# BoyBaykiller/IDKEngine

Hardware: AMD Instinct MI355X
Metric: Mray/s (primary+1 bounce) at 1920x1080, 1M-tri scene (higher is better)
Workload: dtype f32

## Files before the change

### idkengine_amd/csrc/host_context.hpp

```cpp
#pragma once


struct DevBuf {
    void* p = nullptr; size_t bytes = 0;
    hipError_t ensure(size_t n) { if (n <= bytes && p) return hipSuccess; if (p) (void)hipFree(p); p = nullptr; bytes = 0; if (n == 0) return hipSuccess; hipError_t e = hipMalloc(&p, n); if (e == hipSuccess) bytes = n; return e; }
    void release() { if (p) (void)hipFree(p); p = nullptr; bytes = 0; }
    template <class T> T* as() const { return (T*)p; }
};

struct DevOptions {
    int forceGeneric = 0;
    int noTileCull = 0;
    int noLeanPrimary = 0;
    int leafMin = 0;
    int grabUnitLog2 = 10, grabFixed = 0;
    int ldsPad = 0;
    int traceWaves = 0;
    int gridHint = 2;
    int deferLast = 1;
    int graphProbe = 0;
    int gridMidWaves = 20;
    int gridRaysX4 = 6;
    int traceVariant = 0;
    int bvhTiming = 0, bvhSmall = 32;
    int advMin = 0;
    int poolMin = 12;
    int leafPool = -1;
    int splitScatter = 6;
    int queryScheduler = 1;
    int groupThreads = -1;
    int fused = 1;
    int fusedShadeMin = 16;
    int splitPeek = 64;
    int splitDonor = 1;
    int split = 1;
    int wide = 0;
    int wideCap = 0;
    int wideCount = 0;
    int genPixelMajor = 8;
    int bouncePixelMajor = 1;
    int genGroupMax = 16;
    int instSieve = 8;
    int instSieveOverlap = 50;
    int instTlas = 8;
    int instTlasOverlap = 10;
    int instBraid = 0;
    int instUnify = 4096;
    int instGeneral = 0;
    int uniRefill = 32;
    int instUnifyRadius = 15;
    int pairNodes = 1;
    int packet = 1;
    int packetMinLive = 60;
    int packetWaves = 0;
    int bvhStackOptHost = 0;
};

enum { VB_NODES = 0, VB_TRIVERTS, VB_VERTICES, VB_TLAS, VB_XFORMS, VB_COUNT };
struct PendingSample { uint32_t accum; int slot; float cam[36]; uint8_t vs[VB_COUNT]; };

struct dev_ctx {
    int device = 0;
    hipStream_t stream = nullptr; bool ownStream = true;
    std::string lastError;
    idkpt_error_fn errFn = nullptr; void* errUser = nullptr;
    int numCUs = 256;
    idkpt_settings st;
    idkpt_settings stCaller;
    int W = 0, H = 0, rowMod = 1, rowRem = 0, rows = 0, rowBandLog2 = 0;
    float invProj[16], invView[16], viewPos[3];
    int ringSize = 1, curSlot = 0; bool ringStarted = false; std::vector<uint32_t> accum = std::vector<uint32_t>(1, 0u);
    bool counters = false, timing = false, capturePrimary = false;
    DevOptions opt;
    uint32_t seqFirst = 0, seqStride = 1;
    bool haveScene = false, frameOk = false;
    DevBuf nodes, tris, triVerts, descs, instances, tlas, parents, leaves, positions, prevPositions, vertices, meshes, materials, xforms, lights, sky, texDescs, unskinned, joints, levelNodes, tlasScratch, queryIn, queryOut, queryRec, queryList, tileClass, gbases;
    std::vector<DevBuf> texData; std::vector<std::pair<int, int>> texDims; std::vector<uint32_t> texState;
    DevBuf srgbLut;
    std::vector<GpuBlasDesc> hDescs;
    std::vector<std::vector<uint32_t>> levelOffsets;
    std::vector<uint32_t> levelBase;
    std::vector<char> refitCoversAll;
    int nodeCount = 0, triCount = 0, instanceCount = 0, tlasCount = 0, vertexCount = 0, meshCount = 0, materialCount = 0, xformCount = 0, lightCount = 0, skySize = 0, textureCount = 0, unskinnedCount = 0;
    int sceneStack = 1;
    int hInst0Blas = 0;
    DevBuf wnodes, wleaf, wids, wpair, wcounts, wtotals; std::vector<uint32_t> wNodeOff, wLeafOff; bool wideTopoValid = false, wideFillValid = false;
    DevBuf pairNodes; bool pairValid = false;
    DevBuf instRec; bool instRecValid = false;
    DevBuf itlas, imarks, ichunks; int itlasNeed = 1; uint32_t ichunkCount = 0; bool itlasValid = false, imarksValid = false;
    int uniMode = 0; uint32_t uniBaseB = 0, uniRestoreIdx = 0;
    DevBuf unodes, utlas, uTabs, uniBuf, uniEntRec; bool uniValid = false, uniEligible = false, uniTabsValid = false; int uniCap = 0, uniEntries = 0, uniDepth = 0; float* hUni = nullptr; float* dUni = nullptr;
    std::vector<GpuBlasInstance> hInstances; std::vector<char> hXforms; uint64_t uniLaunches = 0;
    DevBuf entRec, braidBuf; bool itlasBraided = false; int itlasDepth = 0, itlasEntries = 0;
    int pkState = 0, pkBatchesSinceProbe = 0; unsigned long long* hPkStats = nullptr; unsigned long long* dPkStats = nullptr; unsigned long long pkSeen[6] = {0, 0, 0, 0, 0, 0}; float pkCam[36] = {0}; int pkW = 0, pkRows = 0, pkBatch = 0; float pkLastLive = -1.0f;
    float* hInstOverlap = nullptr; float* dInstOverlap = nullptr; bool instOverlapKnown = false, itlasBuilt = false, isieveWorth = false;
    int verSlots = 1; size_t vbytes[VB_COUNT] = {0}, vstride[VB_COUNT] = {0}; int valloc[VB_COUNT] = {1, 1, 1, 1, 1}, vcur[VB_COUNT] = {0};
    uint64_t lastMask[VB_COUNT] = {0};
    uint8_t lastSlots[VB_COUNT] = {0}; bool lastMulti = false;
    DevBuf verTab; uint32_t* hVerTab = nullptr; hipEvent_t evVer[2] = {nullptr, nullptr}; int verHalf = 0;
    char* hStage = nullptr; hipEvent_t evStage[4] = {nullptr, nullptr, nullptr, nullptr}; int stageNext = 0;
    int (*groupFlushAll)(void* user) = nullptr;
    DevBuf pmList;
    DevBuf trRec, contFlag, blockSums, rayO, rayT, rayR, aovA, aovN, hit, hitCost, primHit, queue[2], keys[2], keysTmp, sortKeys, sortVals, contMask, waveCounts, counts, work, sortHist, counters64;
    DevBuf img[3];
    DevBuf camTab;
    int rowLimit = 0x7fffffff;
    idkpt_bounce_exchange_fn exchangeFn = nullptr; void* exchangeUser = nullptr;
    idkpt_band_exchange_fn bandExchangeFn = nullptr; void* bandExchangeUser = nullptr; DevBuf bandTab;
    idkpt_band_exchange_device_fn bandExchangeDevFn = nullptr; void* bandExchangeDevUser = nullptr;
    idkpt_stats stats;
    uint32_t* hCounts = nullptr; uint32_t* dCountsMirror = nullptr;
    bool sceneNested = false;
    bool sceneNoEmission = false;
    struct { bool valid = false, allHits = false; int j = 0, side = 0, B = 0; uint32_t total = 0, Npad = 0; } defer;
    DevBuf radSave, deferCount;
    bool countersDirty = true;
    uint32_t* hOverflow = nullptr; uint32_t* dOverflow = nullptr;
    int tlasNeed = 1;
    hipEvent_t evFrame[2] = {nullptr, nullptr};
    std::vector<hipEvent_t> evPool; size_t evUsed = 0;
    double traceMsAcc = 0.0; uint64_t traceLaunchesAcc = 0;
    int lastQueueSide = 0; int lastQueueCountSlot = 0; bool lastFast = false, lastNeedsRegen = false; int lastBatch = 1; Frame lastFrame;
    int maxBatch = 1; uint32_t Npad = 0; std::vector<PendingSample> pending; DevBuf bases, qwork; uint32_t* hBases = nullptr; uint32_t* dBasesMirror = nullptr;
    float* hCams = nullptr; hipEvent_t evCams[2] = {nullptr, nullptr}; int camHalf = 0;
    bool grouped = false, inGroupFlush = false; int groupIndex = 0;
    hipEvent_t* evBounce = nullptr;
    int (*groupExchange)(void* user, dev_ctx* member, int bounce, int samples, const uint32_t** outBases) = nullptr; void* groupUser = nullptr;
    struct BuilderScratch* bscratch = nullptr;
    struct PeerPolicy* peer = nullptr;
};

static hipEvent_t next_event(dev_ctx* ctx)
{
    if (ctx->evUsed == ctx->evPool.size()) { hipEvent_t e = nullptr; if (hipEventCreate(&e) != hipSuccess) return nullptr; ctx->evPool.push_back(e); }
    return ctx->evPool[ctx->evUsed++];
}
static void resolve_trace_events(dev_ctx* ctx)
{
    for (size_t i = 0; i + 1 < ctx->evUsed; i += 2) { float ms = 0.0f; if (hipEventElapsedTime(&ms, ctx->evPool[i], ctx->evPool[i + 1]) == hipSuccess) { ctx->traceMsAcc += ms; ctx->traceLaunchesAcc++; } }
    ctx->evUsed = 0;
}
#define TRACE_T0() do { if (ctx->timing) { hipEvent_t _e = next_event(ctx); if (_e) (void)hipEventRecord(_e, st); } } while (0)
#define TRACE_T1() do { if (ctx->timing) { hipEvent_t _e = next_event(ctx); if (_e) (void)hipEventRecord(_e, st); } } while (0)

static int fail(dev_ctx* c, int code, const std::string& msg) { if (c) { c->lastError = msg; if (c->errFn) c->errFn(c->errUser, (int32_t)code, c->lastError.c_str()); } return code; }
#define HIPC(expr) do { hipError_t _e = (expr); if (_e != hipSuccess) { (void)hipGetLastError(); return fail(ctx, IDKPT_ERR_HIP, std::string(#expr) + ": " + hipGetErrorString(_e)); } } while (0)
#define REQUIRE(cond, msg) do { if (!(cond)) return fail(ctx, IDKPT_ERR_INVALID_ARGUMENT, msg); } while (0)

static int local_rows(int H, int mod, int rem, int bandLog2 = 0)
{
    if (bandLog2 == 0) { int n = 0; for (int y = rem; y < H; y += mod) n++; return n; }
    int n = 0; const int band = 1 << bandLog2;
    for (int b = rem; (b << bandLog2) < H; b += mod) n += std::min(band, H - (b << bandLog2));
    return n;
}
```

### idkengine_amd/csrc/host_options.hpp

```cpp
#pragma once

static int32_t dev_SetOption(dev_ctx* ctx, const char* name, int32_t value)
{
    if (!ctx || !name) return IDKPT_ERR_INVALID_ARGUMENT;
    HIPC(hipSetDevice(ctx->device));
    FLUSH();
    DevOptions& o = ctx->opt;
    const std::string n(name);
    if (n == "force_generic") o.forceGeneric = value != 0;
    else if (n == "no_tile_cull") o.noTileCull = value != 0;
    else if (n == "no_lean_primary") o.noLeanPrimary = value != 0;
    else if (n == "leaf_min") o.leafMin = std::max(0, value);
    else if (n == "grab_unit_log2") o.grabUnitLog2 = value;
    else if (n == "grab_fixed") o.grabFixed = value;
    else if (n == "lds_pad") o.ldsPad = value;
    else if (n == "trace_waves") o.traceWaves = std::max(0, value);
    else if (n == "grid_hint") o.gridHint = std::max(0, value);
    else if (n == "grid_rays_x4") o.gridRaysX4 = std::max(0, value);
    else if (n == "grid_mid_waves") o.gridMidWaves = std::max(0, value);
    else if (n == "defer_last") o.deferLast = value != 0;
    else if (n == "split") { REQUIRE(value >= 0 && value <= 3, "idkptSetDeveloperOption: split is 0..3"); o.split = value; }
    else if (n == "split_donor") o.splitDonor = value != 0;
    else if (n == "split_peek") o.splitPeek = std::max(1, value);
    else if (n == "split_scatter") o.splitScatter = std::min(6, std::max(0, value));
    else if (n == "query_scheduler") o.queryScheduler = value != 0;
    else if (n == "group_threads") o.groupThreads = value;
    else if (n == "fused") { REQUIRE(value >= 0 && value <= 2, "idkptSetDeveloperOption: fused is 0..2"); o.fused = value; }
    else if (n == "fused_shade_min") o.fusedShadeMin = std::min(64, std::max(1, value));
    else if (n == "leaf_pool") { REQUIRE(value >= -1 && value <= 7, "idkptSetDeveloperOption: leaf_pool is -1 (automatic) or a mask 0..7 (1: primary launches, 2: the first bounce, 4: later bounces)"); o.leafPool = value; }
    else if (n == "pool_min") o.poolMin = std::max(0, value);
    else if (n == "adv_min") o.advMin = std::min(64, std::max(0, value));
#ifdef IDKPT_DEVELOPER
    else if (n == "graph_probe") o.graphProbe = std::max(0, value);
#endif
    else if (n == "inst_tlas_overlap") { REQUIRE(value >= 0 && value <= 100, "idkptSetDeveloperOption: inst_tlas_overlap is a percentage"); FLUSH(); o.instTlasOverlap = value; ctx->itlasValid = false; }
    else if (n == "bounce_pixel_major") { REQUIRE(value >= 0 && value <= 2, "idkptSetDeveloperOption: bounce_pixel_major is 0..2"); o.bouncePixelMajor = value; }
    else if (n == "gen_group_max") { REQUIRE(value >= 1 && value <= 16, "idkptSetDeveloperOption: gen_group_max is 1..16"); o.genGroupMax = value; }
    else if (n == "gen_pixel_major") { REQUIRE(value >= 0, "idkptSetDeveloperOption: gen_pixel_major is >= 0"); o.genPixelMajor = value; }
    else if (n == "inst_sieve_overlap") { REQUIRE(value >= 0 && value <= 100, "idkptSetDeveloperOption: inst_sieve_overlap is a percentage"); FLUSH(); o.instSieveOverlap = value; ctx->itlasValid = false; }
    else if (n == "inst_sieve") { REQUIRE(value >= 0, "idkptSetDeveloperOption: inst_sieve is >= 0"); FLUSH(); o.instSieve = value; ctx->itlasValid = false; }
    else if (n == "inst_braid") { REQUIRE(value >= 0, "idkptSetDeveloperOption: inst_braid is >= 0"); FLUSH(); o.instBraid = value; ctx->itlasValid = false; }
    else if (n == "pair_nodes") { REQUIRE(value == 0 || value == 1, "idkptSetDeveloperOption: pair_nodes is 0 or 1"); o.pairNodes = value; }
    else if (n == "inst_general") { REQUIRE(value >= 0, "idkptSetDeveloperOption: inst_general is >= 0"); FLUSH(); o.instGeneral = value; ctx->itlasValid = false; }
    else if (n == "uni_refill") { REQUIRE(value == 16 || value == 32, "idkptSetDeveloperOption: uni_refill is 16 or 32"); o.uniRefill = value; }
    else if (n == "inst_unify_radius") { REQUIRE(value >= 1 && value <= 512, "idkptSetDeveloperOption: inst_unify_radius is 1-512"); FLUSH(); o.instUnifyRadius = value; ctx->itlasValid = false; }
    else if (n == "inst_unify") { REQUIRE(value >= 0, "idkptSetDeveloperOption: inst_unify is >= 0"); FLUSH(); o.instUnify = value; ctx->itlasValid = false; }
    else if (n == "inst_tlas") { REQUIRE(value >= 0, "idkptSetDeveloperOption: inst_tlas is >= 0"); FLUSH(); o.instTlas = value; ctx->itlasValid = false; }
    else if (n == "packet") { REQUIRE(value >= 0 && value <= 2, "idkptSetDeveloperOption: packet is 0..2"); o.packet = value; ctx->pkState = 0; ctx->pkBatchesSinceProbe = 0; }
    else if (n == "packet_min_live") { REQUIRE(value >= 0 && value <= 100, "idkptSetDeveloperOption: packet_min_live is a percentage"); o.packetMinLive = value; ctx->pkState = 0; ctx->pkBatchesSinceProbe = 0; }
    else if (n == "packet_waves") { REQUIRE(value >= 0 && value <= 32, "idkptSetDeveloperOption: packet_waves is 0 (default) or 1..32"); o.packetWaves = value; }
    else if (n == "wide") { REQUIRE(value >= 0 && value <= 1, "idkptSetDeveloperOption: wide is 0 or 1"); FLUSH(); o.wide = value; }
    else if (n == "wide_cap") { REQUIRE(value >= 0 && value <= 96, "idkptSetDeveloperOption: wide_cap is 0 (default) or 4..96 rows"); o.wideCap = value; }
    else if (n == "wide_count") o.wideCount = value != 0;
    else if (n == "bvh_timing") o.bvhTiming = value != 0;
    else if (n == "bvh_small") o.bvhSmall = value;
    else if (n == "bvh_stackopt_host") o.bvhStackOptHost = value != 0;
    else if (n == "force_no_peer") { }
    else if (n == "trace_variant") {
#ifdef IDKPT_DEVELOPER
        o.traceVariant = value;
#else
        REQUIRE(value == 0 || value == 100, "idkptSetDeveloperOption: trace_variant needs the developer build of the library (libidkpt_dev.so)");
#endif
    }
    else return fail(ctx, IDKPT_ERR_INVALID_ARGUMENT, "idkptSetDeveloperOption: unknown option '" + n + "'");
    return IDKPT_OK;
}
```

### idkengine_amd/csrc/host_scene.hpp

```cpp
#pragma once

static int blas_stack_need(const GpuBlasNode* nodes, int nodeCount)
{
    std::vector<int> need((size_t)nodeCount, 0);
    for (int p = nodeCount - 2; p >= 2; p--) {
        const GpuBlasNode& l = nodes[p]; const GpuBlasNode& r = nodes[p + 1];
        const bool tl = l.TriCount == 0 && l.TriStartOrChild != 0, tr = r.TriCount == 0 && r.TriStartOrChild != 0;
        if (tl && tr) need[p] = std::max(need[l.TriStartOrChild], need[r.TriStartOrChild]) + 1;
        else if (tl || tr) need[p] = need[tl ? l.TriStartOrChild : r.TriStartOrChild];
    }
    return nodeCount > 2 ? need[2] : 0;
}

static int tlas_validate(const GpuTlasNode* nodes, int nodeCount, int instanceCount, const char** why)
{
    if (nodeCount <= 0) return 0;
    const uint32_t* w = (const uint32_t*)nodes;
    std::vector<int> need((size_t)nodeCount, 0);
    for (int i = nodeCount - 1; i >= 0; i--) {
        const uint32_t packed = w[8 * (size_t)i + 3], id = packed & 0x7fffffffu;
        if (packed >> 31) { if (id >= (uint32_t)instanceCount) { *why = "TLAS leaf references an instance out of range"; return -1; } continue; }
        if (id <= (uint32_t)i || (uint64_t)id + 1 >= (uint64_t)nodeCount) { *why = "TLAS child index out of range (children must lie behind their parent)"; return -1; }
        need[i] = std::max(need[id], need[id + 1]) + 1;
    }
// ... 4 lines not shown
{
    int maxStack = 1;
    for (int i = 0; i < descCount; i++) {
        const GpuBlasDesc& d = descs[i];
        if (!(d.NodeOffset >= 0 && d.NodeCount >= 4 && d.NodeOffset + d.NodeCount <= nodeCount && d.TriangleOffset >= 0 && d.TriangleOffset + d.TriangleCount <= triangleCount)) return "BlasDesc range out of bounds";
        for (int n = 1; n < d.NodeCount; n++) {
            const GpuBlasNode& nd = nodes[d.NodeOffset + n];
            if (nd.TriCount > 0) { if (!((uint64_t)nd.TriStartOrChild + nd.TriCount <= (uint64_t)d.TriangleCount)) return "leaf triangle range out of bounds"; }
            else if (n == 1 || nd.TriStartOrChild != 0) { if (!(nd.TriStartOrChild >= 2 && nd.TriStartOrChild > (uint32_t)n && nd.TriStartOrChild + 1 < (uint32_t)d.NodeCount)) return "child index out of bounds (children must lie behind their parent)"; }
        }
        const int need = blas_stack_need(nodes + d.NodeOffset, d.NodeCount);
        if (checkClaim && d.RequiredStackSize < need) return "BlasDesc.RequiredStackSize is smaller than the stack the BLAS needs";
        maxStack = std::max(maxStack, need);
    }
    *outMaxStack = maxStack;
    return nullptr;
}

static bool blas_nested(const GpuBlasNode* nodes, const GpuBlasDesc* descs, int descCount)
{
    for (int i = 0; i < descCount; i++) {
        const GpuBlasDesc& d = descs[i];
        for (int n = 1; n < d.NodeCount; n++) {
            const GpuBlasNode& p = nodes[d.NodeOffset + n];
            if (p.TriCount > 0 || p.TriStartOrChild == 0) continue;
            for (int k = 0; k < 2; k++) {
                const GpuBlasNode& c = nodes[d.NodeOffset + p.TriStartOrChild + k];
                if (c.TriCount == 0 && c.TriStartOrChild == 0 && n != 0) continue;
                for (int a = 0; a < 3; a++) if (!(c.Min[a] >= p.Min[a] && c.Max[a] <= p.Max[a])) return false;
            }
        }
    }
    return true;
}


static const char* dev_GetVersionString(void) { return "idkpt 0.1 (gfx950)"; }

static int32_t dev_GetDeviceCount(int32_t* outCount)
{
    int n = 0; hipError_t e = hipGetDeviceCount(&n);
    if (outCount) *outCount = (e == hipSuccess) ? n : 0;
    return e == hipSuccess ? IDKPT_OK : IDKPT_ERR_NO_DEVICE;
}

static int32_t dev_Create(int32_t deviceCount, const int32_t* deviceIds, dev_ctx** outCtx)
{
    if (!outCtx) return IDKPT_ERR_INVALID_ARGUMENT;
    *outCtx = nullptr;
    if (deviceCount != 1) return IDKPT_ERR_INVALID_ARGUMENT;
    int n = 0;
    if (hipGetDeviceCount(&n) != hipSuccess || n <= 0) return IDKPT_ERR_NO_DEVICE;
    int dev = deviceIds ? deviceIds[0] : 0;
    if (dev < 0 || dev >= n) return IDKPT_ERR_INVALID_ARGUMENT;
    if (hipSetDevice(dev) != hipSuccess) return IDKPT_ERR_HIP;
    dev_ctx* ctx = new dev_ctx();
    ctx->device = dev;
    hipDeviceProp_t prop;
    if (hipGetDeviceProperties(&prop, dev) == hipSuccess) ctx->numCUs = prop.multiProcessorCount;
    if (hipStreamCreateWithFlags(&ctx->stream, hipStreamNonBlocking) != hipSuccess) { delete ctx; return IDKPT_ERR_HIP; }
    memset(&ctx->st, 0, sizeof(ctx->st));
    ctx->st.Gpu.FocalLength = 8.0f; ctx->st.Gpu.DoRussianRoulette = 1; ctx->st.RayDepth = 7; ctx->st.SamplesPerPixel = 1;
    ctx->stCaller = ctx->st;
    memset(&ctx->stats, 0, sizeof(ctx->stats));
    memset(ctx->invProj, 0, 64); memset(ctx->invView, 0, 64); memset(ctx->viewPos, 0, 12);
    if (hipHostMalloc((void**)&ctx->hCounts, MAX_DEPTH_SLOTS * 4 + 16, hipHostMallocMapped) != hipSuccess || hipHostGetDevicePointer((void**)&ctx->dCountsMirror, ctx->hCounts, 0) != hipSuccess) { delete ctx; return IDKPT_ERR_OUT_OF_MEMORY; }
    memset(ctx->hCounts, 0, MAX_DEPTH_SLOTS * 4 + 16);
    if (hipHostMalloc((void**)&ctx->hOverflow, 64, hipHostMallocMapped) != hipSuccess || hipHostGetDevicePointer((void**)&ctx->dOverflow, ctx->hOverflow, 0) != hipSuccess) { delete ctx; return IDKPT_ERR_OUT_OF_MEMORY; }
    *ctx->hOverflow = 0;
    if (hipHostMalloc((void**)&ctx->hBases, MAX_DEPTH_SLOTS * (MAX_BATCH + 1) * 4, hipHostMallocMapped) != hipSuccess || hipHostGetDevicePointer((void**)&ctx->dBasesMirror, ctx->hBases, 0) != hipSuccess) { delete ctx; return IDKPT_ERR_OUT_OF_MEMORY; }
    memset(ctx->hBases, 0, MAX_DEPTH_SLOTS * (MAX_BATCH + 1) * 4);
    (void)hipEventCreate(&ctx->evFrame[0]); (void)hipEventCreate(&ctx->evFrame[1]);
    *outCtx = ctx;
    return IDKPT_OK;
}

static void builder_scratch_free(dev_ctx* ctx);
static int32_t dev_Destroy(dev_ctx* ctx)
{
    if (!ctx) return IDKPT_ERR_INVALID_ARGUMENT;
    (void)hipSetDevice(ctx->device);
    ctx->pending.clear();
    (void)hipStreamSynchronize(ctx->stream);
    DevBuf* all[] = {&ctx->srgbLut, &ctx->pmList, &ctx->pairNodes, &ctx->instRec, &ctx->entRec, &ctx->braidBuf, &ctx->unodes, &ctx->utlas, &ctx->uTabs, &ctx->uniBuf, &ctx->uniEntRec, &ctx->itlas, &ctx->imarks, &ctx->ichunks, &ctx->wnodes, &ctx->wleaf, &ctx->wids, &ctx->wpair, &ctx->wcounts, &ctx->wtotals, &ctx->nodes, &ctx->tris, &ctx->triVerts, &ctx->descs, &ctx->instances, &ctx->tlas, &ctx->parents, &ctx->leaves, &ctx->positions, &ctx->prevPositions, &ctx->vertices, &ctx->meshes,
                     &ctx->materials, &ctx->xforms, &ctx->lights, &ctx->sky, &ctx->texDescs, &ctx->unskinned, &ctx->joints, &ctx->levelNodes, &ctx->tlasScratch, &ctx->queryIn, &ctx->queryOut, &ctx->queryRec, &ctx->queryList, &ctx->bandTab, &ctx->tileClass, &ctx->gbases, &ctx->camTab, &ctx->verTab, &ctx->trRec, &ctx->contFlag, &ctx->blockSums, &ctx->rayO, &ctx->rayT, &ctx->rayR, &ctx->aovA, &ctx->aovN, &ctx->hit,
                     &ctx->hitCost, &ctx->primHit, &ctx->queue[0], &ctx->queue[1], &ctx->keys[0], &ctx->keys[1], &ctx->keysTmp, &ctx->sortKeys, &ctx->sortVals, &ctx->contMask, &ctx->waveCounts,
                     &ctx->counts, &ctx->work, &ctx->qwork, &ctx->radSave, &ctx->deferCount, &ctx->sortHist, &ctx->counters64, &ctx->bases, &ctx->img[0], &ctx->img[1], &ctx->img[2]};
    for (DevBuf* b : all) b->release();
    for (auto& t : ctx->texData) t.release();
    builder_scratch_free(ctx);
    if (ctx->hCounts) (void)hipHostFree(ctx->hCounts);
    if (ctx->hOverflow) (void)hipHostFree(ctx->hOverflow);
    if (ctx->hInstOverlap) (void)hipHostFree(ctx->hInstOverlap);
    if (ctx->hUni) (void)hipHostFree(ctx->hUni);
    if (ctx->hPkStats) (void)hipHostFree(ctx->hPkStats);
    if (ctx->hBases) (void)hipHostFree(ctx->hBases);
    if (ctx->hCams) (void)hipHostFree(ctx->hCams);
    for (int i = 0; i < 2; i++) if (ctx->evCams[i]) (void)hipEventDestroy(ctx->evCams[i]);
    if (ctx->hVerTab) (void)hipHostFree(ctx->hVerTab);
    for (int i = 0; i < 2; i++) if (ctx->evVer[i]) (void)hipEventDestroy(ctx->evVer[i]);
    if (ctx->hStage) (void)hipHostFree(ctx->hStage);
    for (int i = 0; i < 4; i++) if (ctx->evStage[i]) (void)hipEventDestroy(ctx->evStage[i]);
    if (ctx->evFrame[0]) (void)hipEventDestroy(ctx->evFrame[0]);
    if (ctx->evFrame[1]) (void)hipEventDestroy(ctx->evFrame[1]);
    for (hipEvent_t e : ctx->evPool) (void)hipEventDestroy(e);
    if (ctx->ownStream && ctx->stream) (void)hipStreamDestroy(ctx->stream);
    delete ctx;
    return IDKPT_OK;
}

static int32_t dev_GetLastError(dev_ctx* ctx, const char** outMessage)
{
    if (!ctx || !outMessage) return IDKPT_ERR_INVALID_ARGUMENT;
    *outMessage = ctx->lastError.c_str();
    return IDKPT_OK;
}

static int32_t dev_SetSize(dev_ctx* ctx, int32_t width, int32_t height)
{
    if (!ctx) return IDKPT_ERR_INVALID_ARGUMENT;
    REQUIRE(width > 0 && height > 0 && width <= 4096 && height <= 65536, "idkptSetSize: bad size (FirstHit seeds pack x into 12 bits: width <= 4096)");
    HIPC(hipSetDevice(ctx->device));
    FLUSH();
    REQUIRE(ctx->rowLimit == 0x7fffffff || ctx->rowRem + ctx->rowLimit <= height, "idkptSetSize: the strip set by idkptSetRowRange exceeds the new image height (set a new range first)");
    REQUIRE((ctx->rowRem << ctx->rowBandLog2) < height, "idkptSetSize: this context's row remainder (idkptSetRowSharding / idkptSetRowBands) is outside the new image height");
    ctx->W = width; ctx->H = height; ctx->rows = std::min(ctx->rowLimit, local_rows(height, ctx->rowMod, ctx->rowRem, ctx->rowBandLog2));
    return alloc_frame(ctx);
}

static int32_t dev_SetLayout(dev_ctx* ctx, int32_t width, int32_t height, int32_t rowMod, int32_t rowRem, int32_t rowLimit, int32_t bandLog2 = 0)
{
    if (!ctx) return IDKPT_ERR_INVALID_ARGUMENT;
    REQUIRE(width > 0 && height > 0 && width <= 4096 && height <= 65536, "idkptSetSize: bad size (FirstHit seeds pack x into 12 bits: width <= 4096)");
    REQUIRE(rowMod >= 1 && rowRem >= 0 && bandLog2 >= 0 && bandLog2 <= 6 && (rowRem << bandLog2) < height && rowLimit >= 1 && (rowMod == 1 ? bandLog2 == 0 : rowRem < rowMod), "internal: bad row layout");
    HIPC(hipSetDevice(ctx->device));
    FLUSH();
    ctx->W = width; ctx->H = height; ctx->rowMod = rowMod; ctx->rowRem = rowRem; ctx->rowLimit = rowLimit; ctx->rowBandLog2 = bandLog2;
    ctx->rows = std::min(rowLimit, local_rows(height, rowMod, rowRem, bandLog2));
    return alloc_frame(ctx);
}

static int32_t dev_SetRowBands(dev_ctx* ctx, int32_t bandRows, int32_t rowModulo, int32_t rowRemainder)
{
    if (!ctx) return IDKPT_ERR_INVALID_ARGUMENT;
    REQUIRE(bandRows >= 1 && bandRows <= 64 && (bandRows & (bandRows - 1)) == 0, "idkptSetRowBands: bandRows must be a power of two in 1..64");
    REQUIRE(rowModulo >= 1 && rowRemainder >= 0 && rowRemainder < rowModulo, "idkptSetRowSharding / idkptSetRowBands: need 0 <= remainder < modulo");
    int bandLog2 = 0; while ((1 << bandLog2) < bandRows) bandLog2++;
    if (rowModulo == 1) bandLog2 = 0;
    REQUIRE(ctx->W <= 0 || (rowRemainder << bandLog2) < ctx->H, "idkptSetRowSharding / idkptSetRowBands: no row of the image has this remainder");
    FLUSH();
    ctx->rowMod = rowModulo; ctx->rowRem = rowRemainder; ctx->rowLimit = 0x7fffffff; ctx->rowBandLog2 = bandLog2;
    if (ctx->W > 0) { HIPC(hipSetDevice(ctx->device)); ctx->rows = local_rows(ctx->H, rowModulo, rowRemainder, bandLog2); return alloc_frame(ctx); }
    return IDKPT_OK;
}
static int32_t dev_SetRowSharding(dev_ctx* ctx, int32_t rowModulo, int32_t rowRemainder) { return dev_SetRowBands(ctx, 1, rowModulo, rowRemainder); }

static int32_t dev_SetRowRange(dev_ctx* ctx, int32_t firstRow, int32_t rowCount)
{
    if (!ctx) return IDKPT_ERR_INVALID_ARGUMENT;
    REQUIRE(firstRow >= 0 && rowCount >= 1, "idkptSetRowRange: need firstRow >= 0 and rowCount >= 1");
    REQUIRE(ctx->W <= 0 || firstRow + rowCount <= ctx->H, "idkptSetRowRange: strip exceeds the image height");
    FLUSH();
    ctx->rowMod = 1; ctx->rowRem = firstRow; ctx->rowLimit = rowCount; ctx->rowBandLog2 = 0;
    if (ctx->W > 0) { HIPC(hipSetDevice(ctx->device)); ctx->rows = std::min(ctx->rowLimit, local_rows(ctx->H, 1, firstRow)); return alloc_frame(ctx); }
    return IDKPT_OK;
}

// ... 9 lines not shown
{
    if (!ctx) return IDKPT_ERR_INVALID_ARGUMENT;
    FLUSH();
    ctx->bandExchangeFn = fn; ctx->bandExchangeUser = user;
    return IDKPT_OK;
}

static int32_t dev_SetBandExchangeDevice(dev_ctx* ctx, idkpt_band_exchange_device_fn fn, void* user)
{
    if (!ctx) return IDKPT_ERR_INVALID_ARGUMENT;
    FLUSH();
    ctx->bandExchangeDevFn = fn; ctx->bandExchangeDevUser = user;
    return IDKPT_OK;
}

static int32_t dev_SetSettings(dev_ctx* ctx, const idkpt_settings* s)
{
    if (!ctx || !s) return IDKPT_ERR_INVALID_ARGUMENT;
    REQUIRE(s->RayDepth >= 1 && s->RayDepth < MAX_DEPTH_SLOTS - 2, "idkptSetSettings: RayDepth out of range (1..61)");
    REQUIRE(s->SamplesPerPixel >= 1, "idkptSetSettings: SamplesPerPixel must be >= 1");
    REQUIRE(s->BlasStackSize >= 0, "idkptSetSettings: BlasStackSize must be >= 0 (0 = derive from BlasDescs)");
    REQUIRE(s->BlasStackSize == 0 || !ctx->haveScene || s->BlasStackSize >= ctx->sceneStack, "idkptSetSettings: BlasStackSize is smaller than the scene's maximum RequiredStackSize");
    if (memcmp(&ctx->stCaller, s, sizeof(*s)) == 0) return IDKPT_OK;
    FLUSH();
    ctx->stCaller = *s;
    const idkpt_settings o = ctx->st;
    bool reset = o.RayDepth != s->RayDepth || o.Gpu.FocalLength != s->Gpu.FocalLength || o.Gpu.LenseRadius != s->Gpu.LenseRadius ||
                 o.Gpu.DoDebugBVHTraversal != s->Gpu.DoDebugBVHTraversal || o.Gpu.DoTraceLights != s->Gpu.DoTraceLights || o.UseTlas != s->UseTlas;
    ctx->st = *s;
    if (ctx->st.Gpu.DoDebugBVHTraversal) ctx->st.RayDepth = 1;
    if (reset) std::fill(ctx->accum.begin(), ctx->accum.end(), 0u);
    return IDKPT_OK;
}
static int32_t dev_GetSettings(dev_ctx* ctx, idkpt_settings* out) { if (!ctx || !out) return IDKPT_ERR_INVALID_ARGUMENT; *out = ctx->st; return IDKPT_OK; }

static int32_t dev_SetPerFrame(dev_ctx* ctx, const float invProjection[16], const float invView[16], const float viewPos[3])
{
    if (!ctx || !invProjection || !invView || !viewPos) return IDKPT_ERR_INVALID_ARGUMENT;
    if (ctx->ringSize == 1 && (memcmp(ctx->invProj, invProjection, 64) || memcmp(ctx->invView, invView, 64) || memcmp(ctx->viewPos, viewPos, 12))) FLUSH_KEEP();
    memcpy(ctx->invProj, invProjection, 64); memcpy(ctx->invView, invView, 64); memcpy(ctx->viewPos, viewPos, 12);
    return IDKPT_OK;
}
static int32_t dev_SetPerFrameData(dev_ctx* ctx, const GpuPerFrameData* p) { if (!ctx || !p) return IDKPT_ERR_INVALID_ARGUMENT; return dev_SetPerFrame(ctx, p->InvProjection, p->InvView, p->ViewPos); }

static int regather_triverts(dev_ctx* ctx, uint32_t first, uint32_t count)
{
    if (count == 0) return IDKPT_OK;
    char *src, *dst; int rc = ver_writable(ctx, VB_TRIVERTS, first == 0 && count == (uint32_t)ctx->triCount, &src, &dst); if (rc) return rc;
    hipLaunchKernelGGL(k_gather_triverts, dim3((count + 255) / 256), dim3(256), 0, ctx->stream, ctx->tris.as<uint4>(), ctx->positions.as<float>(), (float4*)dst, first, count);
    HIPC(hipGetLastError());
    return IDKPT_OK;
}

static int upload(dev_ctx* ctx, DevBuf& b, const void* src, size_t bytes)
{
    HIPC(b.ensure(std::max<size_t>(bytes, 16)));
    if (bytes) HIPC(hipMemcpyAsync(b.p, src, bytes, hipMemcpyHostToDevice, ctx->stream));
    return IDKPT_OK;
}

static size_t tex_texel_bytes(int32_t format) { return format == IDKPT_TEXFMT_RGBA32F ? 16 : 4; }
static int tex_validate(dev_ctx* ctx, const idkpt_texture& t, const char* who)
{
    if (!(t.width > 0 && t.height > 0 && t.rgba)) return fail(ctx, IDKPT_ERR_INVALID_ARGUMENT, std::string(who) + ": bad texture (size / data)");
    if (!(t.wrapS >= 0 && t.wrapS <= 2 && t.wrapT >= 0 && t.wrapT <= 2 && t.magFilter >= 0 && t.magFilter <= 1 && t.format >= 0 && t.format <= 2))
        return fail(ctx, IDKPT_ERR_INVALID_ARGUMENT, std::string(who) + ": bad texture (wrapS / wrapT are enum idkpt_wrap, magFilter enum idkpt_filter, format enum idkpt_texture_format)");
    return IDKPT_OK;
}
static uint32_t tex_state(const idkpt_texture& t) { return (uint32_t)t.wrapS | ((uint32_t)t.wrapT << 2) | ((uint32_t)t.magFilter << 4) | ((uint32_t)t.format << 5); }
static bool tex_all_finite(const idkpt_texture& t)
{
    if (t.format != IDKPT_TEXFMT_RGBA32F) return true;
    const uint32_t* w = reinterpret_cast<const uint32_t*>(t.rgba); uint32_t bad = 0;
    for (size_t k = 0, e = (size_t)t.width * t.height * 4; k < e; k++) bad |= (uint32_t)((w[k] & 0x7f800000u) == 0x7f800000u);
    return !bad;
}
static int tex_srgb_lut(dev_ctx* ctx)
{
    if (ctx->srgbLut.p) return IDKPT_OK;
    float lut[256];
    for (int b = 0; b < 256; b++) { const double cs = (double)b / 255.0; lut[b] = (float)(cs <= 0.04045 ? cs / 12.92 : pow((cs + 0.055) / 1.055, 2.4)); }
    HIPC(ctx->srgbLut.ensure(sizeof(lut)));
    HIPC(hipMemcpy(ctx->srgbLut.p, lut, sizeof(lut), hipMemcpyHostToDevice));
    return IDKPT_OK;
}
static int tex_descs_upload(dev_ctx* ctx)
{
    std::vector<TexDesc> td;
    for (size_t i = 0; i < ctx->texData.size(); i++) td.push_back({ctx->texData[i].p, ctx->texDims[i].first, ctx->texDims[i].second, ctx->texState[i], 0u});
    { int rc = upload(ctx, ctx->texDescs, td.data(), td.size() * sizeof(TexDesc)); if (rc) return rc; }
    if (!td.empty()) HIPC(hipStreamSynchronize(ctx->stream));
    return IDKPT_OK;
}

static DScene make_dscene_last(dev_ctx* ctx);
static int materialize_culled_rays(dev_ctx* ctx)
{
    if (!ctx->lastNeedsRegen) return IDKPT_OK;
    const size_t N = (size_t)ctx->W * ctx->rows;
    RayBufs rays = {ctx->rayO.as<float4>(), ctx->rayT.as<float4>(), ctx->rayR.as<float4>(), ctx->aovA.as<float4>(), ctx->aovN.as<float4>()};
    hipLaunchKernelGGL(k_regen_culled, dim3((unsigned)((N + 255) / 256)), dim3(256), 0, ctx->stream, make_dscene_last(ctx), ctx->lastFrame, rays, (const uint8_t*)ctx->contFlag.as<uint8_t>(), (uint32_t)(ctx->lastBatch - 1), (uint32_t)N);
    HIPC(hipGetLastError());
    ctx->lastNeedsRegen = false;
    return IDKPT_OK;
}

static int32_t dev_UploadScene(dev_ctx* ctx, const idkpt_scene_desc* sc)
{
    if (!ctx || !sc) return IDKPT_ERR_INVALID_ARGUMENT;
    REQUIRE(sc->BlasNodes && sc->BlasNodeCount >= 4, "idkptUploadScene: BlasNodes missing");
    REQUIRE(sc->BlasTriangles && sc->BlasTriangleCount > 0, "idkptUploadScene: BlasTriangles missing");
    REQUIRE(sc->BlasDescs && sc->BlasDescCount > 0 && sc->BlasInstances && sc->BlasInstanceCount > 0, "idkptUploadScene: BlasDescs/BlasInstances missing");
    REQUIRE(sc->VertexPositions && sc->Vertices && sc->VertexCount > 0, "idkptUploadScene: vertices missing");
    REQUIRE(sc->Meshes && sc->MeshCount > 0 && sc->Materials && sc->MaterialCount > 0 && sc->MeshTransforms && sc->MeshTransformCount > 0, "idkptUploadScene: meshes/materials/transforms missing");
    REQUIRE(sc->LightCount >= 0 && sc->LightCount <= IDKPT_MAX_LIGHTS, "idkptUploadScene: more than 256 lights");
    for (int i = 0; i < sc->BlasTriangleCount; i++) { const GpuBlasTriangle& t = sc->BlasTriangles[i]; REQUIRE(t.X < (uint32_t)sc->VertexCount && t.Y < (uint32_t)sc->VertexCount && t.Z < (uint32_t)sc->VertexCount && t.MeshId < (uint32_t)sc->MeshCount, "idkptUploadScene: BlasTriangle index out of range"); }
    for (int i = 0; i < sc->MeshCount; i++) REQUIRE(sc->Meshes[i].MaterialId >= 0 && sc->Meshes[i].MaterialId < sc->MaterialCount, "idkptUploadScene: Mesh.MaterialId out of range");
    for (int i = 0; i < sc->BlasInstanceCount; i++) REQUIRE(sc->BlasInstances[i].BlasId < (uint32_t)sc->BlasDescCount && sc->BlasInstances[i].MeshTransformId < (uint32_t)sc->MeshTransformCount, "idkptUploadScene: BlasInstance out of range");
    int maxStack = 1;
    { const char* why = validate_blas_nodes(sc->BlasNodes, sc->BlasNodeCount, sc->BlasDescs, sc->BlasDescCount, sc->BlasTriangleCount, true, &maxStack); REQUIRE(why == nullptr, std::string("idkptUploadScene: ") + (why ? why : "")); }
    REQUIRE(ctx->st.BlasStackSize == 0 || ctx->st.BlasStackSize >= maxStack, "idkptUploadScene: the BlasStackSize set with idkptSetSettings is smaller than this scene's maximum RequiredStackSize");
    int tlasNeed = 1;
    if (sc->TlasNodes && sc->TlasNodeCount > 0) {
        const char* why = nullptr;
        tlasNeed = tlas_validate(sc->TlasNodes, sc->TlasNodeCount, sc->BlasInstanceCount, &why);
        REQUIRE(tlasNeed >= 0, std::string("idkptUploadScene: ") + (why ? why : "bad TLAS"));
        REQUIRE(tlasNeed <= TLAS_STACK_SIZE, "idkptUploadScene: TLAS deeper than TLAS_STACK_SIZE (32)");
    }
    HIPC(hipSetDevice(ctx->device));
    FLUSH();
    { int rc = materialize_culled_rays(ctx); if (rc) return rc; }
    int rc;
    if ((rc = upload(ctx, ctx->nodes, sc->BlasNodes, (size_t)sc->BlasNodeCount * 32))) return rc;
    if ((rc = upload(ctx, ctx->tris, sc->BlasTriangles, (size_t)sc->BlasTriangleCount * 16))) return rc;
    if ((rc = upload(ctx, ctx->descs, sc->BlasDescs, (size_t)sc->BlasDescCount * sizeof(GpuBlasDesc)))) return rc;
    if ((rc = upload(ctx, ctx->instances, sc->BlasInstances, (size_t)sc->BlasInstanceCount * 8))) return rc;
    if ((rc = upload(ctx, ctx->tlas, sc->TlasNodes, (size_t)(sc->TlasNodes ? sc->TlasNodeCount : 0) * 32))) return rc;
    if ((rc = upload(ctx, ctx->parents, sc->BlasParentIndices, (size_t)(sc->BlasParentIndices ? sc->BlasParentIndexCount : 0) * 4))) return rc;
    if ((rc = upload(ctx, ctx->leaves, sc->BlasLeafIndices, (size_t)(sc->BlasLeafIndices ? sc->BlasLeafIndexCount : 0) * 4))) return rc;
    if ((rc = upload(ctx, ctx->positions, sc->VertexPositions, (size_t)sc->VertexCount * 12))) return rc;
    if ((rc = upload(ctx, ctx->vertices, sc->Vertices, (size_t)sc->VertexCount * 16))) return rc;
    if ((rc = upload(ctx, ctx->meshes, sc->Meshes, (size_t)sc->MeshCount * sizeof(GpuMesh)))) return rc;
    if ((rc = upload(ctx, ctx->materials, sc->Materials, (size_t)sc->MaterialCount * sizeof(GpuMaterial)))) return rc;
    if ((rc = upload(ctx, ctx->xforms, sc->MeshTransforms, (size_t)sc->MeshTransformCount * sizeof(GpuMeshTransform)))) return rc;
    HIPC(ctx->lights.ensure(IDKPT_MAX_LIGHTS * sizeof(GpuLight)));
    if (sc->Lights && sc->LightCount) HIPC(hipMemcpyAsync(ctx->lights.p, sc->Lights, (size_t)sc->LightCount * sizeof(GpuLight), hipMemcpyHostToDevice, ctx->stream));
    {
        bool none = true;
        auto fin = [](float v) { return v - v == 0.0f; };
        for (int i = 0; i < sc->MaterialCount && none; i++) { const GpuMaterial& m = sc->Materials[i]; none = m.EmissiveFactor[0] == 0.0f && m.EmissiveFactor[1] == 0.0f && m.EmissiveFactor[2] == 0.0f && fin(m.Absorbance[0]) && fin(m.Absorbance[1]) && fin(m.Absorbance[2]); }
        for (int i = 0; i < sc->MeshCount && none; i++) none = sc->Meshes[i].EmissiveBias == 0.0f && fin(sc->Meshes[i].AbsorbanceBias[0]) && fin(sc->Meshes[i].AbsorbanceBias[1]) && fin(sc->Meshes[i].AbsorbanceBias[2]);
        for (int i = 0; i < sc->TextureCount && none; i++) {
            const idkpt_texture& t = sc->Textures[i];
            if (!(t.width > 0 && t.height > 0 && t.rgba)) { none = false; break; }
            none = tex_all_finite(t);
        }
        ctx->sceneNoEmission = none;
    }
    ctx->skySize = (sc->SkyFaces && sc->SkyFaceSize > 0) ? sc->SkyFaceSize : 0;
    if ((rc = upload(ctx, ctx->sky, sc->SkyFaces, (size_t)6 * ctx->skySize * ctx->skySize * 16))) return rc;
    for (auto& t : ctx->texData) t.release();
    ctx->texData.clear(); ctx->texDims.clear(); ctx->texState.clear();
    if ((rc = tex_srgb_lut(ctx))) return rc;
    for (int i = 0; i < sc->TextureCount; i++) {
        const idkpt_texture& t = sc->Textures[i];
        if ((rc = tex_validate(ctx, t, "idkptUploadScene"))) return rc;
        ctx->texData.emplace_back();
        if ((rc = upload(ctx, ctx->texData.back(), t.rgba, (size_t)t.width * t.height * tex_texel_bytes(t.format)))) return rc;
        ctx->texDims.push_back({t.width, t.height}); ctx->texState.push_back(tex_state(t));
    }
    if ((rc = tex_descs_upload(ctx))) return rc;
    HIPC(ctx->triVerts.ensure((size_t)sc->BlasTriangleCount * 48));
    ctx->nodeCount = sc->BlasNodeCount; ctx->triCount = sc->BlasTriangleCount; ctx->instanceCount = sc->BlasInstanceCount; ctx->tlasCount = sc->TlasNodes ? sc->TlasNodeCount : 0;
    ctx->vertexCount = sc->VertexCount; ctx->meshCount = sc->MeshCount; ctx->materialCount = sc->MaterialCount; ctx->xformCount = sc->MeshTransformCount;
    ctx->lightCount = sc->Lights ? sc->LightCount : 0; ctx->textureCount = sc->TextureCount;
    ctx->hDescs.assign(sc->BlasDescs, sc->BlasDescs + sc->BlasDescCount); ctx->hInst0Blas = (int)sc->BlasInstances[0].BlasId;
    ctx->hInstances.assign(sc->BlasInstances, sc->BlasInstances + sc->BlasInstanceCount);
    ctx->hXforms.assign((const char*)sc->MeshTransforms, (const char*)sc->MeshTransforms + (size_t)sc->MeshTransformCount * sizeof(GpuMeshTransform));
    ctx->sceneStack = maxStack; ctx->tlasNeed = std::max(1, tlasNeed);
    ctx->sceneNested = blas_nested(sc->BlasNodes, sc->BlasDescs, sc->BlasDescCount);
    ver_reset(ctx);
    if ((rc = ver_reserve(ctx))) return rc;
    ctx->levelOffsets.assign(sc->BlasDescCount, {}); ctx->levelBase.assign(sc->BlasDescCount, 0); ctx->refitCoversAll.assign(sc->BlasDescCount, 0);
    std::vector<int32_t> allLevels;
    for (int bi = 0; bi < sc->BlasDescCount; bi++) {
        const GpuBlasDesc& d = sc->BlasDescs[bi];
        if (!d.IsRefittable) continue;
        std::vector<int> depth(d.NodeCount, 0); int maxD = 0;
        for (int n = 1; n < d.NodeCount; n++) { const GpuBlasNode& nd = sc->BlasNodes[d.NodeOffset + n]; if (nd.TriCount == 0) { int c = (int)nd.TriStartOrChild; depth[c] = depth[c + 1] = depth[n] + 1; maxD = std::max(maxD, depth[n]); } }
        std::vector<std::vector<int32_t>> lv(maxD + 1);
        for (int n = 1; n < d.NodeCount; n++) if (sc->BlasNodes[d.NodeOffset + n].TriCount == 0 && (n == 1 || n >= 2)) lv[depth[n]].push_back(n);
        ctx->levelBase[bi] = (uint32_t)allLevels.size();
        uint32_t off = 0;
        for (auto& l : lv) { ctx->levelOffsets[bi].push_back(off); off += (uint32_t)l.size(); allLevels.insert(allLevels.end(), l.begin(), l.end()); }
        ctx->levelOffsets[bi].push_back(off);
        ctx->refitCoversAll[bi] = (int64_t)off + (int64_t)d.LeafIndicesCount == (int64_t)d.NodeCount - 1;
    }
    if ((rc = upload(ctx, ctx->levelNodes, allLevels.data(), allLevels.size() * 4))) return rc;
    if ((rc = regather_triverts(ctx, 0, (uint32_t)sc->BlasTriangleCount))) return rc;
    HIPC(hipStreamSynchronize(ctx->stream));
    ctx->haveScene = true;
    std::fill(ctx->accum.begin(), ctx->accum.end(), 0u);
    return IDKPT_OK;
}

struct PeerPolicy { bool forceStaged = false, warned = false; void* stage = nullptr; size_t stageBytes = 0; };
static hipError_t member_copy(PeerPolicy* pol, void* dst, int dstDev, const void* src, int srcDev, size_t bytes, hipStream_t st)
{
    if (bytes == 0) return hipSuccess;
    if (!pol || !pol->forceStaged) {
        hipError_t e = hipMemcpyPeerAsync(dst, dstDev, src, srcDev, bytes, st);
        if (e == hipSuccess || !pol) return e;
        (void)hipGetLastError();
        if (!pol->warned) { fprintf(stderr, "[idkpt] warning: peer copy GPU %d -> GPU %d refused (%s); staging device-to-device copies through host memory from now on\n", srcDev, dstDev, hipGetErrorString(e)); pol->warned = true; }
        pol->forceStaged = true;
    }
    hipError_t e = hipStreamSynchronize(st); if (e != hipSuccess) return e;
    if (pol->stageBytes < bytes) {
        if (pol->stage) (void)hipHostFree(pol->stage);
        pol->stage = nullptr; pol->stageBytes = 0;
        e = hipHostMalloc(&pol->stage, bytes, hipHostMallocDefault); if (e != hipSuccess) return e;
        pol->stageBytes = bytes;
    }
    int cur = 0; (void)hipGetDevice(&cur);
    e = hipSetDevice(srcDev); if (e == hipSuccess) e = hipMemcpy(pol->stage, src, bytes, hipMemcpyDeviceToHost);
    if (e == hipSuccess) e = hipSetDevice(dstDev);
    if (e == hipSuccess) e = hipMemcpy(dst, pol->stage, bytes, hipMemcpyHostToDevice);
    (void)hipSetDevice(cur);
    return e;
}

struct CloneItem { void* dst; const void* src; size_t bytes; };
static int clone_prepare(dev_ctx* ctx, dev_ctx* src, std::vector<CloneItem>& items)
{
    if (!ctx || !src || !src->haveScene) return IDKPT_ERR_INVALID_ARGUMENT;
    items.clear();
    HIPC(hipSetDevice(ctx->device));
    FLUSH();
    { int rc = materialize_culled_rays(ctx); if (rc) return rc; }
    DevBuf* d[] = {&ctx->nodes, &ctx->tris, &ctx->triVerts, &ctx->descs, &ctx->instances, &ctx->tlas, &ctx->parents, &ctx->leaves, &ctx->positions, &ctx->vertices, &ctx->meshes,
                   &ctx->materials, &ctx->xforms, &ctx->lights, &ctx->sky, &ctx->levelNodes};
    DevBuf* f[] = {&src->nodes, &src->tris, &src->triVerts, &src->descs, &src->instances, &src->tlas, &src->parents, &src->leaves, &src->positions, &src->vertices, &src->meshes,
                   &src->materials, &src->xforms, &src->lights, &src->sky, &src->levelNodes};
    for (size_t i = 0; i < sizeof(d) / sizeof(d[0]); i++) {
        if (!f[i]->p || f[i]->bytes == 0) continue;
        int vb = -1; for (int b = 0; b < VB_COUNT; b++) if (f[i] == &vb_buf(src, b)) vb = b;
        const size_t bytes = (vb >= 0 && src->vbytes[vb] > 0) ? src->vbytes[vb] : f[i]->bytes;
        const char* from = (vb >= 0 && src->vbytes[vb] > 0) ? vb_ptr(src, vb, src->vcur[vb]) : (const char*)f[i]->p;
        HIPC(d[i]->ensure(bytes));
        items.push_back({d[i]->p, from, bytes});
    }
    for (auto& t : ctx->texData) t.release();
    ctx->texData.clear(); ctx->texDims = src->texDims; ctx->texState = src->texState;
    for (size_t i = 0; i < src->texData.size(); i++) {
        ctx->texData.emplace_back();
        HIPC(ctx->texData.back().ensure(src->texData[i].bytes));
        items.push_back({ctx->texData.back().p, src->texData[i].p, src->texData[i].bytes});
    }
    return IDKPT_OK;
}
static int clone_finish(dev_ctx* ctx, dev_ctx* src)
{
    HIPC(hipSetDevice(ctx->device));
    { int rc = tex_srgb_lut(ctx); if (rc) return rc; }
    { int rc = tex_descs_upload(ctx); if (rc) return rc; }
    ctx->nodeCount = src->nodeCount; ctx->triCount = src->triCount; ctx->instanceCount = src->instanceCount; ctx->tlasCount = src->tlasCount; ctx->vertexCount = src->vertexCount;
    ctx->meshCount = src->meshCount; ctx->materialCount = src->materialCount; ctx->xformCount = src->xformCount; ctx->lightCount = src->lightCount; ctx->skySize = src->skySize;
    ctx->textureCount = src->textureCount; ctx->hDescs = src->hDescs; ctx->hInstances = src->hInstances; ctx->hXforms = src->hXforms; ctx->hInst0Blas = src->hInst0Blas; ctx->sceneNoEmission = src->sceneNoEmission; ctx->sceneNested = src->sceneNested; ctx->sceneStack = src->sceneStack; ctx->tlasNeed = src->tlasNeed;
    ctx->levelOffsets = src->levelOffsets; ctx->levelBase = src->levelBase; ctx->refitCoversAll = src->refitCoversAll;
    ver_reset(ctx);
    { int rc = ver_reserve(ctx); if (rc) return rc; }
    HIPC(hipStreamSynchronize(ctx->stream));
    ctx->haveScene = true;
    std::fill(ctx->accum.begin(), ctx->accum.end(), 0u);
    return IDKPT_OK;
}

static int32_t dev_CloneSceneFrom(dev_ctx* ctx, dev_ctx* src)
{
    std::vector<CloneItem> items;
    int rc = clone_prepare(ctx, src, items); if (rc) return rc;
    for (const CloneItem& it : items) HIPC(member_copy(ctx->peer, it.dst, ctx->device, it.src, src->device, it.bytes, ctx->stream));
    return clone_finish(ctx, src);
}

static int32_t dev_UpdateTexture(dev_ctx* ctx, int32_t index, const idkpt_texture* t)
{
    if (!ctx || !t) return IDKPT_ERR_INVALID_ARGUMENT;
    if (!ctx->haveScene) return fail(ctx, IDKPT_ERR_INVALID_OPERATION, "idkptUpdateTexture: no scene uploaded");
    REQUIRE(index >= 0 && index < ctx->textureCount, "idkptUpdateTexture: index out of range");
    { int rc = tex_validate(ctx, *t, "idkptUpdateTexture"); if (rc) return rc; }
    HIPC(hipSetDevice(ctx->device));
    FLUSH();
    HIPC(hipStreamSynchronize(ctx->stream));
    { int rc = upload(ctx, ctx->texData[index], t->rgba, (size_t)t->width * t->height * tex_texel_bytes(t->format)); if (rc) return rc; }
    HIPC(hipStreamSynchronize(ctx->stream));
    ctx->texDims[index] = {t->width, t->height}; ctx->texState[index] = tex_state(*t);
    if (!tex_all_finite(*t)) ctx->sceneNoEmission = false;
    return tex_descs_upload(ctx);
}

static int32_t dev_SetLightCount(dev_ctx* ctx, int32_t count)
{
    if (!ctx) return IDKPT_ERR_INVALID_ARGUMENT;
    REQUIRE(count >= 0 && count <= IDKPT_MAX_LIGHTS, "idkptSetLightCount: out of range");
    FLUSH();
    ctx->lightCount = count; return IDKPT_OK;
}

static DevBuf* which_buffer(dev_ctx* ctx, int which, size_t* cap, int* vb)
{
    *vb = -1;
    switch (which) {
        case IDKPT_BUF_MESH_TRANSFORMS: *cap = (size_t)ctx->xformCount * sizeof(GpuMeshTransform); *vb = VB_XFORMS; return &ctx->xforms;
        case IDKPT_BUF_VERTEX_POSITIONS: *cap = (size_t)ctx->vertexCount * 12; return &ctx->positions;
        case IDKPT_BUF_VERTICES: *cap = (size_t)ctx->vertexCount * 16; *vb = VB_VERTICES; return &ctx->vertices;
        case IDKPT_BUF_MESHES: *cap = (size_t)ctx->meshCount * sizeof(GpuMesh); return &ctx->meshes;
        case IDKPT_BUF_MATERIALS: *cap = (size_t)ctx->materialCount * sizeof(GpuMaterial); return &ctx->materials;
        case IDKPT_BUF_LIGHTS: *cap = (size_t)IDKPT_MAX_LIGHTS * sizeof(GpuLight); return &ctx->lights;
        case IDKPT_BUF_BLAS_NODES: *cap = (size_t)ctx->nodeCount * 32; *vb = VB_NODES; return &ctx->nodes;
        case IDKPT_BUF_TLAS_NODES: *cap = (size_t)ctx->tlasCount * 32; *vb = VB_TLAS; return &ctx->tlas;
        case IDKPT_BUF_JOINT_MATRICES: *cap = ctx->joints.bytes; return &ctx->joints;
        default: return nullptr;
    }
}

static int32_t dev_UpdateBuffer(dev_ctx* ctx, int32_t which, size_t offsetBytes, size_t bytes, const void* data)
{
    if (!ctx || !data) return IDKPT_ERR_INVALID_ARGUMENT;
    if (!ctx->haveScene) return fail(ctx, IDKPT_ERR_INVALID_OPERATION, "idkptUpdateBuffer: no scene uploaded");
    HIPC(hipSetDevice(ctx->device));
    if (which == IDKPT_BUF_MESHES || which == IDKPT_BUF_MATERIALS || which == IDKPT_BUF_LIGHTS || which == IDKPT_BUF_BLAS_NODES || which == IDKPT_BUF_TLAS_NODES) FLUSH();
    if (which == IDKPT_BUF_JOINT_MATRICES) { size_t need = offsetBytes + bytes; if (need > ctx->joints.bytes) { DevBuf nb; HIPC(nb.ensure(need)); if (ctx->joints.p) { HIPC(hipMemcpyAsync(nb.p, ctx->joints.p, ctx->joints.bytes, hipMemcpyDeviceToDevice, ctx->stream)); } HIPC(hipStreamSynchronize(ctx->stream)); ctx->joints.release(); ctx->joints = nb; } }
    size_t cap = 0; int vb = -1; DevBuf* b = which_buffer(ctx, which, &cap, &vb);
    REQUIRE(b != nullptr, "idkptUpdateBuffer: unknown buffer");
    REQUIRE(offsetBytes + bytes <= cap, "idkptUpdateBuffer: range exceeds buffer");
    if (which == IDKPT_BUF_BLAS_NODES || which == IDKPT_BUF_TLAS_NODES) {
        char* cur = vb_ptr(ctx, vb, ctx->vcur[vb]);
        std::vector<char> h(cap);
        HIPC(hipMemcpyAsync(h.data(), cur, cap, hipMemcpyDeviceToHost, ctx->stream)); HIPC(hipStreamSynchronize(ctx->stream));
        memcpy(h.data() + offsetBytes, data, bytes);
        if (which == IDKPT_BUF_BLAS_NODES) {
            int maxStack = 1;
            const char* why = validate_blas_nodes((const GpuBlasNode*)h.data(), ctx->nodeCount, ctx->hDescs.data(), (int)ctx->hDescs.size(), ctx->triCount, false, &maxStack);
            REQUIRE(why == nullptr, std::string("idkptUpdateBuffer: ") + (why ? why : ""));
            REQUIRE(ctx->st.BlasStackSize == 0 || ctx->st.BlasStackSize >= maxStack, "idkptUpdateBuffer: the patched BLAS needs a deeper traversal stack than the BlasStackSize set with idkptSetSettings");
            HIPC(hipMemcpyAsync(cur + offsetBytes, data, bytes, hipMemcpyHostToDevice, ctx->stream));
            ctx->sceneStack = maxStack; ctx->pairValid = false; ctx->wideTopoValid = false; ctx->wideFillValid = false; ctx->itlasValid = false; ctx->instRecValid = false; ctx->imarksValid = false;
            ctx->sceneNested = blas_nested((const GpuBlasNode*)h.data(), ctx->hDescs.data(), (int)ctx->hDescs.size());
        } else {
            const char* why = nullptr;
            const int need = tlas_validate((const GpuTlasNode*)h.data(), ctx->tlasCount, ctx->instanceCount, &why);
            REQUIRE(need >= 0, std::string("idkptUpdateBuffer: ") + (why ? why : "bad TLAS"));
            REQUIRE(need <= TLAS_STACK_SIZE, "idkptUpdateBuffer: TLAS deeper than TLAS_STACK_SIZE (32)");
            HIPC(hipMemcpyAsync(cur + offsetBytes, data, bytes, hipMemcpyHostToDevice, ctx->stream));
            ctx->tlasNeed = std::max(1, need);
        }
        HIPC(hipStreamSynchronize(ctx->stream));
        return IDKPT_OK;
    }
    if (which == IDKPT_BUF_MESHES || which == IDKPT_BUF_MATERIALS) ctx->sceneNoEmission = false;
    char* dst = (char*)b->p;
    if (vb >= 0) { char* src; int rc = ver_writable(ctx, vb, offsetBytes == 0 && bytes == cap, &src, &dst); if (rc) return rc; }
    { int rc = staged_upload(ctx, dst + offsetBytes, data, bytes); if (rc) return rc; }
    if (which == IDKPT_BUF_MESH_TRANSFORMS && offsetBytes + bytes <= ctx->hXforms.size()) memcpy(ctx->hXforms.data() + offsetBytes, data, bytes);
    if (which == IDKPT_BUF_VERTEX_POSITIONS) { int rc = regather_triverts(ctx, 0, (uint32_t)ctx->triCount); if (rc) return rc; }
    return IDKPT_OK;
}

static int32_t dev_DownloadBuffer(dev_ctx* ctx, int32_t which, size_t offsetBytes, size_t bytes, void* dst)
{
    if (!ctx || !dst) return IDKPT_ERR_INVALID_ARGUMENT;
    if (which == IDKPT_BUF_WIDE_NODES || which == IDKPT_BUF_WIDE_LEAVES || which == IDKPT_BUF_WIDE_COUNTS) {
        if (!ctx->haveScene) return fail(ctx, IDKPT_ERR_INVALID_OPERATION, "idkptDownloadBuffer: no scene uploaded");
        HIPC(hipSetDevice(ctx->device));
        FLUSH();
        { int rc = wide_prepare(ctx); if (rc) return rc; }
        DevBuf& wbuf = which == IDKPT_BUF_WIDE_NODES ? ctx->wnodes : (which == IDKPT_BUF_WIDE_LEAVES ? ctx->wleaf : ctx->wcounts);
        REQUIRE(offsetBytes + bytes <= (which == IDKPT_BUF_WIDE_COUNTS ? ctx->hDescs.size() * 8 : wbuf.bytes), "idkptDownloadBuffer: bad buffer/range");
        HIPC(hipMemcpyAsync(dst, (char*)wbuf.p + offsetBytes, bytes, hipMemcpyDeviceToHost, ctx->stream));
        HIPC(hipStreamSynchronize(ctx->stream));
        return IDKPT_OK;
    }
    size_t cap = 0; int vb = -1; DevBuf* b = which_buffer(ctx, which, &cap, &vb);
    REQUIRE(b != nullptr && offsetBytes + bytes <= cap, "idkptDownloadBuffer: bad buffer/range");
    HIPC(hipSetDevice(ctx->device));
    FLUSH();
    HIPC(hipMemcpyAsync(dst, (vb >= 0 ? vb_ptr(ctx, vb, ctx->vcur[vb]) : (char*)b->p) + offsetBytes, bytes, hipMemcpyDeviceToHost, ctx->stream));
    HIPC(hipStreamSynchronize(ctx->stream));
    return IDKPT_OK;
}

static int32_t dev_BuildTlas(dev_ctx* ctx, const GpuTlasNode* nodes, int32_t nodeCount)
{
    if (!ctx || !nodes || nodeCount <= 0) return IDKPT_ERR_INVALID_ARGUMENT;
    if (!ctx->haveScene) return fail(ctx, IDKPT_ERR_INVALID_OPERATION, "idkptBuildTlas: no scene uploaded");
    const char* why = nullptr;
    const int need = tlas_validate(nodes, nodeCount, ctx->instanceCount, &why);
    REQUIRE(need >= 0, std::string("idkptBuildTlas: ") + (why ? why : "bad TLAS"));
    REQUIRE(need <= TLAS_STACK_SIZE, "idkptBuildTlas: TLAS deeper than TLAS_STACK_SIZE (32)");
    HIPC(hipSetDevice(ctx->device));
    if ((size_t)nodeCount * 32 > ctx->vbytes[VB_TLAS] || nodeCount != ctx->tlasCount) {
        FLUSH();
        if ((size_t)nodeCount * 32 > ctx->vbytes[VB_TLAS]) {
            HIPC(hipStreamSynchronize(ctx->stream));
            ctx->tlas.release();
            ctx->vbytes[VB_TLAS] = (size_t)nodeCount * 32; ctx->vstride[VB_TLAS] = (ctx->vbytes[VB_TLAS] + 255) / 256 * 256; ctx->valloc[VB_TLAS] = 1; ctx->vcur[VB_TLAS] = 0;
            HIPC(ctx->tlas.ensure(ctx->vstride[VB_TLAS]));
        }
    }
    char *src, *dst; int rc = ver_writable(ctx, VB_TLAS, true, &src, &dst); if (rc) return rc;
    HIPC(hipMemcpyAsync(dst, nodes, (size_t)nodeCount * 32, hipMemcpyHostToDevice, ctx->stream));
    HIPC(hipStreamSynchronize(ctx->stream));
    ctx->tlasCount = nodeCount; ctx->tlasNeed = std::max(1, need);
    return IDKPT_OK;
}

static int32_t dev_BuildTlasOnDevice(dev_ctx* ctx, int32_t searchRadius)
{
    if (!ctx) return IDKPT_ERR_INVALID_ARGUMENT;
    if (!ctx->haveScene) return fail(ctx, IDKPT_ERR_INVALID_OPERATION, "idkptBuildTlasOnDevice: no scene uploaded");
    REQUIRE(searchRadius >= 1, "idkptBuildTlasOnDevice: searchRadius must be >= 1 (reference: 15)");
    HIPC(hipSetDevice(ctx->device));
    const int n = ctx->instanceCount, nodeCount = 2 * n - 1;
    if (nodeCount != ctx->tlasCount) FLUSH();
    char *tsrc, *tdst; { int rc = ver_writable(ctx, VB_TLAS, true, &tsrc, &tdst); if (rc) return rc; }
    const size_t tempOff = 0, leafOff = (size_t)nodeCount * 32, keyOff = leafOff + (size_t)n * 32, prefOff = keyOff + (size_t)n * 4;
    HIPC(ctx->tlasScratch.ensure(prefOff + (size_t)n * 4));
    char* sc = ctx->tlasScratch.as<char>();
    hipLaunchKernelGGL(k_tlas_build, dim3(1), dim3(TLAS_BUILD_THREADS), 0, ctx->stream, (const float4*)vb_cur<float4>(ctx, VB_NODES), ctx->descs.as<GpuBlasDesc>(), ctx->instances.as<GpuBlasInstance>(),
                       (const float4*)vb_cur<float4>(ctx, VB_XFORMS), n, (int)searchRadius, (float4*)tdst, (float4*)(sc + tempOff), (float4*)(sc + leafOff), (uint32_t*)(sc + keyOff), (int*)(sc + prefOff));
    HIPC(hipGetLastError());
    ctx->tlasCount = nodeCount; ctx->tlasNeed = std::min(TLAS_STACK_SIZE, std::max(1, n));
    return IDKPT_OK;
}

static int32_t dev_RefitBlas(dev_ctx* ctx, int32_t blasId)
{
    if (!ctx) return IDKPT_ERR_INVALID_ARGUMENT;
    if (!ctx->haveScene) return fail(ctx, IDKPT_ERR_INVALID_OPERATION, "idkptRefitBlas: no scene uploaded");
    REQUIRE(blasId >= 0 && blasId < (int)ctx->hDescs.size(), "idkptRefitBlas: blasId out of range");
    const GpuBlasDesc& d = ctx->hDescs[blasId];
    if (!d.IsRefittable || d.LeafIndicesCount == 0) return fail(ctx, IDKPT_ERR_INVALID_OPERATION, "idkptRefitBlas: BLAS is not refittable (no leaf/parent indices)");
    HIPC(hipSetDevice(ctx->device));
    int rc = regather_triverts(ctx, (uint32_t)d.TriangleOffset, (uint32_t)d.TriangleCount); if (rc) return rc;
    const bool whole = ctx->hDescs.size() == 1 && d.NodeOffset == 0 && d.NodeCount == ctx->nodeCount && ctx->refitCoversAll[blasId];
    char *nsrc, *ndst; rc = ver_writable(ctx, VB_NODES, whole, &nsrc, &ndst); if (rc) return rc;
    if (whole && nsrc != ndst) HIPC(hipMemcpyAsync(ndst, nsrc, 32, hipMemcpyDeviceToDevice, ctx->stream));
// ... 50 lines not shown
```

### idkengine_amd/csrc/host_schedule.hpp

```cpp
#pragma once

static DScene make_dscene(dev_ctx* ctx, const uint8_t* slots, bool multi)
{
    DScene s;
    auto at = [&](int b) -> char* { return multi ? (char*)vb_buf(ctx, b).p : vb_ptr(ctx, b, slots ? slots[b] : ctx->vcur[b]); };
    s.nodes = (const float4*)at(VB_NODES); s.tris = ctx->tris.as<uint4>(); s.triVerts = (const float4*)at(VB_TRIVERTS);
    s.descs = ctx->descs.as<GpuBlasDesc>(); s.instances = ctx->instances.as<GpuBlasInstance>(); s.instanceCount = ctx->instanceCount;
    s.tlas = (const float4*)at(VB_TLAS); s.tlasCount = ctx->tlasCount; s.vertices = (const uint4*)at(VB_VERTICES);
    s.instRec = nullptr;
    s.pairNodes = nullptr;
    s.meshes = ctx->meshes.as<GpuMesh>(); s.materials = ctx->materials.as<GpuMaterial>(); s.xforms = (const float4*)at(VB_XFORMS);
    s.lights = ctx->lights.as<GpuLight>(); s.lightCount = ctx->lightCount; s.sky = ctx->sky.as<float4>(); s.skySize = ctx->skySize;
    s.textures = ctx->texDescs.as<TexDesc>(); s.textureCount = ctx->textureCount; s.srgbLut = ctx->srgbLut.as<float>();
    s.overflow = ctx->dOverflow;
    s.ver = multi ? ctx->verTab.as<uint32_t>() : nullptr;
    return s;
}
static DScene make_dscene(dev_ctx* ctx) { return make_dscene(ctx, nullptr, false); }
static DScene make_dscene_last(dev_ctx* ctx) { return make_dscene(ctx, ctx->lastSlots, ctx->lastMulti); }

static float4* image_ptr(dev_ctx* ctx, int i, int slot) { return ctx->img[i].as<float4>() + (size_t)slot * ((size_t)ctx->W * ctx->rows); }

#define GRID_MID_RAYS 14000000u
#define SPLIT_MAX_RAYS 1500000u
static bool want_split(const dev_ctx* ctx, uint32_t prev, bool known, int samples)
{
    if (ctx->opt.split == 0) return false;
    if (ctx->opt.split >= 2) return true;
    return known && sparse_view(ctx, samples) && prev > 0u && prev < SPLIT_MAX_RAYS;
}
#define FUSED_MAX_RAYS 600000u
static bool want_fused(const dev_ctx* ctx, uint32_t prev, bool known, int samples)
{
    if (ctx->opt.fused == 0) return false;
    if (ctx->opt.fused >= 2) return true;
    const uint64_t pixels = (uint64_t)ctx->W * ctx->rows * (uint64_t)std::max(1, samples);
    return known && prev > 0u && prev < FUSED_MAX_RAYS && (uint64_t)prev * 2u < pixels;
}
static uint32_t small_launch_grid(uint32_t fullGrid, uint32_t prev, int hintMul, int raysX4, uint32_t midGrid)
{
    if (prev == 0u || hintMul <= 0) return fullGrid;
    const uint32_t cap = std::max<uint32_t>(256u, (uint32_t)(((uint64_t)hintMul * prev + 63) / 64));
    uint32_t g = cap;
    if (raysX4 > 0) g = std::max<uint32_t>((uint32_t)(((uint64_t)prev * 4u / (uint32_t)raysX4 + 63) / 64), std::min<uint32_t>(cap, 1024u));
    if (midGrid > 0u && prev < GRID_MID_RAYS) g = std::min(g, midGrid);
    return std::min(fullGrid, std::min(g, cap));
}

static int finish_deferred(dev_ctx* ctx)
{
    if (!ctx->defer.valid) return IDKPT_OK;
    ctx->defer.valid = false;
    using namespace ptd;
    hipStream_t st = ctx->stream;
    const int j = ctx->defer.j, side = ctx->defer.side, B = ctx->defer.B, BS = MAX_BATCH + 1;
    const uint32_t total = ctx->defer.total, Npad = ctx->defer.Npad, gridTotal = (total + 255) / 256;
    const Frame f = ctx->lastFrame;
    DScene s = make_dscene_last(ctx);
    const bool multiVer = ctx->lastMulti;
    RayBufs rays = {ctx->rayO.as<float4>(), ctx->rayT.as<float4>(), ctx->rayR.as<float4>(), ctx->aovA.as<float4>(), ctx->aovN.as<float4>()};
    HitBufs hits = {ctx->hit.as<float4>(), ctx->hitCost.as<float>()};
    TraceBufs tr = {ctx->trRec.as<float4>(), nullptr, nullptr};
    uint32_t* counts = ctx->counts.as<uint32_t>(); uint32_t* bases = ctx->bases.as<uint32_t>();
    unsigned long long* contMask = ctx->contMask.as<unsigned long long>();
    uint32_t* waveLocal = ctx->waveCounts.as<uint32_t>(); uint32_t* blockSums = ctx->blockSums.as<uint32_t>(); uint32_t* keysTmp = ctx->keysTmp.as<uint32_t>();
    const uint32_t scanBlocks = ((total + 63) / 64 + SCAN_WAVES_PER_BLOCK - 1) / SCAN_WAVES_PER_BLOCK;
    const uint32_t* q = ctx->queue[side].as<uint32_t>();
    const uint32_t* cnt = ctx->deferCount.as<uint32_t>();
    if (ctx->defer.allHits) hipLaunchKernelGGL((k_restore_last<true>), dim3(gridTotal), dim3(256), 0, st, rays, hits, q, cnt, (const float4*)ctx->radSave.as<float4>(), f.hitsByRid);
    else hipLaunchKernelGGL((k_restore_last<false>), dim3(gridTotal), dim3(256), 0, st, rays, hits, q, cnt, (const float4*)ctx->radSave.as<float4>(), f.hitsByRid);
    if (multiVer) hipLaunchKernelGGL((k_shade<false, true>), dim3(gridTotal), dim3(256), 0, st, s, f, rays, tr, hits, q, cnt, 0u, (const uint32_t*)(bases + j * BS), (const uint32_t*)nullptr, contMask, waveLocal, keysTmp);
    else hipLaunchKernelGGL((k_shade<false, false>), dim3(gridTotal), dim3(256), 0, st, s, f, rays, tr, hits, q, cnt, 0u, (const uint32_t*)(bases + j * BS), (const uint32_t*)nullptr, contMask, waveLocal, keysTmp);
    hipLaunchKernelGGL((k_scan_local<false>), dim3(scanBlocks), dim3(SCAN_WAVES_PER_BLOCK), 0, st, cnt, 0u, (const uint8_t*)nullptr, contMask, waveLocal, blockSums);
    hipLaunchKernelGGL(k_scan_blocks, dim3(1), dim3(1024), 0, st, cnt, 0u, blockSums, (const uint32_t*)waveLocal, counts + j + 1, (unsigned long long*)nullptr,
                       (const unsigned long long*)contMask, (const uint32_t*)(bases + j * BS), Npad, B, bases + (j + 1) * BS,
                       ctx->dCountsMirror + j + 1, ctx->dBasesMirror + (size_t)(j + 1) * BS, (const uint32_t*)nullptr, (uint32_t*)nullptr);
    hipLaunchKernelGGL((k_compact<false>), dim3(gridTotal), dim3(256), 0, st, q, cnt, 0u, (const unsigned long long*)contMask, (const uint32_t*)waveLocal, (const uint32_t*)blockSums,
                       (const uint32_t*)keysTmp, ctx->queue[1 - side].as<uint32_t>(), ctx->keys[1 - side].as<uint32_t>());
    HIPC(hipGetLastError());
    ctx->lastQueueSide = 1 - side;
    ctx->countersDirty = true;
    return IDKPT_OK;
}

static int flush_batch(dev_ctx* ctx)
{
    const int B = (int)ctx->pending.size();
    if (B == 0) return IDKPT_OK;
    if (ctx->grouped && !ctx->inGroupFlush) return fail(ctx, IDKPT_ERR_UNKNOWN, "internal: a member of a multi-device context was flushed on its own");
    const uint32_t N = (uint32_t)((size_t)ctx->W * ctx->rows);
    const uint32_t Npad = ctx->Npad;
    const uint32_t total = (uint32_t)B * Npad;
    bool multiVer = false;
    for (int k = 1; k < B && !multiVer; k++) multiVer = memcmp(ctx->pending[k].vs, ctx->pending[0].vs, VB_COUNT) != 0;
    for (int b = 0; b < VB_COUNT; b++) { uint64_t m = 0; for (int k = 0; k < B; k++) m |= 1ull << ctx->pending[k].vs[b]; ctx->lastMask[b] = m; ctx->lastSlots[b] = ctx->pending[0].vs[b]; }
    ctx->lastMulti = multiVer;
    if (multiVer) {
        if (!ctx->hVerTab) {
            HIPC(hipHostMalloc((void**)&ctx->hVerTab, (size_t)2 * MAX_BATCH * SCENE_VER_WORDS * 4, hipHostMallocDefault));
            for (int i = 0; i < 2; i++) HIPC(hipEventCreateWithFlags(&ctx->evVer[i], hipEventDisableTiming));
            ctx->verHalf = 0;
        } else HIPC(hipEventSynchronize(ctx->evVer[ctx->verHalf]));
        uint32_t* stage = ctx->hVerTab + (size_t)ctx->verHalf * MAX_BATCH * SCENE_VER_WORDS;
        for (int k = 0; k < B; k++) {
            const uint8_t* vs = ctx->pending[k].vs;
            uint32_t* row = stage + (size_t)k * SCENE_VER_WORDS;
            for (int b = 0; b < VB_COUNT; b++) row[b] = (uint32_t)(((size_t)vs[b] * ctx->vstride[b]) / 16);
            for (int b = VB_COUNT; b < SCENE_VER_WORDS; b++) row[b] = 0u;
        }
        HIPC(ctx->verTab.ensure((size_t)MAX_BATCH * SCENE_VER_WORDS * 4));
        HIPC(hipMemcpyAsync(ctx->verTab.p, stage, (size_t)B * SCENE_VER_WORDS * 4, hipMemcpyHostToDevice, ctx->stream));
        HIPC(hipEventRecord(ctx->evVer[ctx->verHalf], ctx->stream));
        ctx->verHalf ^= 1;
    }
    DScene s = make_dscene_last(ctx);
    Frame f; memset(&f, 0, sizeof(f));
    memcpy(f.invProj, ctx->pending[0].cam, 64); memcpy(f.invView, ctx->pending[0].cam + 16, 64); memcpy(f.viewPos, ctx->pending[0].cam + 32, 12);
    f.W = ctx->W; f.H = ctx->H; f.rowMod = ctx->rowMod; f.rowRem = ctx->rowRem; f.rows = ctx->rows; f.rowBandLog2 = ctx->rowBandLog2;
    f.g = ctx->st.Gpu; f.useTlas = ctx->st.UseTlas;
    f.stackCap = std::max(1, ctx->st.BlasStackSize > 0 ? ctx->st.BlasStackSize : ctx->sceneStack);
    f.outputAovs = ctx->st.OutputAOVs;
    f.batch = B; f.Npad = Npad;
    HIPC(ctx->trRec.ensure((size_t)ctx->maxBatch * Npad * 64));
    for (int k = 0; k < MAX_BATCH; k++) { f.accum[k] = k < B ? ctx->pending[k].accum : 0u; f.slotOf[k] = (uint32_t)(k < B ? ctx->pending[k].slot : 0); }
    f.seqFirst = ctx->seqFirst; f.seqStride = ctx->seqStride;
    f.accumulated = f.seqFirst + f.accum[0] * f.seqStride;
    f.cams = nullptr;
    if (ctx->ringSize > 1) {
        if (!ctx->hCams) {
            HIPC(hipHostMalloc((void**)&ctx->hCams, (size_t)2 * MAX_BATCH * 36 * 4, hipHostMallocDefault));
            for (int i = 0; i < 2; i++) HIPC(hipEventCreateWithFlags(&ctx->evCams[i], hipEventDisableTiming));
            ctx->camHalf = 0;
        } else HIPC(hipEventSynchronize(ctx->evCams[ctx->camHalf]));
        float* stage = ctx->hCams + (size_t)ctx->camHalf * MAX_BATCH * 36;
        for (int k = 0; k < B; k++) memcpy(stage + (size_t)k * 36, ctx->pending[k].cam, 36 * 4);
        HIPC(ctx->camTab.ensure((size_t)MAX_BATCH * 36 * 4));
        HIPC(hipMemcpyAsync(ctx->camTab.p, stage, (size_t)B * 36 * 4, hipMemcpyHostToDevice, ctx->stream));
        HIPC(hipEventRecord(ctx->evCams[ctx->camHalf], ctx->stream));
        ctx->camHalf ^= 1;
        f.cams = ctx->camTab.as<float>();
    }
    f.tilePerSample = (f.cams != nullptr || multiVer) ? 1 : 0;
    RayBufs rays = {ctx->rayO.as<float4>(), ctx->rayT.as<float4>(), ctx->rayR.as<float4>(), ctx->aovA.as<float4>(), ctx->aovN.as<float4>()};
    HitBufs hits = {ctx->hit.as<float4>(), ctx->hitCost.as<float>()};
    uint32_t* counts = ctx->counts.as<uint32_t>();
    uint32_t* bases = ctx->bases.as<uint32_t>();
    uint32_t* work = ctx->work.as<uint32_t>();
    uint64_t* counters = ctx->counters64.as<uint64_t>();
    const int depth = ctx->st.RayDepth;
    hipStream_t st = ctx->stream;
#ifdef IDKPT_DEVELOPER
    bool capturing = false;
    if (ctx->opt.graphProbe > 0 && !ctx->timing) capturing = hipStreamBeginCapture(st, hipStreamCaptureModeThreadLocal) == hipSuccess;
#endif
    if (ctx->timing) HIPC(hipEventRecord(ctx->evFrame[0], st));
    ctx->defer.valid = false;
    if (ctx->countersDirty) { HIPC(hipMemsetAsync(work, 0, WORK_WORDS * 4, st)); HIPC(hipMemsetAsync(counts, 0, MAX_DEPTH_SLOTS * 4, st)); }
    ctx->countersDirty = true;
    uint32_t* hostCounts = ctx->dCountsMirror; uint32_t* hostBases = ctx->dBasesMirror;

    f.tlasCap = std::min(TLAS_STACK_SIZE, std::max(1, ctx->tlasNeed));
    f.grabUnitLog2 = std::min(24, std::max(6, ctx->opt.grabUnitLog2)); f.grabFixed = std::max(0, ctx->opt.grabFixed);
    f.leafMin = ctx->opt.leafMin > 0 ? ctx->opt.leafMin : (B >= 4 ? 16 : 12);
    const bool fast = fast_path(ctx);
    f.genPixelMajor = (fast && ctx->opt.genPixelMajor > 0 && B >= ctx->opt.genPixelMajor && !f.tilePerSample) ? 1 : 0;
    TracePlan plan; { int rc = trace_plan(ctx, f, s, multiVer, false, false, plan); if (rc) { ctx->pending.clear(); return rc; } }
    const size_t ldsBytes = plan.ldsBytes; const int wavesPerCU = plan.wavesPerCU; const bool fused = plan.fused;
    const uint32_t traceGrid = std::min<uint32_t>(plan.grid, std::max<uint32_t>(1u, (uint32_t)(((size_t)B * N + 63) / 64)));
    const uint32_t midGrid = (ctx->opt.gridMidWaves > 0 && ctx->opt.traceWaves == 0) ? (uint32_t)(ctx->numCUs * std::min(wavesPerCU, ctx->opt.gridMidWaves)) : 0u;
    f.gridRaysX4 = (uint32_t)std::max(0, ctx->opt.gridRaysX4); f.gridMid = midGrid; f.gridMidRays = GRID_MID_RAYS; f.splitMode = (ctx->opt.split == 3 ? 2 : 1) | (ctx->opt.splitDonor ? 4 : 0); f.poolMin = ctx->opt.poolMin; f.advMin = ctx->opt.advMin > 0 ? ctx->opt.advMin : (B >= 4 ? 8 : 1); f.splitPeek = ctx->opt.splitPeek;
    const bool debug = f.g.DoDebugBVHTraversal != 0;
    const uint32_t gridTotal = (total + 255) / 256;
    f.shadeMin = ctx->opt.fusedShadeMin; f.scatterLog2 = ctx->opt.splitScatter;
    if (!fast && (B != 1 || multiVer)) { ctx->pending.clear(); return fail(ctx, IDKPT_ERR_UNKNOWN, "internal: generic path is never batched"); }
    unsigned long long* contMask = ctx->contMask.as<unsigned long long>();
    uint32_t* waveCounts = ctx->waveCounts.as<uint32_t>();
    const int BS = MAX_BATCH + 1;

    const uint8_t* tileClass = nullptr;
    uint32_t* activeList = ctx->sortVals.as<uint32_t>();
    uint32_t* activeCount = counts + (MAX_DEPTH_SLOTS - 1);
    uint32_t* pmList = nullptr; uint32_t* const pmCount = counts + (MAX_DEPTH_SLOTS - 2); bool pmBounce = false;
    TraceBufs tr = {ctx->trRec.as<float4>(), nullptr, nullptr};
    TraceBufs trNone = {nullptr, nullptr, nullptr};
    uint32_t* waveLocal = waveCounts;
    uint32_t* blockSums = ctx->blockSums.as<uint32_t>();
    const uint32_t scanBlocks = ((total + 63) / 64 + SCAN_WAVES_PER_BLOCK - 1) / SCAN_WAVES_PER_BLOCK;
    uint32_t* keysTmp = ctx->keysTmp.as<uint32_t>();
    {
        if (fast) {
            const uint32_t tilesX = ((uint32_t)f.W + 7) / 8, tilesY = ((uint32_t)f.rows + 7) / 8;
            const uint32_t genWaves = tilesX * tilesY;
            const int cull = f.g.DoTraceLights ? 0 : 1;
            const bool noLean = ctx->opt.noLeanPrimary != 0;
            const int lean = (cull && !f.useTlas && s.instanceCount == 1 && !noLean) ? 1 : 0;
            if (ctx->capturePrimary) hipLaunchKernelGGL(k_fill_miss, dim3((N + 255) / 256), dim3(256), 0, st, hits, (size_t)(B - 1) * Npad, N);
            tileClass = nullptr;
            if (cull && !ctx->opt.noTileCull) {
                const uint32_t classSets = f.tilePerSample ? (uint32_t)B : 1u;
                HIPC(ctx->tileClass.ensure((size_t)genWaves * classSets));
                if (multiVer) hipLaunchKernelGGL((k_classify_tiles<true>), dim3((genWaves + 255) / 256, classSets), dim3(256), 0, st, s, f, ctx->tileClass.as<uint8_t>(), tilesX, tilesY);
                else hipLaunchKernelGGL((k_classify_tiles<false>), dim3((genWaves + 255) / 256, classSets), dim3(256), 0, st, s, f, ctx->tileClass.as<uint8_t>(), tilesX, tilesY);
                tileClass = ctx->tileClass.as<uint8_t>();
            }
            const int genMax = std::min(16, std::max(1, ctx->opt.genGroupMax)), genGroups = (B + genMax - 1) / genMax, genPer = (B + genGroups - 1) / genGroups;
            const dim3 genGrid = f.genPixelMajor ? dim3(genGroups, genWaves) : dim3(B, (genWaves + 15) / 16), genBlock = f.genPixelMajor ? dim3(64 * genPer) : dim3(1024);
            if (multiVer) hipLaunchKernelGGL((k_gen_primary<true>), genGrid, genBlock, 0, st, s, f, rays, tr, cull, activeList, activeCount, keysTmp, ctx->contFlag.as<uint8_t>(), tileClass, lean);
            else hipLaunchKernelGGL((k_gen_primary<false>), genGrid, genBlock, 0, st, s, f, rays, tr, cull, activeList, activeCount, keysTmp, ctx->contFlag.as<uint8_t>(), tileClass, lean);
            TRACE_T0();
            uint32_t grid0 = traceGrid;
            if (ctx->opt.gridRaysX4 > 0 && ctx->lastFast && ctx->lastBatch == B) grid0 = small_launch_grid(traceGrid, ctx->hCounts[MAX_DEPTH_SLOTS - 1], 2, ctx->opt.gridRaysX4, midGrid);
            if (fused) {
                hipLaunchKernelGGL((k_trace_fused<32>), dim3(grid0), dim3(WAVE), ldsBytes, st, s, f, rays, tr, hits, (const uint32_t*)activeList, (const uint32_t*)activeCount, work + 0, ctx->contFlag.as<uint8_t>(), keysTmp, lean);
            } else
            launch_trace2<true>(ctx, plan, grid0, st, s, f, rays, tr, hits, (const uint32_t*)activeList, (const uint32_t*)activeCount, work + 0, counters,
                                want_split(ctx, ctx->hCounts[MAX_DEPTH_SLOTS - 1], ctx->lastFast && ctx->lastBatch == B, B), 0);
            TRACE_T1();
            if (ctx->capturePrimary) { HIPC(ctx->primHit.ensure((size_t)N * 16)); hipLaunchKernelGGL(k_capture_primary, dim3((N + 255) / 256), dim3(256), 0, st, hits, (size_t)(B - 1) * Npad, N, ctx->primHit.as<float4>()); }
            if (fused) {}
            else {
                const bool sparseView = ctx->lastFast && ctx->lastBatch >= 1 && (uint64_t)ctx->hCounts[MAX_DEPTH_SLOTS - 1] * 2u < (uint64_t)ctx->W * ctx->rows * (uint64_t)ctx->lastBatch;
                pmBounce = f.genPixelMajor && (ctx->opt.bouncePixelMajor >= 2 || (ctx->opt.bouncePixelMajor == 1 && sparseView)) && depth >= 2 && !multiVer;
                if (pmBounce) { HIPC(ctx->pmList.ensure((size_t)total * 4)); pmList = ctx->pmList.as<uint32_t>(); }
                if (multiVer) hipLaunchKernelGGL((k_shade_first<true>), dim3(gridTotal), dim3(256), 0, st, s, f, rays, tr, hits, (const uint32_t*)activeList, (const uint32_t*)activeCount, ctx->contFlag.as<uint8_t>(), keysTmp, lean, (uint32_t*)nullptr, (uint32_t*)nullptr);
                else hipLaunchKernelGGL((k_shade_first<false>), dim3(gridTotal), dim3(256), 0, st, s, f, rays, tr, hits, (const uint32_t*)activeList, (const uint32_t*)activeCount, ctx->contFlag.as<uint8_t>(), keysTmp, lean, pmList, pmCount);
            }
            hipLaunchKernelGGL((k_scan_local<true>), dim3(scanBlocks), dim3(SCAN_WAVES_PER_BLOCK), 0, st, (const uint32_t*)nullptr, total, (const uint8_t*)ctx->contFlag.as<uint8_t>(), contMask, waveLocal, blockSums);
        } else {
            TRACE_T0();
            uint32_t g = std::min<uint32_t>(traceGrid, (N + 63) / 64);
            if (ctx->counters) { if (debug) hipLaunchKernelGGL((k_trace_primary<true, true>), dim3(g), dim3(WAVE), ldsBytes, st, s, f, rays, hits, N, work + 0, counters); else hipLaunchKernelGGL((k_trace_primary<true, false>), dim3(g), dim3(WAVE), ldsBytes, st, s, f, rays, hits, N, work + 0, counters); }
            else { if (debug) hipLaunchKernelGGL((k_trace_primary<false, true>), dim3(g), dim3(WAVE), ldsBytes, st, s, f, rays, hits, N, work + 0, counters); else hipLaunchKernelGGL((k_trace_primary<false, false>), dim3(g), dim3(WAVE), ldsBytes, st, s, f, rays, hits, N, work + 0, counters); }
            TRACE_T1();
            if (ctx->capturePrimary) { HIPC(ctx->primHit.ensure((size_t)N * 16)); hipLaunchKernelGGL(k_capture_primary, dim3((N + 255) / 256), dim3(256), 0, st, hits, (size_t)0, N, ctx->primHit.as<float4>()); }
            hipLaunchKernelGGL((k_shade<true, false>), dim3(gridTotal), dim3(256), 0, st, s, f, rays, trNone, hits, (const uint32_t*)nullptr, (const uint32_t*)nullptr, total, (const uint32_t*)nullptr, (const uint32_t*)nullptr,
                               contMask, waveCounts, keysTmp);
            hipLaunchKernelGGL((k_scan_local<false>), dim3(scanBlocks), dim3(SCAN_WAVES_PER_BLOCK), 0, st, (const uint32_t*)nullptr, total, (const uint8_t*)nullptr, contMask, waveLocal, blockSums);
        }
        hipLaunchKernelGGL(k_scan_blocks, dim3(1), dim3(1024), 0, st, (const uint32_t*)nullptr, total, blockSums, (const uint32_t*)waveLocal, counts + 1, (unsigned long long*)(1 < depth ? counters + 2 : nullptr),
                           (const unsigned long long*)contMask, (const uint32_t*)nullptr, Npad, B, bases + 1 * BS,
                           hostCounts + 1, hostBases + 1 * BS, (const uint32_t*)(counts + MAX_DEPTH_SLOTS - 1), hostCounts + MAX_DEPTH_SLOTS - 1);
        if (ctx->evBounce) HIPC(hipEventRecord(ctx->evBounce[1], st));
        hipLaunchKernelGGL((k_compact<true>), dim3(gridTotal), dim3(256), 0, st, (const uint32_t*)nullptr, (const uint32_t*)nullptr, total, (const unsigned long long*)contMask, (const uint32_t*)waveLocal, (const uint32_t*)blockSums,
                           (const uint32_t*)keysTmp, ctx->queue[1].as<uint32_t>(), ctx->keys[1].as<uint32_t>());
    }
    int side = 1;
    const bool deferLast = fast && depth >= 2 && ctx->opt.deferLast != 0 && !f.outputAovs && !debug;
    const bool deferAllHits = !(ctx->sceneNoEmission && !(f.g.DoTraceLights && s.lightCount > 0));
    for (int j = 1; j < depth; j++) {
        uint32_t* q = ctx->queue[side].as<uint32_t>(); uint32_t* k = ctx->keys[side].as<uint32_t>();
        const uint32_t* cnt = counts + j;
        f.hitsByRid = (fused || (pmBounce && j == 1)) ? 1 : 0;
        const uint32_t* gbase = nullptr;
        const bool bandExchange = (ctx->bandExchangeFn || ctx->bandExchangeDevFn) && ctx->rowMod > 1 && !(ctx->st.DoRaySorting && j > 1);
        if (bandExchange) {}
        else if (ctx->groupExchange) {
            int rc = ctx->groupExchange(ctx->groupUser, ctx, j, B, &gbase); if (rc) { ctx->pending.clear(); return rc; }
        } else if (ctx->exchangeFn) {
            std::vector<uint32_t> hb(B + 1), local(B), outBases(B, 0u);
            HIPC(hipMemcpyAsync(hb.data(), bases + j * BS, (size_t)(B + 1) * 4, hipMemcpyDeviceToHost, st));
            HIPC(hipStreamSynchronize(st));
            for (int b2 = 0; b2 < B; b2++) local[b2] = hb[b2 + 1] - hb[b2];
            ctx->exchangeFn(ctx->exchangeUser, j, B, local.data(), outBases.data());
            HIPC(ctx->gbases.ensure((size_t)MAX_BATCH * 4));
            HIPC(hipMemcpyAsync(ctx->gbases.p, outBases.data(), (size_t)B * 4, hipMemcpyHostToDevice, st));
            HIPC(hipStreamSynchronize(st));
            gbase = ctx->gbases.as<uint32_t>();
        }
        if (bandExchange) {
            const int bandRows = 1 << ctx->rowBandLog2, LB = (ctx->rows + bandRows - 1) / bandRows;
            HIPC(ctx->bandTab.ensure((size_t)4 * MAX_BATCH * ((size_t)LB + 1) * 4));
            uint32_t* dStarts = ctx->bandTab.as<uint32_t>(); uint32_t* dTab = dStarts + (size_t)MAX_BATCH * (LB + 1);
            hipLaunchKernelGGL(k_band_starts, dim3((uint32_t)(((size_t)B * (LB + 1) + 255) / 256)), dim3(256), 0, st, (const uint32_t*)q, (const uint32_t*)(bases + j * BS), B, LB, (uint32_t)ctx->W * (uint32_t)bandRows, Npad, dStarts);
            if (ctx->bandExchangeDevFn) {
                uint32_t* dCounts = dTab + (size_t)MAX_BATCH * (LB + 1); uint32_t* dBases = dCounts + (size_t)MAX_BATCH * (LB + 1);
                const uint32_t nb = (uint32_t)(((size_t)B * LB + 255) / 256);
                hipLaunchKernelGGL(k_band_counts, dim3(nb), dim3(256), 0, st, (const uint32_t*)dStarts, B, LB, dCounts);
                HIPC(hipGetLastError());
                ctx->bandExchangeDevFn(ctx->bandExchangeDevUser, j, B, LB, dCounts, dBases, (void*)st);
                hipLaunchKernelGGL(k_band_tab, dim3(nb), dim3(256), 0, st, (const uint32_t*)dStarts, (const uint32_t*)dBases, B, LB, dTab);
                gbase = dTab; f.gbStride = LB; f.gbBands = 1;
            } else {
            std::vector<uint32_t> starts((size_t)B * (LB + 1)), local((size_t)B * LB), outBases((size_t)B * LB, 0u), tab((size_t)B * LB);
            HIPC(hipMemcpyAsync(starts.data(), dStarts, starts.size() * 4, hipMemcpyDeviceToHost, st));
            HIPC(hipStreamSynchronize(st));
            for (int k2 = 0; k2 < B; k2++) for (int b2 = 0; b2 < LB; b2++) local[(size_t)k2 * LB + b2] = starts[(size_t)k2 * (LB + 1) + b2 + 1] - starts[(size_t)k2 * (LB + 1) + b2];
            ctx->bandExchangeFn(ctx->bandExchangeUser, j, B, LB, local.data(), outBases.data());
            for (int k2 = 0; k2 < B; k2++) for (int b2 = 0; b2 < LB; b2++) tab[(size_t)k2 * LB + b2] = outBases[(size_t)k2 * LB + b2] - starts[(size_t)k2 * (LB + 1) + b2];
            HIPC(hipMemcpyAsync(dTab, tab.data(), tab.size() * 4, hipMemcpyHostToDevice, st));
            HIPC(hipStreamSynchronize(st));
            gbase = dTab; f.gbStride = LB; f.gbBands = 1;
            }
        }
        if (!bandExchange) { f.gbStride = 1; f.gbBands = 0; }
        if (ctx->st.DoRaySorting && j > 1) {
            const uint32_t nTiles = (total + SORT_TILE - 1) / SORT_TILE;
            int sampleBits = 0; while ((1 << sampleBits) < B) sampleBits++;
            const int passes = (IDKPT_SORT_KEY_BITS + sampleBits + 6) / 7;
            uint32_t* digitTotals = ctx->sortHist.as<uint32_t>() + (size_t)SORT_RADIX * nTiles;
            uint32_t* ka = k; uint32_t* va = q; uint32_t* kb = ctx->sortKeys.as<uint32_t>(); uint32_t* vb = ctx->sortVals.as<uint32_t>();
            for (int pass = 0; pass < passes; pass++) {
                hipLaunchKernelGGL(k_sort_hist, dim3(nTiles), dim3(SORT_BLOCK), 0, st, (const uint32_t*)ka, cnt, (uint32_t)(7 * pass), ctx->sortHist.as<uint32_t>(), nTiles);
                hipLaunchKernelGGL(k_sort_scan, dim3(SORT_RADIX), dim3(1024), 0, st, cnt, ctx->sortHist.as<uint32_t>(), nTiles, digitTotals);
                hipLaunchKernelGGL(k_sort_scatter, dim3(nTiles), dim3(SORT_BLOCK), 0, st, (const uint32_t*)ka, (const uint32_t*)va, cnt, (uint32_t)(7 * pass), (const uint32_t*)ctx->sortHist.as<uint32_t>(), nTiles, (const uint32_t*)digitTotals, kb, vb);
                std::swap(ka, kb); std::swap(va, vb);
            }
            if (va != q) HIPC(hipMemcpyAsync(q, va, (size_t)total * 4, hipMemcpyDeviceToDevice, st));
        }
        if (!fused) {
        TRACE_T0();
        uint32_t gridj = traceGrid;
        const int hintMul = ctx->opt.gridHint;
        if (hintMul > 0 && ctx->lastBatch == B && ctx->hBases) gridj = small_launch_grid(traceGrid, ctx->hBases[(size_t)j * BS + B], hintMul, ctx->opt.gridRaysX4, midGrid);
        if (fast && pmBounce && j == 1) {
            Frame ft = f; ft.hitsByRid = 0;
            launch_trace2<true>(ctx, plan, gridj, st, s, ft, rays, tr, hits, (const uint32_t*)pmList, (const uint32_t*)pmCount, work + j, counters,
                                want_split(ctx, ctx->hBases ? ctx->hBases[(size_t)j * BS + B] : 0u, ctx->lastFast && ctx->lastBatch == B && ctx->hBases != nullptr, B), j);
        } else
        if (fast) launch_trace2<false>(ctx, plan, gridj, st, s, f, rays, tr, hits, (const uint32_t*)q, cnt, work + j, counters,
                                       want_split(ctx, ctx->hBases ? ctx->hBases[(size_t)j * BS + B] : 0u, ctx->lastFast && ctx->lastBatch == B && ctx->hBases != nullptr, B), j);
        else {
            if (ctx->counters) hipLaunchKernelGGL((k_trace_queue<true>), dim3(traceGrid), dim3(WAVE), ldsBytes, st, s, f, rays, hits, (const uint32_t*)q, cnt, work + j, counters);
            else hipLaunchKernelGGL((k_trace_queue<false>), dim3(traceGrid), dim3(WAVE), ldsBytes, st, s, f, rays, hits, (const uint32_t*)q, cnt, work + j, counters);
        }
        TRACE_T1();
        }
        if (deferLast && j == depth - 1 && gbase == nullptr) {
            HIPC(ctx->radSave.ensure((size_t)ctx->maxBatch * ctx->Npad * 16)); HIPC(ctx->deferCount.ensure(64));
#define SHADE_LAST(A, V) hipLaunchKernelGGL((k_shade_last<A, V>), dim3(gridTotal), dim3(256), 0, st, s, f, rays, hits, (const uint32_t*)q, cnt, (const uint32_t*)(bases + j * BS), ctx->radSave.as<float4>(), ctx->deferCount.as<uint32_t>())
            if (deferAllHits) { if (multiVer) SHADE_LAST(true, true); else SHADE_LAST(true, false); }
            else SHADE_LAST(false, false);
#undef SHADE_LAST
            ctx->defer.allHits = deferAllHits; ctx->defer.valid = true; ctx->defer.j = j; ctx->defer.side = side; ctx->defer.B = B; ctx->defer.total = total; ctx->defer.Npad = Npad;
            break;
        }
        if (multiVer) hipLaunchKernelGGL((k_shade<false, true>), dim3(gridTotal), dim3(256), 0, st, s, f, rays, fast ? tr : trNone, hits, (const uint32_t*)q, cnt, 0u, (const uint32_t*)(bases + j * BS), gbase, contMask, waveCounts, keysTmp);
        else hipLaunchKernelGGL((k_shade<false, false>), dim3(gridTotal), dim3(256), 0, st, s, f, rays, fast ? tr : trNone, hits, (const uint32_t*)q, cnt, 0u, (const uint32_t*)(bases + j * BS), gbase, contMask, waveCounts, keysTmp);
        hipLaunchKernelGGL((k_scan_local<false>), dim3(scanBlocks), dim3(SCAN_WAVES_PER_BLOCK), 0, st, cnt, 0u, (const uint8_t*)nullptr, contMask, waveLocal, blockSums);
        hipLaunchKernelGGL(k_scan_blocks, dim3(1), dim3(1024), 0, st, cnt, 0u, blockSums, (const uint32_t*)waveLocal, counts + j + 1, (unsigned long long*)(j + 1 < depth ? counters + 2 : nullptr),
                           (const unsigned long long*)contMask, (const uint32_t*)(bases + j * BS), Npad, B, bases + (j + 1) * BS,
                           hostCounts + j + 1, hostBases + (size_t)(j + 1) * BS, (const uint32_t*)nullptr, (uint32_t*)nullptr);
        if (ctx->evBounce) HIPC(hipEventRecord(ctx->evBounce[j + 1], st));
        hipLaunchKernelGGL((k_compact<false>), dim3(gridTotal), dim3(256), 0, st, (const uint32_t*)q, cnt, 0u, (const unsigned long long*)contMask, (const uint32_t*)waveLocal, (const uint32_t*)blockSums,
                           (const uint32_t*)keysTmp, ctx->queue[1 - side].as<uint32_t>(), ctx->keys[1 - side].as<uint32_t>());
        side = 1 - side;
    }
    ctx->lastQueueSide = side; ctx->lastQueueCountSlot = depth; ctx->lastFast = fast; ctx->lastNeedsRegen = fast; ctx->lastBatch = B; ctx->lastFrame = f;
    hipLaunchKernelGGL(k_final_draw, dim3((N + 255) / 256), dim3(256), 0, st, s, f, rays, image_ptr(ctx, 0, 0), image_ptr(ctx, 1, 0), image_ptr(ctx, 2, 0), N, tileClass,
                       work, (uint32_t)WORK_WORDS, counts, (uint32_t)MAX_DEPTH_SLOTS);
    HIPC(hipGetLastError());
    ctx->countersDirty = false;
#ifdef IDKPT_DEVELOPER
    if (capturing) {
        hipGraph_t g = nullptr; hipGraphExec_t ex = nullptr;
        const int K = ctx->opt.graphProbe; ctx->opt.graphProbe = 0;
        if (hipStreamEndCapture(st, &g) == hipSuccess && g && hipGraphInstantiate(&ex, g, nullptr, nullptr, 0) == hipSuccess) {
            hipEvent_t e0 = nullptr, e1 = nullptr; (void)hipEventCreate(&e0); (void)hipEventCreate(&e1);
            (void)hipGraphLaunch(ex, st); (void)hipStreamSynchronize(st);
            (void)hipEventRecord(e0, st);
            for (int k = 0; k < K; k++) (void)hipGraphLaunch(ex, st);
            (void)hipEventRecord(e1, st); (void)hipStreamSynchronize(st);
            float ms = 0.0f; (void)hipEventElapsedTime(&ms, e0, e1);
            size_t nodes = 0; (void)hipGraphGetNodes(g, nullptr, &nodes);
            fprintf(stderr, "[idkpt graph] batch of %d sample(s) captured: %zu graph nodes; %d replays: %.1f us per batch\n", B, nodes, K, ms * 1000.0f / (float)K);
            (void)hipEventDestroy(e0); (void)hipEventDestroy(e1); (void)hipGraphExecDestroy(ex);
        } else fprintf(stderr, "[idkpt graph] capture or instantiation failed: %s\n", hipGetErrorString(hipGetLastError()));
        if (g) (void)hipGraphDestroy(g);
    }
#endif
    if (ctx->timing) HIPC(hipEventRecord(ctx->evFrame[1], st));
    ctx->stats.Frames += (uint64_t)B;
    ctx->stats.PrimaryRays += (uint64_t)N * (uint64_t)B;
    ctx->pending.clear();
    return IDKPT_OK;
}

static int32_t dev_Render(dev_ctx* ctx)
{
    if (!ctx) return IDKPT_ERR_INVALID_ARGUMENT;
    if (!ctx->haveScene) return fail(ctx, IDKPT_ERR_INVALID_OPERATION, "idkptRender: no scene uploaded");
    if (ctx->W <= 0 || !ctx->frameOk) return fail(ctx, IDKPT_ERR_INVALID_OPERATION, "idkptRender: no frame buffers (idkptSetSize not called, or its allocation failed)");
    if (ctx->st.UseTlas && ctx->tlasCount == 0) return fail(ctx, IDKPT_ERR_INVALID_OPERATION, "idkptRender: UseTlas set but no TLAS nodes uploaded");
    HIPC(hipSetDevice(ctx->device));
    if (ctx->timing && ctx->evUsed > 4096) { HIPC(hipStreamSynchronize(ctx->stream)); resolve_trace_events(ctx); }
    const int limit = fast_path(ctx) ? ctx->maxBatch : 1;
    for (int i = 0; i < ctx->st.SamplesPerPixel; i++) {
        PendingSample ps; ps.accum = ctx->accum[ctx->curSlot]++; ps.slot = ctx->curSlot;
        memcpy(ps.cam, ctx->invProj, 64); memcpy(ps.cam + 16, ctx->invView, 64); memcpy(ps.cam + 32, ctx->viewPos, 12); ps.cam[35] = 0.0f;
        for (int b = 0; b < VB_COUNT; b++) ps.vs[b] = (uint8_t)ctx->vcur[b];
        ctx->pending.push_back(ps);
        if (!ctx->grouped && (int)ctx->pending.size() >= limit) { int rc = flush_batch(ctx); if (rc) return rc; }
    }
    return IDKPT_OK;
}

static int32_t dev_Synchronize(dev_ctx* ctx) { if (!ctx) return IDKPT_ERR_INVALID_ARGUMENT; HIPC(hipSetDevice(ctx->device)); FLUSH_KEEP(); SYNC_CHECKED(); return IDKPT_OK; }

static int32_t dev_Flush(dev_ctx* ctx) { if (!ctx) return IDKPT_ERR_INVALID_ARGUMENT; HIPC(hipSetDevice(ctx->device)); FLUSH_KEEP(); return IDKPT_OK; }

static int32_t dev_SetMaxBatch(dev_ctx* ctx, int32_t maxBatch)
{
    if (!ctx) return IDKPT_ERR_INVALID_ARGUMENT;
    REQUIRE(maxBatch >= 1 && maxBatch <= MAX_BATCH, "idkptSetMaxBatch: 1..256");
    HIPC(hipSetDevice(ctx->device));
    FLUSH();
    HIPC(hipStreamSynchronize(ctx->stream));
    if (maxBatch == ctx->maxBatch) return IDKPT_OK;
    const int previous = ctx->maxBatch;
    ctx->maxBatch = maxBatch;
    if (ctx->W > 0) {
        std::vector<uint32_t> acc = ctx->accum; int slot = ctx->curSlot; const bool started = ctx->ringStarted;
        int rc = alloc_frame_keep_images(ctx);
        if (rc) {
            const std::string why = ctx->lastError;
            ctx->maxBatch = previous;
            (void)alloc_frame(ctx);
            return fail(ctx, rc, "idkptSetMaxBatch: could not allocate the wavefront buffers for " + std::to_string(maxBatch) + " samples in flight (" + why + "); kept " + std::to_string(previous));
        }
        ctx->accum = acc; ctx->curSlot = slot; ctx->ringStarted = started;
// ... 46 lines not shown
```

### idkengine_amd/csrc/idkpt.hip

```cpp
#include <hip/hip_runtime.h>
#include <stdint.h>
#include <stdio.h>
#include <stdlib.h>
#include <string.h>
#include <string>
#include <vector>
#include <chrono>
#include <algorithm>
#include "../../include/idkpt.h"
#include "pt_kernels.hpp"

using namespace ptd;

#define WAVE 64
#define MAX_DEPTH_SLOTS 64
#define WORK_WORDS (GRAB_SLICES * GRAB_STRIDE)

#include "kernels_common.hpp"
#include "kernels_trace.hpp"
#include "kernels_wide.hpp"
#include "kernels_trace_inst.hpp"
#include "kernels_packet.hpp"
#include "kernels_trace_split.hpp"
#include "kernels_query.hpp"
#include "kernels_shade.hpp"
#include "kernels_trace_fused.hpp"
#include "kernels_queue.hpp"
#include "kernels_frame.hpp"
#include "kernels_scene.hpp"
#include "bvh_gpu.hpp"
#include "bvh_gpu_full.hpp"

#include "host_context.hpp"
#include "walk_plan.hpp"
#include "host_launch.hpp"
#include "host_frame.hpp"
#include "host_scene.hpp"
#include "host_builder.hpp"
#include "host_queries.hpp"
#include "host_schedule.hpp"
#include "host_readback.hpp"
#include "host_options.hpp"
#include "transport_rccl.hpp"

#include "idkpt_api.hpp"
```

### idkengine_amd/csrc/kernels_shade.hpp

```cpp
#pragma once

DEV void write_trace_ready(const DScene& s, const Frame& f, const TraceBufs& tr, uint32_t rid, const RayState& r)
{
    f3 rd = DecodeUnitVec(r.pdx, r.pdy);
    if (f.useTlas || s.instanceCount > 1) {
        tr.rec[4 * (size_t)rid] = make_float4(r.origin.x, r.origin.y, r.origin.z, 0.0f); tr.rec[4 * (size_t)rid + 1] = make_float4(rd.x, rd.y, rd.z, 0.0f);
        if (f.useTlas || f.instTlas) tr.rec[4 * (size_t)rid + 2] = make_float4(1.0f / rd.x, 1.0f / rd.y, 1.0f / rd.z, 0.0f);
        return;
    }
    GpuBlasInstance inst = s.instances[0];
    M34 inv = load_inv_model(s, inst.MeshTransformId);
    f3 lo = xform34(inv, r.origin, 1.0f), ld = xform34(inv, rd, 0.0f);
    const f3 iv = mk3(1.0f / ld.x, 1.0f / ld.y, 1.0f / ld.z);
    const float4* root = s.nodes + 2 * (size_t)s.descs[inst.BlasId].NodeOffset + 2;
    float t1;
    const float rootT = RayBoxIntersect(lo, iv, root[0], root[1], &t1) ? t1 : __builtin_inff();
    tr.rec[4 * (size_t)rid] = make_float4(lo.x, lo.y, lo.z, rootT); tr.rec[4 * (size_t)rid + 1] = make_float4(ld.x, ld.y, ld.z, 0.0f);
    tr.rec[4 * (size_t)rid + 2] = make_float4(iv.x, iv.y, iv.z, 0.0f);
}

template <bool VER >
__global__ __launch_bounds__(256) void k_shade_first(DScene s0, Frame f, RayBufs rays, TraceBufs tr, HitBufs hits, const uint32_t* activeList, const uint32_t* activeCount,
                                                     uint8_t* contFlag, uint32_t* seedsAndKeys, int lean ,
                                                     uint32_t* pmList , uint32_t* pmCount)
{
    __shared__ uint32_t waveCont[4]; __shared__ uint32_t blockBase;
    const uint32_t item = blockIdx.x * blockDim.x + threadIdx.x;
    const bool live = item < *activeCount;
    if (!pmList && !live) return;
    bool cont = false; uint32_t rid = 0;
    if (live) {
        rid = activeList[item];
        const uint32_t smp = rid / f.Npad, pix = rid - smp * f.Npad;
        const DScene s = VER ? scene_of_sample(s0, smp) : s0;
        const uint32_t acc = sample_index(f, smp);
        const HitRec hit = load_hit(hits, rid);
        RayState r; uint32_t rng, key = 0;
        if (lean) {
            f2 pd; gen_primary(f, smp, pix, acc, r.origin, pd, rng);
            r.prevIor = 1.0f; r.throughput = splat3(1.0f); r.pdx = pd.x; r.radiance = splat3(0.0f); r.pdy = pd.y;
        } else {
            float4 a = rays.o_ior[rid], b = rays.thr_px[rid], c = rays.rad_py[rid];
            r.origin = mk3(a.x, a.y, a.z); r.prevIor = a.w; r.throughput = mk3(b.x, b.y, b.z); r.pdx = b.w; r.radiance = mk3(c.x, c.y, c.z); r.pdy = c.w;
            rng = seedsAndKeys[rid];
        }
        AovState aov; aov.albedo = splat3(0.0f); aov.normal = splat3(0.0f); aov.newWeight = 1.0f;
        int lx = (int)(pix % (uint32_t)f.W), ly = (int)(pix / (uint32_t)f.W);
        uint32_t gidSeed = first_hit_gid_seed(f.W, f.H, lx, global_row(f, ly));
        f3 rd = DecodeUnitVec(r.pdx, r.pdy);
        cont = ShadeHit<true>(s, f, acc, hit, hit.T != PT_FLOAT_MAX, rd, r, aov, rng, gidSeed, key);
        rays.o_ior[rid] = make_float4(r.origin.x, r.origin.y, r.origin.z, r.prevIor);
        rays.thr_px[rid] = make_float4(r.throughput.x, r.throughput.y, r.throughput.z, r.pdx);
        rays.rad_py[rid] = make_float4(r.radiance.x, r.radiance.y, r.radiance.z, r.pdy);
        if (f.outputAovs) { rays.aovA[rid] = make_float4(aov.albedo.x, aov.albedo.y, aov.albedo.z, aov.newWeight); rays.aovN[rid] = make_float4(aov.normal.x, aov.normal.y, aov.normal.z, 0.0f); }
        seedsAndKeys[rid] = (key & ((1u << IDKPT_SORT_KEY_BITS) - 1u)) | (smp << IDKPT_SORT_KEY_BITS);
        if (cont) { contFlag[rid] = 1; write_trace_ready(s, f, tr, rid, r); }
    }
    if (pmList) {
        const unsigned long long m = __ballot(cont);
        const uint32_t wv = threadIdx.x >> 6, lane = threadIdx.x & 63;
        if (lane == 0) waveCont[wv] = (uint32_t)__popcll(m);
        __syncthreads();
        if (threadIdx.x == 0) { uint32_t tot = 0; for (int i = 0; i < 4; i++) { const uint32_t c = waveCont[i]; waveCont[i] = tot; tot += c; } blockBase = tot ? atomicAdd(pmCount, tot) : 0u; }
        __syncthreads();
        if (cont) pmList[blockBase + waveCont[wv] + (uint32_t)__popcll(m & ((1ull << lane) - 1ull))] = rid;
    }
}

template <bool FIRST, bool VER = false>
__global__ __launch_bounds__(256) void k_shade(DScene s0, Frame f, RayBufs rays, TraceBufs tr, HitBufs hits, const uint32_t* queue, const uint32_t* countPtr, uint32_t countImm,
                                               const uint32_t* qbase, const uint32_t* gbase , unsigned long long* contMask, uint32_t* waveCounts, uint32_t* keysTmp)
{
    const uint32_t N = FIRST ? countImm : *countPtr;
    const uint32_t slot = blockIdx.x * blockDim.x + threadIdx.x;
    if ((slot & ~63u) >= N) return;
    bool cont = false;
    uint32_t key = 0;
    bool inRange = slot < N;
    uint32_t smp = 0, pix = 0, idx = 0;
    if (inRange) {
        idx = FIRST ? slot : queue[slot];
        smp = idx / f.Npad; pix = idx - smp * f.Npad;
        if (FIRST && pix >= (uint32_t)f.W * (uint32_t)f.rows) inRange = false;
    }
    if (inRange) {
        const DScene s = VER ? scene_of_sample(s0, smp) : s0;
        const uint32_t acc = sample_index(f, smp);
        float4 a = rays.o_ior[idx], b = rays.thr_px[idx], c = rays.rad_py[idx];
        const HitRec hit = load_hit(hits, (!FIRST && f.hitsByRid) ? idx : slot);
        if (FIRST && f.g.DoDebugBVHTraversal) {
            rays.o_ior[idx] = make_float4(a.x, a.y, a.z, hits.cost[slot]);
        } else {
            RayState r; r.origin = mk3(a.x, a.y, a.z); r.prevIor = a.w; r.throughput = mk3(b.x, b.y, b.z); r.pdx = b.w; r.radiance = mk3(c.x, c.y, c.z); r.pdy = c.w;
            AovState aov; aov.albedo = splat3(0.0f); aov.normal = splat3(0.0f); aov.newWeight = 1.0f;
            if (!FIRST && f.outputAovs) { float4 aa = rays.aovA[idx], an = rays.aovN[idx]; aov.albedo = mk3(aa.x, aa.y, aa.z); aov.newWeight = aa.w; aov.normal = mk3(an.x, an.y, an.z); }
            uint32_t rng, gidSeed;
            if (FIRST) {
                f3 o2; f2 pd2; gen_primary(f, smp, pix, acc, o2, pd2, rng);
                int lx = (int)(pix % (uint32_t)f.W), ly = (int)(pix / (uint32_t)f.W);
                gidSeed = first_hit_gid_seed(f.W, f.H, lx, global_row(f, ly));
            } else {
                uint32_t gslot = (gbase ? gbase[f.gbBands ? smp * (uint32_t)f.gbStride + ((pix / (uint32_t)f.W) >> f.rowBandLog2) : smp] : 0u) + (slot - qbase[smp]);
                rng = gslot * 4096u + acc;
                gidSeed = gslot;
            }
            f3 rd = DecodeUnitVec(r.pdx, r.pdy);
            bool hitScene = hit.T != PT_FLOAT_MAX;
            cont = ShadeHit<FIRST>(s, f, acc, hit, hitScene, rd, r, aov, rng, gidSeed, key);
            rays.o_ior[idx] = make_float4(r.origin.x, r.origin.y, r.origin.z, r.prevIor);
            rays.thr_px[idx] = make_float4(r.throughput.x, r.throughput.y, r.throughput.z, r.pdx);
            rays.rad_py[idx] = make_float4(r.radiance.x, r.radiance.y, r.radiance.z, r.pdy);
            if (f.outputAovs) { rays.aovA[idx] = make_float4(aov.albedo.x, aov.albedo.y, aov.albedo.z, aov.newWeight); rays.aovN[idx] = make_float4(aov.normal.x, aov.normal.y, aov.normal.z, 0.0f); }
            if (cont && tr.rec) write_trace_ready(s, f, tr, idx, r);
        }
        keysTmp[slot] = (key & ((1u << IDKPT_SORT_KEY_BITS) - 1u)) | (smp << IDKPT_SORT_KEY_BITS);
    }
    unsigned long long m = __ballot(cont);
    if ((threadIdx.x & 63) == 0) contMask[slot >> 6] = m;
    (void)waveCounts;
}

template <bool ALL_HITS , bool VER = false>
__global__ __launch_bounds__(256) void k_shade_last(DScene s0, Frame f, RayBufs rays, HitBufs hits, const uint32_t* queue, const uint32_t* countPtr, const uint32_t* qbase,
                                                    float4* radSave, uint32_t* deferCount)
{
    const uint32_t N = *countPtr;
    const uint32_t slot = blockIdx.x * blockDim.x + threadIdx.x;
    if (slot == 0u) *deferCount = N;
    if (slot >= N) return;
    const uint32_t idx = queue[slot];
    const HitRec hit = load_hit(hits, f.hitsByRid ? idx : slot);
    const float4 b = rays.thr_px[idx];
    const bool miss = hit.T == PT_FLOAT_MAX;
    const bool odd = ALL_HITS || !(__builtin_isfinite(b.x) && __builtin_isfinite(b.y) && __builtin_isfinite(b.z));
    if (!miss && !odd) return;
    const float4 c = rays.rad_py[idx];
    radSave[slot] = c;
    if (miss) {
        const f3 albedo = SampleSky(s0, DecodeUnitVec(b.w, c.w));
        const f3 rad = mk3(c.x, c.y, c.z) + albedo * mk3(b.x, b.y, b.z);
        rays.rad_py[idx] = make_float4(rad.x, rad.y, rad.z, c.w);
    } else {
        const uint32_t smp = idx / f.Npad;
        const DScene s = VER ? scene_of_sample(s0, smp) : s0;
        const uint32_t acc = sample_index(f, smp);
        const float4 a = rays.o_ior[idx];
        RayState r; r.origin = mk3(a.x, a.y, a.z); r.prevIor = a.w; r.throughput = mk3(b.x, b.y, b.z); r.pdx = b.w; r.radiance = mk3(c.x, c.y, c.z); r.pdy = c.w;
        AovState aov; aov.albedo = splat3(0.0f); aov.normal = splat3(0.0f); aov.newWeight = 1.0f;
        const uint32_t gslot = slot - qbase[smp];
        uint32_t rng = gslot * 4096u + acc, key = 0;
        (void)ShadeHit<false, true>(s, f, acc, hit, true, DecodeUnitVec(b.w, c.w), r, aov, rng, gslot, key);
        rays.rad_py[idx] = make_float4(r.radiance.x, r.radiance.y, r.radiance.z, c.w);
    }
}
template <bool ALL_HITS>
__global__ __launch_bounds__(256) void k_restore_last(RayBufs rays, HitBufs hits, const uint32_t* queue, const uint32_t* countPtr, const float4* radSave, int hitsByRid)
{
    const uint32_t slot = blockIdx.x * blockDim.x + threadIdx.x;
    if (slot >= *countPtr) return;
    const uint32_t idx = queue[slot];
    const HitRec hit = load_hit(hits, hitsByRid ? idx : slot);
    const float4 b = rays.thr_px[idx];
    if (ALL_HITS || hit.T == PT_FLOAT_MAX || !(__builtin_isfinite(b.x) && __builtin_isfinite(b.y) && __builtin_isfinite(b.z))) rays.rad_py[idx] = radSave[slot];
}
```

### idkengine_amd/csrc/kernels_trace.hpp

```cpp
#pragma once

template <bool COUNT, bool COST>
__global__ __launch_bounds__(WAVE) void k_trace_primary(DScene s, Frame f, RayBufs rays, HitBufs hits, uint32_t N, uint32_t* workCounter, uint64_t* counters)
{
    extern __shared__ uint32_t lds[];
    const int lane = threadIdx.x;
    uint32_t* stk = lds + lane;
    uint32_t nPairs = 0, nTris = 0;
    while (true) {
        uint32_t base = wave_grab(workCounter, WAVE);
        if (base >= N) break;
        uint32_t pix = base + lane;
        if (pix < N) {
            f3 origin; f2 pd; uint32_t seed;
            gen_primary(f, 0u, pix, f.accumulated, origin, pd, seed);
            rays.o_ior[pix] = make_float4(origin.x, origin.y, origin.z, 1.0f);
            rays.thr_px[pix] = make_float4(1.0f, 1.0f, 1.0f, pd.x);
            rays.rad_py[pix] = make_float4(0.0f, 0.0f, 0.0f, pd.y);
            f3 rd = DecodeUnitVec(pd.x, pd.y);
            HitRec hit; float cost;
            TraceRay<COUNT, COST>(s, f, origin, rd, hit, cost, stk, WAVE, nPairs, nTris);
            store_hit(hits, pix, hit.T, hit.bx, hit.by, hit.tri, hit.xform);
            if (COST) hits.cost[pix] = cost;
        }
// ... 57 lines not shown
            pn[i] = n;
        }
        const f3 C = mk3(vp[0], vp[1], vp[2]);
        int nBoxes = s.instanceCount;
        uint32_t tlasChild = 0;
        const bool viaTlas = f.useTlas || f.instTlas;
        if (viaTlas) {
            nBoxes = 0;
            if (s.tlasCount > 0) { const uint32_t packed = __float_as_uint(s.tlas[0].w); if ((packed >> 31) == 0u) { nBoxes = 2; tlasChild = packed & 0x7fffffffu; } }
        }
        bool outside = nBoxes > 0;
        for (int ii = 0; ii < nBoxes && outside; ii++) {
            float4 bmin, bmax, m0 = make_float4(1.0f, 0.0f, 0.0f, 0.0f), m1 = make_float4(0.0f, 1.0f, 0.0f, 0.0f), m2 = make_float4(0.0f, 0.0f, 1.0f, 0.0f);
            if (viaTlas) { bmin = s.tlas[2 * (size_t)(tlasChild + ii)]; bmax = s.tlas[2 * (size_t)(tlasChild + ii) + 1]; }
            else {
                const GpuBlasInstance inst = s.instances[ii];
                const float4* root = s.nodes + 2 * (size_t)s.descs[inst.BlasId].NodeOffset + 2;
                bmin = root[0]; bmax = root[1];
                const float4* x = s.xforms + 9 * (size_t)inst.MeshTransformId;
                m0 = x[0]; m1 = x[1]; m2 = x[2];
            }
            f3 rel[8]; float D = 0.0f;
            for (int c = 0; c < 8; c++) {
                const float cx = (c & 1) ? bmax.x : bmin.x, cy = (c & 2) ? bmax.y : bmin.y, cz = (c & 4) ? bmax.z : bmin.z;
                rel[c] = mk3(m0.x * cx + m0.y * cy + m0.z * cz + m0.w, m1.x * cx + m1.y * cy + m1.z * cz + m1.w, m2.x * cx + m2.y * cy + m2.z * cz + m2.w) - C;
                D = gmax(D, gsqrt(dot(rel[c], rel[c])));
            }
            const float margin = r + (D + r) * (r / F) * 1.5f + 1e-4f * (D + 1.0f);
            bool boxOutside = false;
            for (int i = 0; i < 4; i++) {
                if (!planeOk[i]) continue;
                float dmin = PT_FLOAT_MAX;
                for (int c = 0; c < 8; c++) dmin = gmin(dmin, dot(pn[i], rel[c]));
                if (dmin > margin) boxOutside = true;
            }
            outside = boxOutside;
        }
        if (outside) {
            if (s.skySize <= 0) cls = 7;
            else if (s.skySize > 1) cls = 8;
            else {
                const float eta = 2.0f * (r / F) + 1e-4f;
                int face = -1; bool same = true;
                for (int i = 0; i < 4; i++) {
                    const float ax = gabs(u[i].x), ay = gabs(u[i].y), az = gabs(u[i].z);
                    int fc = -1;
                    if (ax >= gmax(ay, az) + eta) fc = u[i].x > 0.0f ? 0 : 1;
                    else if (ay >= gmax(ax, az) + eta) fc = u[i].y > 0.0f ? 2 : 3;
                    else if (az >= gmax(ax, ay) + eta) fc = u[i].z > 0.0f ? 4 : 5;
                    if (fc < 0 || (face >= 0 && fc != face)) same = false;
                    face = fc;
                }
                if (same && face >= 0) cls = (uint8_t)(1 + face);
            }
        }
    }
    tileClass[(size_t)smp * (tilesX * tilesY) + t] = cls;
}

template <bool VER>
__global__ __launch_bounds__(1024) void k_gen_primary(DScene s0, Frame f, RayBufs rays, TraceBufs tr, int cull, uint32_t* activeList, uint32_t* activeCount, uint32_t* seedOut, uint8_t* contFlag,
                                                     const uint8_t* tileClass ,
                                                     int lean )
{
    __shared__ uint32_t waveKeep[16]; __shared__ uint32_t blockBase; __shared__ unsigned long long keepMask[16];
    const bool pm = f.genPixelMajor != 0;
    const uint32_t G = blockDim.x >> 6;
    const uint32_t smp = pm ? blockIdx.x * G + (threadIdx.x >> 6) : blockIdx.x;
    const DScene s = VER ? scene_of_sample(s0, min(smp, (uint32_t)f.batch - 1u)) : s0;
    const uint32_t wave = pm ? blockIdx.y : (blockIdx.y * blockDim.x + threadIdx.x) >> 6, lane = threadIdx.x & 63;
    const uint32_t tilesX = ((uint32_t)f.W + 7) / 8;
    const uint32_t tx = wave % tilesX, ty = wave / tilesX;
    const uint32_t x = tx * 8 + (lane & 7), y = ty * 8 + (lane >> 3);
    const bool valid = x < (uint32_t)f.W && y < (uint32_t)f.rows && smp < (uint32_t)f.batch;
    const uint32_t pix = y * (uint32_t)f.W + x;
    const uint32_t rid = smp * f.Npad + pix;
    bool keep = false;
    const uint32_t nTilesAll = tilesX * (((uint32_t)f.rows + 7) / 8);
    const uint32_t cls = (tileClass && wave < nTilesAll) ? tileClass[(f.tilePerSample ? (size_t)min(smp, (uint32_t)f.batch - 1u) * nTilesAll : 0) + wave] : 0u;
    if (valid && cls != 0u) {
        contFlag[rid] = 4;
    } else if (valid) {
        f3 origin; f2 pd; uint32_t seed;
        gen_primary(f, smp, pix, sample_index(f, smp), origin, pd, seed);
        f3 rd = DecodeUnitVec(pd.x, pd.y);
        f3 lo = origin, ld = rd, invDir = splat3(0.0f);
        float rootT = __builtin_inff();
        keep = !cull;
        if (f.useTlas || f.instTlas) {
            invDir = mk3(1.0f / rd.x, 1.0f / rd.y, 1.0f / rd.z);
            if (cull) {
                if (s.tlasCount == 0) keep = false;
                else {
                    const uint32_t packed = __float_as_uint(s.tlas[0].w), id = packed & 0x7fffffffu;
                    if ((packed >> 31) == 1u) keep = true;
                    else {
                        float t1, t2;
                        const bool tl = RayBoxIntersect(origin, invDir, s.tlas[2 * (size_t)id], s.tlas[2 * (size_t)id + 1], &t1) && t1 < PT_FLOAT_MAX;
                        const bool tr2 = RayBoxIntersect(origin, invDir, s.tlas[2 * (size_t)id + 2], s.tlas[2 * (size_t)id + 3], &t2) && t2 < PT_FLOAT_MAX;
                        keep = tl || tr2;
                    }
                }
            }
        } else
        for (int ii = 0; ii < s.instanceCount && (ii == 0 || cull); ii++) {
            GpuBlasInstance inst = s.instances[ii];
            M34 inv = load_inv_model(s, inst.MeshTransformId);
            f3 l0 = xform34(inv, origin, 1.0f), l1 = xform34(inv, rd, 0.0f);
            f3 iv = mk3(1.0f / l1.x, 1.0f / l1.y, 1.0f / l1.z);
            if (s.instanceCount == 1) { lo = l0; ld = l1; invDir = iv; }
            if (cull || s.instanceCount == 1) {
                const float4* root = s.nodes + 2 * (size_t)s.descs[inst.BlasId].NodeOffset + 2;
                float t1;
                const bool boxHit = RayBoxIntersect(l0, iv, root[0], root[1], &t1);
                if (s.instanceCount == 1 && boxHit) rootT = t1;
                if (cull && boxHit && t1 < PT_FLOAT_MAX) keep = true;
            }
        }
        f3 radiance = splat3(0.0f);
        if (keep) {
            tr.rec[4 * (size_t)rid] = make_float4(lo.x, lo.y, lo.z, rootT); tr.rec[4 * (size_t)rid + 1] = make_float4(ld.x, ld.y, ld.z, 0.0f); tr.rec[4 * (size_t)rid + 2] = make_float4(invDir.x, invDir.y, invDir.z, 0.0f);
            if (!lean) seedOut[rid] = seed;
        } else {
            f3 albedo = SampleSky(s, rd);
            radiance = radiance + albedo * splat3(1.0f);
            if (f.outputAovs) { f3 fn = CubemapFaceNormal(rd); rays.aovA[rid] = make_float4(albedo.x, albedo.y, albedo.z, 0.0f); rays.aovN[rid] = make_float4(fn.x, fn.y, fn.z, 0.0f); }
        }
        if (keep && !lean) { rays.o_ior[rid] = make_float4(origin.x, origin.y, origin.z, 1.0f); rays.thr_px[rid] = make_float4(1.0f, 1.0f, 1.0f, pd.x); }
        contFlag[rid] = keep ? 0 : 2;
        if (!(keep && lean)) rays.rad_py[rid] = make_float4(radiance.x, radiance.y, radiance.z, pd.y);
    }
    const unsigned long long m = __ballot(keep);
    const uint32_t wv = threadIdx.x >> 6;
    if (pm) {
        if (cls != 0u) return;
        if (lane == 0) keepMask[wv] = m;
        __syncthreads();
        uint32_t cnt = 0, before = 0;
        for (uint32_t w = 0; w < G; w++) { const uint32_t b = (uint32_t)(keepMask[w] >> lane) & 1u; cnt += b; before += w < wv ? b : 0u; }
        uint32_t incl = cnt;
        for (int off = 1; off < 64; off <<= 1) { const uint32_t v = (uint32_t)__shfl_up((int)incl, off); incl += lane >= (uint32_t)off ? v : 0u; }
        const uint32_t tot = (uint32_t)__shfl((int)incl, 63);
        if (threadIdx.x == 0) blockBase = tot ? atomicAdd(activeCount, tot) : 0u;
        __syncthreads();
        if (keep) activeList[blockBase + (incl - cnt) + before] = rid;
        return;
    }
    if (lane == 0) waveKeep[wv] = (uint32_t)__popcll(m);
    __syncthreads();
    if (threadIdx.x == 0) { uint32_t tot = 0; for (int i = 0; i < 16; i++) { uint32_t c = waveKeep[i]; waveKeep[i] = tot; tot += c; } blockBase = tot ? atomicAdd(activeCount, tot) : 0u; }
    __syncthreads();
    if (keep) activeList[blockBase + waveKeep[wv] + (uint32_t)__popcll(m & ((1ull << lane) - 1ull))] = rid;
}

#define GRAB_SLICES 8u
#define GRAB_STRIDE 256u
template <bool PRIMARY, bool COUNT, int REFILL_MIN = 32, int OCC = 1, bool PROF = false, int LEAF_MIN = 24, int MODE = 0, int DBG = 0, bool VER = false, bool ANY = false, bool FAST = false>
__global__ __launch_bounds__(WAVE, OCC) void k_trace2(DScene s, Frame f, RayBufs rays, TraceBufs tr, HitBufs hits, const uint32_t* list, const uint32_t* countPtr, uint32_t* workCounter, uint64_t* counters)
{
    static_assert(MODE >= 0 && MODE <= 2 && (DBG == 0 || DBG == 16), "k_trace2: MODE 0-2, DBG 0 or 16 (pooled leaf phase)");
    static_assert(!FAST || (MODE == 0 && !COUNT && !VER && !ANY && !PROF), "k_trace2: FAST is the plain one-BLAS closest-hit walk");
    constexpr bool MULTI = MODE != 0, TLAS = MODE == 2;
    constexpr bool POOL = DBG == 16;
    extern __shared__ uint32_t lds[];
    const uint32_t lane = threadIdx.x;
    typedef __attribute__((address_space(3))) uint32_t lds_u32;
    lds_u32* const stkBase = (lds_u32*)lds + lane + (FAST ? WAVE : 0);
// ... 286 lines not shown
```

### idkengine_amd/csrc/pt_kernels.hpp

```cpp
#pragma once
#include "pt_device.hpp"

namespace ptd {

struct TexDesc { const void* data; int w, h; uint32_t state; uint32_t pad; };

struct DScene {
    const float4* nodes;
    const float4* pairNodes;
    const uint4* tris;
    const float4* triVerts;
    const GpuBlasDesc* descs;
    const GpuBlasInstance* instances; int instanceCount;
    const float4* tlas; int tlasCount;
    const float4* instRec;
    const uint4* vertices;
    const GpuMesh* meshes;
    const GpuMaterial* materials;
    const float4* xforms;
    const GpuLight* lights; int lightCount;
    const float4* sky; int skySize;
    const TexDesc* textures; int textureCount;
    const float* srgbLut;
    uint32_t* overflow;
    const uint32_t* ver;
};
#define SCENE_VER_WORDS 8
DEV DScene scene_of_sample(const DScene& s, uint32_t smp)
{
    DScene v = s;
    const uint32_t* t = s.ver + SCENE_VER_WORDS * (size_t)smp;
    v.nodes = s.nodes + t[0]; v.triVerts = s.triVerts + t[1]; v.vertices = s.vertices + t[2]; v.tlas = s.tlas + t[3]; v.xforms = s.xforms + t[4];
    return v;
}

struct Frame {
    float invProj[16]; float invView[16]; float viewPos[3];
    int W, H, rowMod, rowRem, rows;
    int rowBandLog2;
    GpuSettings g;
    uint32_t accumulated;
    int useTlas, stackCap, outputAovs;
    int tlasCap;
    int leafMin;
    uint32_t gridRaysX4, gridMid, gridMidRays;
    int grabUnitLog2, grabFixed;
    int batch; uint32_t Npad; uint32_t accum[256];
    uint32_t seqFirst, seqStride;
    const float* cams; uint32_t slotOf[256];
    int advMin;
    int poolMin;
    int splitPeek;
    int splitMode;
    int scatterLog2;
    int gbStride, gbBands;
    int queryMode;
    int shadeMin;
    int hitsByRid;
    int genPixelMajor;
    int instSieve;
    int instTlas;
    int packet;
    int tilePerSample;
};
#define MAX_BATCH 256

struct RayBufs {
    float4* o_ior;
    float4* thr_px;
    float4* rad_py;
    float4* aovA;
    float4* aovN;
};
struct TraceBufs {
    float4* rec;
    const uint32_t* order; const uint32_t* orderIdx;
};
struct HitBufs {
    float4* hit;
    float* cost;
};

struct HitRec { float T, bx, by; uint32_t tri, xform; };
DEV void store_hit(const HitBufs& h, size_t slot, float T, float bx, float by, uint32_t tri, uint32_t xform)
{
    h.hit[2 * slot] = make_float4(T, bx, by, __uint_as_float(tri));
    h.hit[2 * slot + 1] = make_float4(__uint_as_float(xform), 0.0f, 0.0f, 0.0f);
}
DEV HitRec load_hit(const HitBufs& h, size_t slot)
{
    const float4 a = h.hit[2 * slot]; const float x = h.hit[2 * slot + 1].x;
    HitRec r; r.T = a.x; r.bx = a.y; r.by = a.z; r.tri = __float_as_uint(a.w); r.xform = __float_as_uint(x);
    return r;
}

#define TLAS_STACK_SIZE 32

template <bool COUNT, bool COST>
DEV bool IntersectBlas(const DScene& s, f3 ro, f3 rd, const GpuBlasDesc& dref, bool useTlas, HitRec& hit, float& debugCost,
                       uint32_t* stk, int stride, int cap, uint32_t& nPairs, uint32_t& nTris)
{
    bool anyHit = false;
    float tMinLeft, tMinRight;
    f3 invDir = mk3(1.0f / rd.x, 1.0f / rd.y, 1.0f / rd.z);
    struct { int NodeOffset, TriangleOffset; } d = {dref.NodeOffset, dref.TriangleOffset};
    const float4* nodes = s.nodes + 2 * (size_t)d.NodeOffset;
// ... 132 lines not shown
            uint32_t first = intersectLeft ? lStart : rStart;
            uint32_t end = !intersectRight ? (lStart + lCount) : (rStart + rCount);
            first += (uint32_t)triOffset; end += (uint32_t)triOffset;
            for (uint32_t i = first; i < end; i++) {
                const float4* tv = s.triVerts + 3 * (size_t)i;
                float4 a = tv[0], b = tv[1], c = tv[2];
                float by, bz, t;
                if (RayTriangleIntersect(ro, rd, mk3(a.x, a.y, a.z), mk3(b.x, b.y, b.z), mk3(c.x, c.y, c.z), &by, &bz, &t) && t < hit.T) {
                    hit.tri = i; hit.bx = 1.0f - by - bz; hit.by = by; hit.T = t;
                    return true;
                }
            }
        }
        bool traverseLeft = hitLeft && lCount == 0, traverseRight = hitRight && rCount == 0;
        if (traverseLeft || traverseRight) {
            if (traverseLeft && traverseRight) { top = lStart; if (sp < cap) stk[sp * stride] = rStart; else *s.overflow = 1u; sp++; }
            else top = traverseLeft ? lStart : rStart;
        } else {
            if (sp == 0) break;
            sp--;
            if (sp >= cap) break;
            top = stk[sp * stride];
        }
    }
    return false;
}

DEV bool TraceRayAny(const DScene& s, const Frame& f, f3 ro, f3 rd, HitRec& hit, uint32_t* stk, int stride, bool traceLights, float maxDist)
{
    hit.T = maxDist; hit.tri = ~0u; hit.xform = 0; hit.bx = 0.0f; hit.by = 0.0f;
    if (traceLights) {
        for (int i = 0; i < s.lightCount; i++) {
            const GpuLight& l = s.lights[i];
            float tMin, tMax;
            if (RaySphereIntersect(ro, rd, mk3(l.Position[0], l.Position[1], l.Position[2]), l.Radius, &tMin, &tMax) && tMin < hit.T) {
                hit.T = tMin < 0.0f ? tMax : tMin; hit.xform = (uint32_t)i;
                return true;
            }
        }
    }
    if (f.useTlas) {
        if (s.tlasCount == 0) return false;
        uint32_t* tstk = stk + f.stackCap * stride;
        float tMinLeft, tMinRight;
        f3 invDir = mk3(1.0f / rd.x, 1.0f / rd.y, 1.0f / rd.z);
        int sp = 0; uint32_t top = 0;
        while (true) {
            float4 pmin = s.tlas[2 * (size_t)top];
            uint32_t packed = __float_as_uint(pmin.w);
            bool isLeaf = (packed >> 31) == 1;
            uint32_t id = packed & 0x7fffffffu;
            if (isLeaf) {
                GpuBlasInstance inst = s.instances[id];
                M34 inv = load_inv_model(s, inst.MeshTransformId);
                f3 lo = xform34(inv, ro, 1.0f), ld = xform34(inv, rd, 0.0f);
                if (IntersectBlasAny(s, lo, ld, s.descs[inst.BlasId], true, hit, stk, stride, f.stackCap)) { hit.xform = inst.MeshTransformId; return true; }
                if (sp == 0 || sp > f.tlasCap) break;
                top = tstk[--sp * stride];
                continue;
            }
            uint32_t l = id, r = id + 1;
            float4 lmin = s.tlas[2 * (size_t)l], lmax = s.tlas[2 * (size_t)l + 1], rmin = s.tlas[2 * (size_t)r], rmax = s.tlas[2 * (size_t)r + 1];
            bool tl = RayBoxIntersect(ro, invDir, lmin, lmax, &tMinLeft) && tMinLeft < hit.T;
            bool tr = RayBoxIntersect(ro, invDir, rmin, rmax, &tMinRight) && tMinRight < hit.T;
            if (tl || tr) {
                if (tl && tr) { bool lc = tMinLeft < tMinRight; top = lc ? l : r; if (sp < f.tlasCap) tstk[sp * stride] = lc ? r : l; else *s.overflow = 1u; sp++; }
                else top = tl ? l : r;
            } else { if (sp == 0 || sp > f.tlasCap) break; top = tstk[--sp * stride]; }
        }
    } else {
        for (int i = 0; i < s.instanceCount; i++) {
            GpuBlasInstance inst = s.instances[i];
            M34 inv = load_inv_model(s, inst.MeshTransformId);
            f3 lo = xform34(inv, ro, 1.0f), ld = xform34(inv, rd, 0.0f);
            if (IntersectBlasAny(s, lo, ld, s.descs[inst.BlasId], false, hit, stk, stride, f.stackCap)) { hit.xform = inst.MeshTransformId; return true; }
        }
    }
    return false;
}

DEV int global_row(const Frame& f, int ly) { return ((((ly >> f.rowBandLog2) * f.rowMod + f.rowRem) << f.rowBandLog2) | (ly & ((1 << f.rowBandLog2) - 1))); }

DEV uint32_t sample_index(const Frame& f, uint32_t smp) { return f.seqFirst + f.accum[smp] * f.seqStride; }
DEV void gen_primary(const Frame& f, uint32_t smp, uint32_t pix, uint32_t acc, f3& origin, f2& packedDir, uint32_t& rngSeed)
{
    const float* cam = f.cams ? f.cams + 36u * smp : f.invProj;
    const float* invProj = cam; const float* invView = cam + 16; const float* vp = cam + 32;
    int lx = (int)(pix % (uint32_t)f.W), ly = (int)(pix / (uint32_t)f.W);
    int y = global_row(f, ly), x = lx;
    uint32_t seed = (uint32_t)(y * 4096 + x) * (acc + 1u);
    float ox = rnd01(seed), oy = rnd01(seed);
    float nx = ((float)x + ox) / (float)f.W * 2.0f - 1.0f, ny = ((float)y + oy) / (float)f.H * 2.0f - 1.0f;
    f3 camDir = GetWorldSpaceDirection(invProj, invView, nx, ny);
    f3 viewPos = mk3(vp[0], vp[1], vp[2]);
    f3 focalPoint = viewPos + camDir * f.g.FocalLength;
    f2 disk = SampleDisk(seed);
    f3 pointOnLense = mat4_mul_xyz(invView, f.g.LenseRadius * disk.x, f.g.LenseRadius * disk.y, 0.0f, 1.0f);
    camDir = normalize(focalPoint - pointOnLense);
    origin = pointOnLense;
    packedDir = EncodeUnitVec(camDir);
    rngSeed = seed;
}

DEV uint32_t first_hit_gid_seed(int W, int H, int px, int py)
{
    const uint32_t n = 20;
    uint32_t numX = (uint32_t)(W + 7) / 8, numY = (uint32_t)(H + 7) / 8;
    uint32_t sx = (uint32_t)px / 8, sy = (uint32_t)py / 8;
    uint32_t columnSize = numY * n, fullColumnCount = numX / n, lastColumnWidth = numX % n;
    uint32_t columnIdx = sx / n;
    uint32_t columnWidth = (columnIdx == fullColumnCount) ? lastColumnWidth : n;
    uint32_t idxInColumn = sy * columnWidth + (sx - columnIdx * n);
    uint32_t idx = columnIdx * columnSize + idxInColumn;
    uint32_t wgY = idx / numX, wgX = idx % numX;
    uint32_t gx = wgX * 8 + (uint32_t)px % 8, gy = wgY * 8 + (uint32_t)py % 8;
    return gy * 4096u + gx;
}

DEV int tex_wrap(int i, int n, uint32_t mode)
{
    if (mode == 1u) return i < 0 ? 0 : (i > n - 1 ? n - 1 : i);
    if (mode == 2u) { int m = i % (2 * n); if (m < 0) m += 2 * n; const int a = m - n; return (n - 1) - (a >= 0 ? a : -(1 + a)); }
    int k = i % n; if (k < 0) k += n; return k;
}
DEV float4 tex_fetch(const DScene& s, const TexDesc& t, int x, int y)
{
    const uint32_t fmt = t.state >> 5;
    const size_t at = (size_t)y * (size_t)t.w + (size_t)x;
    if (fmt == 0u) return ((const float4*)t.data)[at];
    const uint32_t p = ((const uint32_t*)t.data)[at];
    const float a = (float)(p >> 24) / 255.0f;
    if (fmt == 1u) return make_float4((float)(p & 255u) / 255.0f, (float)((p >> 8) & 255u) / 255.0f, (float)((p >> 16) & 255u) / 255.0f, a);
    return make_float4(s.srgbLut[p & 255u], s.srgbLut[(p >> 8) & 255u], s.srgbLut[(p >> 16) & 255u], a);
}
DEV float4 SampleTex(const DScene& s, uint64_t handle, float u, float v)
{
    if (handle == 0 || handle > (uint64_t)s.textureCount) return make_float4(1.0f, 1.0f, 1.0f, 1.0f);
    const TexDesc t = s.textures[handle - 1];
    if (t.w == 1 && t.h == 1) return tex_fetch(s, t, 0, 0);
    const uint32_t ws = t.state & 3u, wt = (t.state >> 2) & 3u;
    if ((t.state >> 4) & 1u) {
        const int x = tex_wrap((int)gfloor(u * (float)t.w), t.w, ws), y = tex_wrap((int)gfloor(v * (float)t.h), t.h, wt);
        return tex_fetch(s, t, x, y);
    }
    float fx = u * (float)t.w - 0.5f, fy = v * (float)t.h - 0.5f;
    float x0f = gfloor(fx), y0f = gfloor(fy);
    float ax = fx - x0f, ay = fy - y0f;
    const int x0 = tex_wrap((int)x0f, t.w, ws), x1 = tex_wrap((int)(x0f + 1.0f), t.w, ws), y0 = tex_wrap((int)y0f, t.h, wt), y1 = tex_wrap((int)(y0f + 1.0f), t.h, wt);
    const float4 a = tex_fetch(s, t, x0, y0), b = tex_fetch(s, t, x1, y0), c = tex_fetch(s, t, x0, y1), d = tex_fetch(s, t, x1, y1);
    return make_float4(gmix(gmix(a.x, b.x, ax), gmix(c.x, d.x, ax), ay), gmix(gmix(a.y, b.y, ax), gmix(c.y, d.y, ax), ay),
                       gmix(gmix(a.z, b.z, ax), gmix(c.z, d.z, ax), ay), gmix(gmix(a.w, b.w, ax), gmix(c.w, d.w, ax), ay));
}
DEV void SkyFold(int S, int& face, int& x, int& y)
{
    int sc = 2 * x + 1 - S, tc = 2 * y + 1 - S;
    int px, py, pz;
    switch (face) {
        case 0: px = S; py = -tc; pz = -sc; break;
        case 1: px = -S; py = -tc; pz = sc; break;
        case 2: py = S; px = sc; pz = tc; break;
        case 3: py = -S; px = sc; pz = -tc; break;
        case 4: pz = S; px = sc; py = -tc; break;
        default: pz = -S; px = -sc; py = -tc; break;
    }
    const int m = face >> 1;
    const bool ox = m != 0 && (px > S || px < -S), oy = m != 1 && (py > S || py < -S), oz = m != 2 && (pz > S || pz < -S);
    if (!(ox || oy || oz)) return;
    const int in = S - 1;
    if (m == 0) px = px > 0 ? in : -in; else if (m == 1) py = py > 0 ? in : -in; else pz = pz > 0 ? in : -in;
    if (oz) { pz = pz > 0 ? S : -S; face = pz > 0 ? 4 : 5; }
    else if (oy) { py = py > 0 ? S : -S; face = py > 0 ? 2 : 3; }
    else { px = px > 0 ? S : -S; face = px > 0 ? 0 : 1; }
    switch (face) {
        case 0: sc = -pz; tc = -py; break;
        case 1: sc = pz; tc = -py; break;
        case 2: sc = px; tc = pz; break;
        case 3: sc = px; tc = -pz; break;
        case 4: sc = px; tc = -py; break;
        default: sc = -px; tc = -py; break;
    }
    x = (sc + S - 1) / 2; y = (tc + S - 1) / 2;
}
DEV f3 SampleSky(const DScene& s, f3 d)
{
    if (s.skySize <= 0) return splat3(0.0f);
    float ax = gabs(d.x), ay = gabs(d.y), az = gabs(d.z);
    int face; float sc, tc, ma;
    if (ax >= ay && ax >= az) { face = d.x >= 0.0f ? 0 : 1; sc = d.x >= 0.0f ? -d.z : d.z; tc = -d.y; ma = ax; }
    else if (ay >= az) { face = d.y >= 0.0f ? 2 : 3; sc = d.x; tc = d.y >= 0.0f ? d.z : -d.z; ma = ay; }
    else { face = d.z >= 0.0f ? 4 : 5; sc = d.z >= 0.0f ? d.x : -d.x; tc = -d.y; ma = az; }
    const int S = s.skySize;
    if (S == 1) { float4 p = s.sky[face]; return mk3(p.x, p.y, p.z); }
    float u = 0.5f * (sc / ma + 1.0f), v = 0.5f * (tc / ma + 1.0f);
    float fx = u * (float)S - 0.5f, fy = v * (float)S - 0.5f;
    float x0f = gfloor(fx), y0f = gfloor(fy);
    float wx = fx - x0f, wy = fy - y0f;
    const int x0 = (int)gmin(gmax(x0f, -1.0f), (float)(S - 1)), y0 = (int)gmin(gmax(y0f, -1.0f), (float)(S - 1));
    f3 t[4]; bool corner[4]; bool anyCorner = false;
#pragma unroll
    for (int k = 0; k < 4; k++) {
        int x = x0 + (k & 1), y = y0 + (k >> 1), f2 = face;
        corner[k] = (x < 0 || x >= S) && (y < 0 || y >= S);
        t[k] = splat3(0.0f);
        if (corner[k]) { anyCorner = true; continue; }
        SkyFold(S, f2, x, y);
        float4 p = s.sky[((size_t)f2 * S + y) * S + x];
        t[k] = mk3(p.x, p.y, p.z);
    }
    if (anyCorner) {
        f3 sum = splat3(0.0f);
#pragma unroll
        for (int k = 0; k < 4; k++) if (!corner[k]) sum = sum + t[k];
        const f3 mean = mk3(sum.x / 3.0f, sum.y / 3.0f, sum.z / 3.0f);
#pragma unroll
        for (int k = 0; k < 4; k++) if (corner[k]) t[k] = mean;
    }
    return mk3(gmix(gmix(t[0].x, t[1].x, wx), gmix(t[2].x, t[3].x, wx), wy),
               gmix(gmix(t[0].y, t[1].y, wx), gmix(t[2].y, t[3].y, wx), wy),
               gmix(gmix(t[0].z, t[1].z, wx), gmix(t[2].z, t[3].z, wx), wy));
}

struct RayState { f3 origin; float prevIor; f3 throughput; float pdx; f3 radiance; float pdy; };
struct AovState { f3 albedo; float newWeight; f3 normal; };

template <bool FIRST, bool RAD_ONLY = false>
DEV bool ShadeHit(const DScene& s, const Frame& f, uint32_t acc, const HitRec& hit, bool hitScene, f3 rayDir, RayState& r, AovState& aov, uint32_t& rng, uint32_t gidSeed, uint32_t& sortingKey)
{
    if (hitScene) {
        r.origin = r.origin + rayDir * hit.T;
        f3 sAlbedo = splat3(1.0f), sNormal = splat3(0.0f), sEmissive = splat3(0.0f), sAbsorbance = splat3(0.0f);
        float sAlpha = 1.0f, sMetallic = 0.0f, sRoughness = 0.0f, sTransmission = 0.0f, sIOR = 1.5f, sAlphaCutoff = 0.5f;
        bool sIsVolumetric = false, sTint = true;
        f3 geometricNormal = splat3(0.0f);
        bool hitLight = hit.tri == ~0u;
        if (!hitLight) {
            sortingKey = hit.tri;
            uint4 tri = s.tris[hit.tri];
            uint4 v0 = s.vertices[tri.x], v1 = s.vertices[tri.y], v2 = s.vertices[tri.z];
            f3 bary = mk3(hit.bx, hit.by, 1.0f - hit.bx - hit.by);
            float u = __uint_as_float(v0.x) * bary.x + __uint_as_float(v1.x) * bary.y + __uint_as_float(v2.x) * bary.z;
            float v = __uint_as_float(v0.y) * bary.x + __uint_as_float(v1.y) * bary.y + __uint_as_float(v2.y) * bary.z;
            f3 interpNormal = normalize(Interpolate(DecompressSR11G11B10(v0.w), DecompressSR11G11B10(v1.w), DecompressSR11G11B10(v2.w), bary));
            f3 interpTangent = normalize(Interpolate(DecompressSR11G11B10(v0.z), DecompressSR11G11B10(v1.z), DecompressSR11G11B10(v2.z), bary));
            M34 inv = load_inv_model(s, hit.xform);
            const GpuMesh& mesh = s.meshes[tri.w];
            const GpuMaterial& mat = s.materials[mesh.MaterialId];
            {
                uint32_t bcf = mat.BaseColorFactor;
                float4 bc = SampleTex(s, mat.BaseColorTexture, u, v);
                sAlbedo = mk3(bc.x * ((float)(bcf & 255u) / 255.0f), bc.y * ((float)((bcf >> 8) & 255u) / 255.0f), bc.z * ((float)((bcf >> 16) & 255u) / 255.0f));
                sAlpha = bc.w * ((float)((bcf >> 24) & 255u) / 255.0f);
                float4 nm = SampleTex(s, mat.NormalTexture, u, v);
                sNormal = mk3(nm.x * 2.0f - 1.0f, nm.y * 2.0f - 1.0f, gsqrt(gmax(1.0f - (nm.x * nm.x + nm.y * nm.y), 0.0f)));
                float4 em = SampleTex(s, mat.EmissiveTexture, u, v);
                sEmissive = mk3(em.x * mat.EmissiveFactor[0], em.y * mat.EmissiveFactor[1], em.z * mat.EmissiveFactor[2]);
                sAbsorbance = mk3(mat.Absorbance[0], mat.Absorbance[1], mat.Absorbance[2]);
                float4 mr = SampleTex(s, mat.MetallicRoughnessTexture, u, v);
                sMetallic = mr.x * mat.MetallicFactor; sRoughness = mr.y * mat.RoughnessFactor;
                float4 tr = SampleTex(s, mat.TransmissionTexture, u, v);
                sTransmission = tr.x * mat.TransmissionFactor; sIOR = mat.IOR;
                sAlphaCutoff = mat.AlphaCutoff; sIsVolumetric = mat.IsVolumetric != 0;
            }
            {
                sEmissive = sEmissive * 1.0f + mesh.EmissiveBias * sAlbedo;
                sAbsorbance = mk3(gmax(sAbsorbance.x + mesh.AbsorbanceBias[0], 0.0f), gmax(sAbsorbance.y + mesh.AbsorbanceBias[1], 0.0f), gmax(sAbsorbance.z + mesh.AbsorbanceBias[2], 0.0f));
                sMetallic = gclamp(sMetallic + mesh.SpecularBias, 0.0f, 1.0f);
                sRoughness = gclamp(sRoughness + mesh.RoughnessBias, 0.0f, 1.0f);
                sTransmission = gclamp(sTransmission + mesh.TransmissionBias, 0.0f, 1.0f);
                sIOR = gmax(sIOR + mesh.IORBias, 1.0f);
                sTint = mesh.TintOnTransmissive != 0;
            }
            float alphaCutoff = (sAlphaCutoff == 2.0f) ? rnd01(rng) : sAlphaCutoff;
            if (sAlpha < alphaCutoff) { r.origin = r.origin + rayDir * 0.001f; return true; }
            f3 worldNormal = normalize(xform34_transposed3(inv, interpNormal));
            f3 worldTangent = normalize(xform34_transposed3(inv, interpTangent));
            f3 N = normalize(worldNormal), T = normalize(worldTangent), B = normalize(cross(N, T));
            f3 tn = mk3((T.x * sNormal.x + B.x * sNormal.y) + N.x * sNormal.z, (T.y * sNormal.x + B.y * sNormal.y) + N.y * sNormal.z, (T.z * sNormal.x + B.z * sNormal.y) + N.z * sNormal.z);
            sNormal = normalize(gmix(worldNormal, tn, mesh.NormalMapStrength));
            const float4* tv = s.triVerts + 3 * (size_t)hit.tri;
            float4 a = tv[0], b = tv[1], c = tv[2];
            f3 p0 = mk3(a.x, a.y, a.z), p1 = mk3(b.x, b.y, b.z), p2 = mk3(c.x, c.y, c.z);
            geometricNormal = normalize(cross(p1 - p0, p2 - p0));
            geometricNormal = normalize(xform34_transposed3(inv, geometricNormal));
        } else if (f.g.DoTraceLights) {
            sortingKey = hit.xform;
            const GpuLight& l = s.lights[hit.xform];
            sEmissive = mk3(l.Color[0], l.Color[1], l.Color[2]); sAlbedo = sEmissive;
            sNormal = (r.origin - mk3(l.Position[0], l.Position[1], l.Position[2])) / l.Radius;
            geometricNormal = sNormal;
        }
        float prevIor = FIRST ? 1.0f : r.prevIor;
        bool fromInside = dot(-rayDir, geometricNormal) < 0.0f;
        if (fromInside) {
            if (FIRST) prevIor = sIOR;
            geometricNormal = geometricNormal * -1.0f;
            if (sIsVolumetric) {
                f3 e = (-sAbsorbance) * hit.T;
                r.throughput = r.throughput * mk3(gexp(e.x), gexp(e.y), gexp(e.z));
            }
        }
        float cosTheta = dot(-rayDir, sNormal);
        if (cosTheta < 0.0f) { sNormal = sNormal * -1.0f; }
        r.radiance = r.radiance + sEmissive * r.throughput;
        if (RAD_ONLY) return false;

        float roughness2 = sRoughness * sRoughness;
        float metallic, transmission;
        {
            float ct = dot(-rayDir, sNormal);
            float diffuseChance = 1.0f - sMetallic - sTransmission;
            float f0 = BaseReflectivity(prevIor, sIOR);
            metallic = gmix(sMetallic, 1.0f, FresnelSchlick(f0, 1.0f, ct));
            transmission = gmax(1.0f - diffuseChance - metallic, 0.0f);
        }
        uint32_t bsdfType;
        {
            float rnd = rnd01(rng);
            if (metallic > rnd) bsdfType = 1u;
            else if (metallic + transmission > rnd) bsdfType = 2u;
            else bsdfType = 0u;
        }
        f3 diffuseRayDir;
        {
            uint32_t local = gidSeed;
            f2 r2 = R2Sequence(acc);
            float px = rnd01(local), py = rnd01(local);
            f2 uv; uv.x = gfract(r2.x + px); uv.y = gfract(r2.y + py);
            diffuseRayDir = CosineSampleHemisphere(sNormal, uv);
        }
        f3 newDir, bsdf; float pdf, newIor;
        if (bsdfType == 0u) { newDir = diffuseRayDir; newIor = prevIor; bsdf = sAlbedo; pdf = 1.0f; }
        else if (bsdfType == 1u) {
            f3 refl = reflect(rayDir, sNormal);
            newDir = normalize(gmix(refl, diffuseRayDir, roughness2));
            bsdf = sAlbedo; pdf = 1.0f; newIor = prevIor;
        } else {
            newIor = fromInside ? 1.0f : sIOR;
            f3 refr; bool tir;
            if (!sIsVolumetric) { refr = rayDir; tir = false; newIor = 1.0f; }
            else {
                refr = refract(rayDir, sNormal, prevIor / newIor);
                tir = (refr.x == 0.0f && refr.y == 0.0f && refr.z == 0.0f);
                if (tir) { refr = reflect(rayDir, sNormal); newIor = prevIor; }
            }
            newDir = normalize(gmix(refr, !tir ? -diffuseRayDir : diffuseRayDir, roughness2));
            bool gltfWantsTint = sIsVolumetric || !fromInside;
            bsdf = (gltfWantsTint && sTint) ? sAlbedo : splat3(1.0f);
            pdf = 1.0f;
        }
        pdf = gmax(pdf, 0.0001f);
        r.throughput = r.throughput * (bsdf / pdf);
        {
            float diffuseC = 1.0f - sMetallic - sTransmission;
            float weight = diffuseC + sMetallic * sRoughness + sTransmission * sRoughness;
            if (FIRST) { aov.albedo = sAlbedo * weight; aov.normal = sNormal * weight; aov.newWeight = 1.0f - weight; }
            else { aov.albedo = aov.albedo + aov.newWeight * sAlbedo * weight; aov.normal = aov.normal + aov.newWeight * sNormal * weight; aov.newWeight *= (1.0f - weight); }
        }
        if (!FIRST) {
            if (f.g.DoRussianRoulette) {
                float p = gmax(r.throughput.x, gmax(r.throughput.y, r.throughput.z));
                if (rnd01(rng) > p) return false;
                r.throughput = r.throughput / p;
            }
        }
// ... 19 lines not shown
```

### idkengine_amd/pathtracer.py

```python
import ctypes as C
import os
import numpy as np
from . import _lib
from . import gputypes as T
from ._lib import IdkPtError


_OPTION_NAMES = ("force_generic", "no_tile_cull", "no_lean_primary", "leaf_min", "grab_unit_log2", "grab_fixed", "lds_pad", "trace_waves", "grid_hint", "grid_rays_x4", "grid_mid_waves", "defer_last", "split", "split_donor", "split_peek", "group_threads", "query_scheduler", "split_scatter", "fused", "fused_shade_min", "leaf_pool", "pool_min", "adv_min",
                 "wide", "wide_cap", "wide_count", "packet", "packet_min_live", "packet_waves", "inst_tlas", "inst_tlas_overlap", "inst_braid", "inst_unify", "inst_unify_radius", "uni_refill", "inst_general", "pair_nodes", "inst_sieve", "inst_sieve_overlap", "gen_pixel_major", "gen_group_max", "bounce_pixel_major", "transport", "bvh_timing", "bvh_small", "bvh_stackopt_host", "force_no_peer", "trace_variant")


class PathTracer:
    def __init__(self, width, height, settings=None, device=0, row_modulo=1, row_remainder=0, devices=None, row_band=1):
        self._L = _lib.load()
        n = C.c_int32(0)
        self._L.idkptGetDeviceCount(C.byref(n))
        if n.value <= 0:
            raise IdkPtError("no HIP device visible: the path tracer has no CPU fallback")
        ctx = C.c_void_p()
        ids = list(devices) if devices else [device]
        self.device_count = len(ids)
        if self.device_count > 1 and (row_modulo, row_remainder) != (1, 0):
            raise IdkPtError("a multi-device context deals its rows itself")
        dev = (C.c_int32 * len(ids))(*ids)
        rc = self._L.idkptCreate(len(ids), dev, C.byref(ctx))
        if rc != 0:
            raise IdkPtError(f"idkptCreate failed with status {rc}")
        self._ctx = ctx
        for name in _OPTION_NAMES:
            v = os.environ.get("IDKPT_" + name.upper())
            if v is not None and v != "":
                self.set_option(name, int(v))
        self._settings = settings if settings is not None else T.Settings.default()
        self._cached_ray_depth = self._settings.RayDepth
        self._scene = None
        self.width, self.height = width, height
        self.row_modulo, self.row_remainder, self.row_band = row_modulo, row_remainder, (int(row_band) if row_modulo > 1 else 1)
        self._row_limit = None
        if self.device_count == 1:
            if self.row_band > 1:
                self._check(self._L.idkptSetRowBands(ctx, self.row_band, row_modulo, row_remainder))
            else:
                self._check(self._L.idkptSetRowSharding(ctx, row_modulo, row_remainder))
        self._check(self._L.idkptSetSize(ctx, width, height))
        self._push_settings()

    def _check(self, rc):
        err = getattr(self, "_callback_error", None)
        if err is not None:
            self._callback_error = None
            raise err
        if rc != 0:
            msg = C.c_char_p()
            self._L.idkptGetLastError(self._ctx, C.byref(msg))
            raise IdkPtError(f"idkpt status {rc}: {(msg.value or b'').decode()}")

    def _push_settings(self):
        self._check(self._L.idkptSetSettings(self._ctx, C.addressof(self._settings)))

    def global_rows(self):
        b = self.row_band
        ys = [y for y in range(self.height) if (y // b) % self.row_modulo == self.row_remainder] if self.row_modulo > 1 else list(range(self.row_remainder, self.height))
        return ys if self._row_limit is None else ys[:self._row_limit]

    @property
    def rows(self):
        return len(self.global_rows())

    def _prop(name, gpu=False):
        def get(self):
            return getattr(self._settings.Gpu if gpu else self._settings, name)

        def set_(self, v):
            setattr(self._settings.Gpu if gpu else self._settings, name, type(get(self))(v))
            self._push_settings()
        return property(get, set_)

    SamplesPerPixel = _prop("SamplesPerPixel")
    RayDepth = _prop("RayDepth")
    FocalLength = _prop("FocalLength", gpu=True)
    LenseRadius = _prop("LenseRadius", gpu=True)
    DoTraceLights = _prop("DoTraceLights", gpu=True)
    DoRussianRoulette = _prop("DoRussianRoulette", gpu=True)
    DoRaySorting = _prop("DoRaySorting")
    OutputAOVs = _prop("OutputAOVs")
    UseTlas = _prop("UseTlas")
    BlasStackSize = _prop("BlasStackSize")

    @property
    def DoDebugBVHTraversal(self):
        return self._settings.Gpu.DoDebugBVHTraversal == 1

# ... 297 lines not shown
```

Baseline: 7675.

## Add plain-material shading path that skips texture sampling for untextured scenes

Precomputes a per-material view on the host (decoded base color factor plus no-texture and volumetric flags). When every material in the scene is untextured and non-volumetric, the shade kernels are instantiated with a PLAIN flag that skips all five texture samples and volumetric absorption, and hoists the triangle-vertex and inverse-model loads earlier. The general path can also skip sampling per material based on the flag. Unorm conversions are swapped for a lookup table. The cost is extra kernel instantiations, host-side table rebuilds whenever materials are uploaded, and a new expect_shade developer check.

```diff
diff --git a/idkengine_amd/csrc/host_context.hpp b/idkengine_amd/csrc/host_context.hpp
--- a/idkengine_amd/csrc/host_context.hpp
+++ b/idkengine_amd/csrc/host_context.hpp
@@ -77,6 +77,11 @@
     DevBuf nodes, tris, triVerts, descs, instances, tlas, parents, leaves, positions, prevPositions, vertices, meshes, materials, xforms, lights, sky, texDescs, unskinned, joints, levelNodes, tlasScratch, queryIn, queryOut, queryRec, queryList, tileClass, gbases;
     std::vector<DevBuf> texData; std::vector<std::pair<int, int>> texDims; std::vector<uint32_t> texState;
     DevBuf srgbLut;
+    DevBuf unormLut, matView;
+    std::vector<GpuMaterial> hMaterials;
+    std::vector<float> hUnorm;
+    int expectShade = 0;
+    bool scenePlain = false;
     std::vector<GpuBlasDesc> hDescs;
     std::vector<std::vector<uint32_t>> levelOffsets;
     std::vector<uint32_t> levelBase;
@@ -112,7 +117,7 @@
     uint32_t* hCounts = nullptr; uint32_t* dCountsMirror = nullptr;
     bool sceneNested = false;
     bool sceneNoEmission = false;
-    struct { bool valid = false, allHits = false; int j = 0, side = 0, B = 0; uint32_t total = 0, Npad = 0; } defer;
+    struct { bool valid = false, allHits = false, plain = false; int j = 0, side = 0, B = 0; uint32_t total = 0, Npad = 0; } defer;
     DevBuf radSave, deferCount;
     bool countersDirty = true;
     uint32_t* hOverflow = nullptr; uint32_t* dOverflow = nullptr;
diff --git a/idkengine_amd/csrc/host_options.hpp b/idkengine_amd/csrc/host_options.hpp
--- a/idkengine_amd/csrc/host_options.hpp
+++ b/idkengine_amd/csrc/host_options.hpp
@@ -29,6 +29,7 @@
     else if (n == "fused_shade_min") o.fusedShadeMin = std::min(64, std::max(1, value));
     else if (n == "leaf_pool") { REQUIRE(value >= -1 && value <= 7, "idkptSetDeveloperOption: leaf_pool is -1 (automatic) or a mask 0..7 (1: primary launches, 2: the first bounce, 4: later bounces)"); o.leafPool = value; }
     else if (n == "pool_min") o.poolMin = std::max(0, value);
+    else if (n == "expect_shade") { REQUIRE(value >= 0 && value <= 2, "idkptSetDeveloperOption: expect_shade is 0 (off), 1 (plain) or 2 (general)"); ctx->expectShade = value; }
     else if (n == "adv_min") o.advMin = std::min(64, std::max(0, value));
 #ifdef IDKPT_DEVELOPER
     else if (n == "graph_probe") o.graphProbe = std::max(0, value);
diff --git a/idkengine_amd/csrc/host_scene.hpp b/idkengine_amd/csrc/host_scene.hpp
--- a/idkengine_amd/csrc/host_scene.hpp
+++ b/idkengine_amd/csrc/host_scene.hpp
@@ -110,7 +110,7 @@
     (void)hipSetDevice(ctx->device);
     ctx->pending.clear();
     (void)hipStreamSynchronize(ctx->stream);
-    DevBuf* all[] = {&ctx->srgbLut, &ctx->pmList, &ctx->pairNodes, &ctx->instRec, &ctx->entRec, &ctx->braidBuf, &ctx->unodes, &ctx->utlas, &ctx->uTabs, &ctx->uniBuf, &ctx->uniEntRec, &ctx->itlas, &ctx->imarks, &ctx->ichunks, &ctx->wnodes, &ctx->wleaf, &ctx->wids, &ctx->wpair, &ctx->wcounts, &ctx->wtotals, &ctx->nodes, &ctx->tris, &ctx->triVerts, &ctx->descs, &ctx->instances, &ctx->tlas, &ctx->parents, &ctx->leaves, &ctx->positions, &ctx->prevPositions, &ctx->vertices, &ctx->meshes,
+    DevBuf* all[] = {&ctx->srgbLut, &ctx->unormLut, &ctx->matView, &ctx->pmList, &ctx->pairNodes, &ctx->instRec, &ctx->entRec, &ctx->braidBuf, &ctx->unodes, &ctx->utlas, &ctx->uTabs, &ctx->uniBuf, &ctx->uniEntRec, &ctx->itlas, &ctx->imarks, &ctx->ichunks, &ctx->wnodes, &ctx->wleaf, &ctx->wids, &ctx->wpair, &ctx->wcounts, &ctx->wtotals, &ctx->nodes, &ctx->tris, &ctx->triVerts, &ctx->descs, &ctx->instances, &ctx->tlas, &ctx->parents, &ctx->leaves, &ctx->positions, &ctx->prevPositions, &ctx->vertices, &ctx->meshes,
                      &ctx->materials, &ctx->xforms, &ctx->lights, &ctx->sky, &ctx->texDescs, &ctx->unskinned, &ctx->joints, &ctx->levelNodes, &ctx->tlasScratch, &ctx->queryIn, &ctx->queryOut, &ctx->queryRec, &ctx->queryList, &ctx->bandTab, &ctx->tileClass, &ctx->gbases, &ctx->camTab, &ctx->verTab, &ctx->trRec, &ctx->contFlag, &ctx->blockSums, &ctx->rayO, &ctx->rayT, &ctx->rayR, &ctx->aovA, &ctx->aovN, &ctx->hit,
                      &ctx->hitCost, &ctx->primHit, &ctx->queue[0], &ctx->queue[1], &ctx->keys[0], &ctx->keys[1], &ctx->keysTmp, &ctx->sortKeys, &ctx->sortVals, &ctx->contMask, &ctx->waveCounts,
                      &ctx->counts, &ctx->work, &ctx->qwork, &ctx->radSave, &ctx->deferCount, &ctx->sortHist, &ctx->counters64, &ctx->bases, &ctx->img[0], &ctx->img[1], &ctx->img[2]};
@@ -286,6 +286,20 @@
     for (int b = 0; b < 256; b++) { const double cs = (double)b / 255.0; lut[b] = (float)(cs <= 0.04045 ? cs / 12.92 : pow((cs + 0.055) / 1.055, 2.4)); }
     HIPC(ctx->srgbLut.ensure(sizeof(lut)));
     HIPC(hipMemcpy(ctx->srgbLut.p, lut, sizeof(lut), hipMemcpyHostToDevice));
+    return IDKPT_OK;
+}
+static int shade_tables_rebuild(dev_ctx* ctx)
+{
+    if (ctx->hUnorm.empty()) { ctx->hUnorm.resize(256); shade::fill_unorm_lut(ctx->hUnorm.data()); }
+    if (!ctx->unormLut.p) {
+        HIPC(ctx->unormLut.ensure(256 * sizeof(float)));
+        HIPC(hipMemcpy(ctx->unormLut.p, ctx->hUnorm.data(), 256 * sizeof(float), hipMemcpyHostToDevice));
+    }
+    std::vector<shade::MatView> views(ctx->hMaterials.size());
+    for (size_t i = 0; i < views.size(); i++) views[i] = shade::mat_view(ctx->hMaterials[i], ctx->textureCount, ctx->hUnorm.data());
+    ctx->scenePlain = shade::scene_plain(views.data(), (int)views.size());
+    { int rc = upload(ctx, ctx->matView, views.data(), views.size() * sizeof(shade::MatView)); if (rc) return rc; }
+    HIPC(hipStreamSynchronize(ctx->stream));
     return IDKPT_OK;
 }
 static int tex_descs_upload(dev_ctx* ctx)
@@ -378,6 +392,8 @@
     ctx->nodeCount = sc->BlasNodeCount; ctx->triCount = sc->BlasTriangleCount; ctx->instanceCount = sc->BlasInstanceCount; ctx->tlasCount = sc->TlasNodes ? sc->TlasNodeCount : 0;
     ctx->vertexCount = sc->VertexCount; ctx->meshCount = sc->MeshCount; ctx->materialCount = sc->MaterialCount; ctx->xformCount = sc->MeshTransformCount;
     ctx->lightCount = sc->Lights ? sc->LightCount : 0; ctx->textureCount = sc->TextureCount;
+    ctx->hMaterials.assign(sc->Materials, sc->Materials + sc->MaterialCount);
+    if ((rc = shade_tables_rebuild(ctx))) return rc;
     ctx->hDescs.assign(sc->BlasDescs, sc->BlasDescs + sc->BlasDescCount); ctx->hInst0Blas = (int)sc->BlasInstances[0].BlasId;
     ctx->hInstances.assign(sc->BlasInstances, sc->BlasInstances + sc->BlasInstanceCount);
     ctx->hXforms.assign((const char*)sc->MeshTransforms, (const char*)sc->MeshTransforms + (size_t)sc->MeshTransformCount * sizeof(GpuMeshTransform));
@@ -472,6 +488,8 @@
     ctx->meshCount = src->meshCount; ctx->materialCount = src->materialCount; ctx->xformCount = src->xformCount; ctx->lightCount = src->lightCount; ctx->skySize = src->skySize;
     ctx->textureCount = src->textureCount; ctx->hDescs = src->hDescs; ctx->hInstances = src->hInstances; ctx->hXforms = src->hXforms; ctx->hInst0Blas = src->hInst0Blas; ctx->sceneNoEmission = src->sceneNoEmission; ctx->sceneNested = src->sceneNested; ctx->sceneStack = src->sceneStack; ctx->tlasNeed = src->tlasNeed;
     ctx->levelOffsets = src->levelOffsets; ctx->levelBase = src->levelBase; ctx->refitCoversAll = src->refitCoversAll;
+    ctx->hMaterials = src->hMaterials;
+    { int rc = shade_tables_rebuild(ctx); if (rc) return rc; }
     ver_reset(ctx);
     { int rc = ver_reserve(ctx); if (rc) return rc; }
     HIPC(hipStreamSynchronize(ctx->stream));
@@ -568,6 +586,10 @@
     if (vb >= 0) { char* src; int rc = ver_writable(ctx, vb, offsetBytes == 0 && bytes == cap, &src, &dst); if (rc) return rc; }
     { int rc = staged_upload(ctx, dst + offsetBytes, data, bytes); if (rc) return rc; }
     if (which == IDKPT_BUF_MESH_TRANSFORMS && offsetBytes + bytes <= ctx->hXforms.size()) memcpy(ctx->hXforms.data() + offsetBytes, data, bytes);
+    if (which == IDKPT_BUF_MATERIALS) {
+        memcpy((char*)ctx->hMaterials.data() + offsetBytes, data, bytes);
+        int rc = shade_tables_rebuild(ctx); if (rc) return rc;
+    }
     if (which == IDKPT_BUF_VERTEX_POSITIONS) { int rc = regather_triverts(ctx, 0, (uint32_t)ctx->triCount); if (rc) return rc; }
     return IDKPT_OK;
 }
diff --git a/idkengine_amd/csrc/host_schedule.hpp b/idkengine_amd/csrc/host_schedule.hpp
--- a/idkengine_amd/csrc/host_schedule.hpp
+++ b/idkengine_amd/csrc/host_schedule.hpp
@@ -12,12 +12,15 @@
     s.meshes = ctx->meshes.as<GpuMesh>(); s.materials = ctx->materials.as<GpuMaterial>(); s.xforms = (const float4*)at(VB_XFORMS);
     s.lights = ctx->lights.as<GpuLight>(); s.lightCount = ctx->lightCount; s.sky = ctx->sky.as<float4>(); s.skySize = ctx->skySize;
     s.textures = ctx->texDescs.as<TexDesc>(); s.textureCount = ctx->textureCount; s.srgbLut = ctx->srgbLut.as<float>();
+    s.unormLut = ctx->unormLut.as<float>(); s.matView = ctx->matView.as<float4>();
     s.overflow = ctx->dOverflow;
     s.ver = multi ? ctx->verTab.as<uint32_t>() : nullptr;
     return s;
 }
 static DScene make_dscene(dev_ctx* ctx) { return make_dscene(ctx, nullptr, false); }
 static DScene make_dscene_last(dev_ctx* ctx) { return make_dscene(ctx, ctx->lastSlots, ctx->lastMulti); }
+
+static bool shade_plain(const dev_ctx* ctx, bool multiVer) { return ctx->scenePlain && !multiVer; }
 
 static float4* image_ptr(dev_ctx* ctx, int i, int slot) { return ctx->img[i].as<float4>() + (size_t)slot * ((size_t)ctx->W * ctx->rows); }
 
@@ -70,6 +73,7 @@
     if (ctx->defer.allHits) hipLaunchKernelGGL((k_restore_last<true>), dim3(gridTotal), dim3(256), 0, st, rays, hits, q, cnt, (const float4*)ctx->radSave.as<float4>(), f.hitsByRid);
     else hipLaunchKernelGGL((k_restore_last<false>), dim3(gridTotal), dim3(256), 0, st, rays, hits, q, cnt, (const float4*)ctx->radSave.as<float4>(), f.hitsByRid);
     if (multiVer) hipLaunchKernelGGL((k_shade<false, true>), dim3(gridTotal), dim3(256), 0, st, s, f, rays, tr, hits, q, cnt, 0u, (const uint32_t*)(bases + j * BS), (const uint32_t*)nullptr, contMask, waveLocal, keysTmp);
+    else if (ctx->defer.plain) hipLaunchKernelGGL((k_shade<false, false, true>), dim3(gridTotal), dim3(256), 0, st, s, f, rays, tr, hits, q, cnt, 0u, (const uint32_t*)(bases + j * BS), (const uint32_t*)nullptr, contMask, waveLocal, keysTmp);
     else hipLaunchKernelGGL((k_shade<false, false>), dim3(gridTotal), dim3(256), 0, st, s, f, rays, tr, hits, q, cnt, 0u, (const uint32_t*)(bases + j * BS), (const uint32_t*)nullptr, contMask, waveLocal, keysTmp);
     hipLaunchKernelGGL((k_scan_local<false>), dim3(scanBlocks), dim3(SCAN_WAVES_PER_BLOCK), 0, st, cnt, 0u, (const uint8_t*)nullptr, contMask, waveLocal, blockSums);
     hipLaunchKernelGGL(k_scan_blocks, dim3(1), dim3(1024), 0, st, cnt, 0u, blockSums, (const uint32_t*)waveLocal, counts + j + 1, (unsigned long long*)nullptr,
@@ -178,6 +182,8 @@
     const int BS = MAX_BATCH + 1;
 
     const uint8_t* tileClass = nullptr;
+    const bool plainShade = shade_plain(ctx, multiVer);
+    if (ctx->expectShade && plainShade != (ctx->expectShade == 1)) { ctx->pending.clear(); return fail(ctx, IDKPT_ERR_INVALID_OPERATION, plainShade ? "expect_shade: this batch takes the plain shading kernels" : "expect_shade: this batch takes the general shading kernels"); }
     uint32_t* activeList = ctx->sortVals.as<uint32_t>();
     uint32_t* activeCount = counts + (MAX_DEPTH_SLOTS - 1);
     uint32_t* pmList = nullptr; uint32_t* const pmCount = counts + (MAX_DEPTH_SLOTS - 2); bool pmBounce = false;
@@ -223,6 +229,7 @@
                 pmBounce = f.genPixelMajor && (ctx->opt.bouncePixelMajor >= 2 || (ctx->opt.bouncePixelMajor == 1 && sparseView)) && depth >= 2 && !multiVer;
                 if (pmBounce) { HIPC(ctx->pmList.ensure((size_t)total * 4)); pmList = ctx->pmList.as<uint32_t>(); }
                 if (multiVer) hipLaunchKernelGGL((k_shade_first<true>), dim3(gridTotal), dim3(256), 0, st, s, f, rays, tr, hits, (const uint32_t*)activeList, (const uint32_t*)activeCount, ctx->contFlag.as<uint8_t>(), keysTmp, lean, (uint32_t*)nullptr, (uint32_t*)nullptr);
+                else if (plainShade) hipLaunchKernelGGL((k_shade_first<false, true>), dim3(gridTotal), dim3(256), 0, st, s, f, rays, tr, hits, (const uint32_t*)activeList, (const uint32_t*)activeCount, ctx->contFlag.as<uint8_t>(), keysTmp, lean, pmList, pmCount);
                 else hipLaunchKernelGGL((k_shade_first<false>), dim3(gridTotal), dim3(256), 0, st, s, f, rays, tr, hits, (const uint32_t*)activeList, (const uint32_t*)activeCount, ctx->contFlag.as<uint8_t>(), keysTmp, lean, pmList, pmCount);
             }
             hipLaunchKernelGGL((k_scan_local<true>), dim3(scanBlocks), dim3(SCAN_WAVES_PER_BLOCK), 0, st, (const uint32_t*)nullptr, total, (const uint8_t*)ctx->contFlag.as<uint8_t>(), contMask, waveLocal, blockSums);
@@ -327,14 +334,16 @@
         }
         if (deferLast && j == depth - 1 && gbase == nullptr) {
             HIPC(ctx->radSave.ensure((size_t)ctx->maxBatch * ctx->Npad * 16)); HIPC(ctx->deferCount.ensure(64));
-#define SHADE_LAST(A, V) hipLaunchKernelGGL((k_shade_last<A, V>), dim3(gridTotal), dim3(256), 0, st, s, f, rays, hits, (const uint32_t*)q, cnt, (const uint32_t*)(bases + j * BS), ctx->radSave.as<float4>(), ctx->deferCount.as<uint32_t>())
-            if (deferAllHits) { if (multiVer) SHADE_LAST(true, true); else SHADE_LAST(true, false); }
-            else SHADE_LAST(false, false);
+#define SHADE_LAST(A, V, P) hipLaunchKernelGGL((k_shade_last<A, V, P>), dim3(gridTotal), dim3(256), 0, st, s, f, rays, hits, (const uint32_t*)q, cnt, (const uint32_t*)(bases + j * BS), ctx->radSave.as<float4>(), ctx->deferCount.as<uint32_t>())
+            if (deferAllHits) { if (multiVer) SHADE_LAST(true, true, false); else if (plainShade) SHADE_LAST(true, false, true); else SHADE_LAST(true, false, false); }
+            else if (plainShade) SHADE_LAST(false, false, true);
+            else SHADE_LAST(false, false, false);
 #undef SHADE_LAST
-            ctx->defer.allHits = deferAllHits; ctx->defer.valid = true; ctx->defer.j = j; ctx->defer.side = side; ctx->defer.B = B; ctx->defer.total = total; ctx->defer.Npad = Npad;
+            ctx->defer.allHits = deferAllHits; ctx->defer.plain = plainShade; ctx->defer.valid = true; ctx->defer.j = j; ctx->defer.side = side; ctx->defer.B = B; ctx->defer.total = total; ctx->defer.Npad = Npad;
             break;
         }
         if (multiVer) hipLaunchKernelGGL((k_shade<false, true>), dim3(gridTotal), dim3(256), 0, st, s, f, rays, fast ? tr : trNone, hits, (const uint32_t*)q, cnt, 0u, (const uint32_t*)(bases + j * BS), gbase, contMask, waveCounts, keysTmp);
+        else if (plainShade) hipLaunchKernelGGL((k_shade<false, false, true>), dim3(gridTotal), dim3(256), 0, st, s, f, rays, fast ? tr : trNone, hits, (const uint32_t*)q, cnt, 0u, (const uint32_t*)(bases + j * BS), gbase, contMask, waveCounts, keysTmp);
         else hipLaunchKernelGGL((k_shade<false, false>), dim3(gridTotal), dim3(256), 0, st, s, f, rays, fast ? tr : trNone, hits, (const uint32_t*)q, cnt, 0u, (const uint32_t*)(bases + j * BS), gbase, contMask, waveCounts, keysTmp);
         hipLaunchKernelGGL((k_scan_local<false>), dim3(scanBlocks), dim3(SCAN_WAVES_PER_BLOCK), 0, st, cnt, 0u, (const uint8_t*)nullptr, contMask, waveLocal, blockSums);
         hipLaunchKernelGGL(k_scan_blocks, dim3(1), dim3(1024), 0, st, cnt, 0u, blockSums, (const uint32_t*)waveLocal, counts + j + 1, (unsigned long long*)(j + 1 < depth ? counters + 2 : nullptr),
diff --git a/idkengine_amd/csrc/idkpt.hip b/idkengine_amd/csrc/idkpt.hip
--- a/idkengine_amd/csrc/idkpt.hip
+++ b/idkengine_amd/csrc/idkpt.hip
@@ -33,6 +33,7 @@
 
 #include "host_context.hpp"
 #include "walk_plan.hpp"
+#include "shade_tables.hpp"
 #include "host_launch.hpp"
 #include "host_frame.hpp"
 #include "host_scene.hpp"
diff --git a/idkengine_amd/csrc/kernels_shade.hpp b/idkengine_amd/csrc/kernels_shade.hpp
--- a/idkengine_amd/csrc/kernels_shade.hpp
+++ b/idkengine_amd/csrc/kernels_shade.hpp
@@ -19,7 +19,7 @@
     tr.rec[4 * (size_t)rid + 2] = make_float4(iv.x, iv.y, iv.z, 0.0f);
 }
 
-template <bool VER >
+template <bool VER , bool PLAIN = false>
 __global__ __launch_bounds__(256) void k_shade_first(DScene s0, Frame f, RayBufs rays, TraceBufs tr, HitBufs hits, const uint32_t* activeList, const uint32_t* activeCount,
                                                      uint8_t* contFlag, uint32_t* seedsAndKeys, int lean ,
                                                      uint32_t* pmList , uint32_t* pmCount)
@@ -48,7 +48,7 @@
         int lx = (int)(pix % (uint32_t)f.W), ly = (int)(pix / (uint32_t)f.W);
         uint32_t gidSeed = first_hit_gid_seed(f.W, f.H, lx, global_row(f, ly));
         f3 rd = DecodeUnitVec(r.pdx, r.pdy);
-        cont = ShadeHit<true>(s, f, acc, hit, hit.T != PT_FLOAT_MAX, rd, r, aov, rng, gidSeed, key);
+        cont = ShadeHit<true, false, PLAIN>(s, f, acc, hit, hit.T != PT_FLOAT_MAX, rd, r, aov, rng, gidSeed, key);
         rays.o_ior[rid] = make_float4(r.origin.x, r.origin.y, r.origin.z, r.prevIor);
         rays.thr_px[rid] = make_float4(r.throughput.x, r.throughput.y, r.throughput.z, r.pdx);
         rays.rad_py[rid] = make_float4(r.radiance.x, r.radiance.y, r.radiance.z, r.pdy);
@@ -67,7 +67,7 @@
     }
 }
 
-template <bool FIRST, bool VER = false>
+template <bool FIRST, bool VER = false, bool PLAIN = false>
 __global__ __launch_bounds__(256) void k_shade(DScene s0, Frame f, RayBufs rays, TraceBufs tr, HitBufs hits, const uint32_t* queue, const uint32_t* countPtr, uint32_t countImm,
                                                const uint32_t* qbase, const uint32_t* gbase , unsigned long long* contMask, uint32_t* waveCounts, uint32_t* keysTmp)
 {
@@ -106,7 +106,7 @@
             }
             f3 rd = DecodeUnitVec(r.pdx, r.pdy);
             bool hitScene = hit.T != PT_FLOAT_MAX;
-            cont = ShadeHit<FIRST>(s, f, acc, hit, hitScene, rd, r, aov, rng, gidSeed, key);
+            cont = ShadeHit<FIRST, false, PLAIN>(s, f, acc, hit, hitScene, rd, r, aov, rng, gidSeed, key);
             rays.o_ior[idx] = make_float4(r.origin.x, r.origin.y, r.origin.z, r.prevIor);
             rays.thr_px[idx] = make_float4(r.throughput.x, r.throughput.y, r.throughput.z, r.pdx);
             rays.rad_py[idx] = make_float4(r.radiance.x, r.radiance.y, r.radiance.z, r.pdy);
@@ -120,7 +120,7 @@
     (void)waveCounts;
 }
 
-template <bool ALL_HITS , bool VER = false>
+template <bool ALL_HITS , bool VER = false, bool PLAIN = false>
 __global__ __launch_bounds__(256) void k_shade_last(DScene s0, Frame f, RayBufs rays, HitBufs hits, const uint32_t* queue, const uint32_t* countPtr, const uint32_t* qbase,
                                                     float4* radSave, uint32_t* deferCount)
 {
@@ -149,7 +149,7 @@
         AovState aov; aov.albedo = splat3(0.0f); aov.normal = splat3(0.0f); aov.newWeight = 1.0f;
         const uint32_t gslot = slot - qbase[smp];
         uint32_t rng = gslot * 4096u + acc, key = 0;
-        (void)ShadeHit<false, true>(s, f, acc, hit, true, DecodeUnitVec(b.w, c.w), r, aov, rng, gslot, key);
+        (void)ShadeHit<false, true, PLAIN>(s, f, acc, hit, true, DecodeUnitVec(b.w, c.w), r, aov, rng, gslot, key);
         rays.rad_py[idx] = make_float4(r.radiance.x, r.radiance.y, r.radiance.z, c.w);
     }
 }
diff --git a/idkengine_amd/csrc/kernels_trace.hpp b/idkengine_amd/csrc/kernels_trace.hpp
--- a/idkengine_amd/csrc/kernels_trace.hpp
+++ b/idkengine_amd/csrc/kernels_trace.hpp
@@ -163,7 +163,7 @@
         contFlag[rid] = 4;
     } else if (valid) {
         f3 origin; f2 pd; uint32_t seed;
-        gen_primary(f, smp, pix, sample_index(f, smp), origin, pd, seed);
+        gen_primary_xy(f, smp, (int)x, (int)y, sample_index(f, smp), origin, pd, seed);
         f3 rd = DecodeUnitVec(pd.x, pd.y);
         f3 lo = origin, ld = rd, invDir = splat3(0.0f);
         float rootT = __builtin_inff();
diff --git a/idkengine_amd/csrc/pt_kernels.hpp b/idkengine_amd/csrc/pt_kernels.hpp
--- a/idkengine_amd/csrc/pt_kernels.hpp
+++ b/idkengine_amd/csrc/pt_kernels.hpp
@@ -22,6 +22,8 @@
     const float4* sky; int skySize;
     const TexDesc* textures; int textureCount;
     const float* srgbLut;
+    const float* unormLut;
+    const float4* matView;
     uint32_t* overflow;
     const uint32_t* ver;
 };
@@ -320,11 +322,10 @@
 DEV int global_row(const Frame& f, int ly) { return ((((ly >> f.rowBandLog2) * f.rowMod + f.rowRem) << f.rowBandLog2) | (ly & ((1 << f.rowBandLog2) - 1))); }
 
 DEV uint32_t sample_index(const Frame& f, uint32_t smp) { return f.seqFirst + f.accum[smp] * f.seqStride; }
-DEV void gen_primary(const Frame& f, uint32_t smp, uint32_t pix, uint32_t acc, f3& origin, f2& packedDir, uint32_t& rngSeed)
+DEV void gen_primary_xy(const Frame& f, uint32_t smp, int lx, int ly, uint32_t acc, f3& origin, f2& packedDir, uint32_t& rngSeed)
 {
     const float* cam = f.cams ? f.cams + 36u * smp : f.invProj;
     const float* invProj = cam; const float* invView = cam + 16; const float* vp = cam + 32;
-    int lx = (int)(pix % (uint32_t)f.W), ly = (int)(pix / (uint32_t)f.W);
     int y = global_row(f, ly), x = lx;
     uint32_t seed = (uint32_t)(y * 4096 + x) * (acc + 1u);
     float ox = rnd01(seed), oy = rnd01(seed);
@@ -339,6 +340,10 @@
     packedDir = EncodeUnitVec(camDir);
     rngSeed = seed;
 }
+DEV void gen_primary(const Frame& f, uint32_t smp, uint32_t pix, uint32_t acc, f3& origin, f2& packedDir, uint32_t& rngSeed)
+{
+    gen_primary_xy(f, smp, (int)(pix % (uint32_t)f.W), (int)(pix / (uint32_t)f.W), acc, origin, packedDir, rngSeed);
+}
 
 DEV uint32_t first_hit_gid_seed(int W, int H, int px, int py)
 {
@@ -367,8 +372,8 @@
     const size_t at = (size_t)y * (size_t)t.w + (size_t)x;
     if (fmt == 0u) return ((const float4*)t.data)[at];
     const uint32_t p = ((const uint32_t*)t.data)[at];
-    const float a = (float)(p >> 24) / 255.0f;
-    if (fmt == 1u) return make_float4((float)(p & 255u) / 255.0f, (float)((p >> 8) & 255u) / 255.0f, (float)((p >> 16) & 255u) / 255.0f, a);
+    const float a = s.unormLut[p >> 24];
+    if (fmt == 1u) return make_float4(s.unormLut[p & 255u], s.unormLut[(p >> 8) & 255u], s.unormLut[(p >> 16) & 255u], a);
     return make_float4(s.srgbLut[p & 255u], s.srgbLut[(p >> 8) & 255u], s.srgbLut[(p >> 16) & 255u], a);
 }
 DEV float4 SampleTex(const DScene& s, uint64_t handle, float u, float v)
@@ -461,7 +466,7 @@
 struct RayState { f3 origin; float prevIor; f3 throughput; float pdx; f3 radiance; float pdy; };
 struct AovState { f3 albedo; float newWeight; f3 normal; };
 
-template <bool FIRST, bool RAD_ONLY = false>
+template <bool FIRST, bool RAD_ONLY = false, bool PLAIN = false>
 DEV bool ShadeHit(const DScene& s, const Frame& f, uint32_t acc, const HitRec& hit, bool hitScene, f3 rayDir, RayState& r, AovState& aov, uint32_t& rng, uint32_t gidSeed, uint32_t& sortingKey)
 {
     if (hitScene) {
@@ -474,30 +479,36 @@
         if (!hitLight) {
             sortingKey = hit.tri;
             uint4 tri = s.tris[hit.tri];
+            const float4* tv = s.triVerts + 3 * (size_t)hit.tri;
+            float4 tvA, tvB, tvC; M34 inv;
+            if (PLAIN) { tvA = tv[0]; tvB = tv[1]; tvC = tv[2]; inv = load_inv_model(s, hit.xform); }
             uint4 v0 = s.vertices[tri.x], v1 = s.vertices[tri.y], v2 = s.vertices[tri.z];
             f3 bary = mk3(hit.bx, hit.by, 1.0f - hit.bx - hit.by);
             float u = __uint_as_float(v0.x) * bary.x + __uint_as_float(v1.x) * bary.y + __uint_as_float(v2.x) * bary.z;
             float v = __uint_as_float(v0.y) * bary.x + __uint_as_float(v1.y) * bary.y + __uint_as_float(v2.y) * bary.z;
             f3 interpNormal = normalize(Interpolate(DecompressSR11G11B10(v0.w), DecompressSR11G11B10(v1.w), DecompressSR11G11B10(v2.w), bary));
             f3 interpTangent = normalize(Interpolate(DecompressSR11G11B10(v0.z), DecompressSR11G11B10(v1.z), DecompressSR11G11B10(v2.z), bary));
-            M34 inv = load_inv_model(s, hit.xform);
+            if (!PLAIN) inv = load_inv_model(s, hit.xform);
             const GpuMesh& mesh = s.meshes[tri.w];
             const GpuMaterial& mat = s.materials[mesh.MaterialId];
             {
-                uint32_t bcf = mat.BaseColorFactor;
-                float4 bc = SampleTex(s, mat.BaseColorTexture, u, v);
-                sAlbedo = mk3(bc.x * ((float)(bcf & 255u) / 255.0f), bc.y * ((float)((bcf >> 8) & 255u) / 255.0f), bc.z * ((float)((bcf >> 16) & 255u) / 255.0f));
-                sAlpha = bc.w * ((float)((bcf >> 24) & 255u) / 255.0f);
-                float4 nm = SampleTex(s, mat.NormalTexture, u, v);
+                const float4* mv = s.matView + 2 * (size_t)mesh.MaterialId;
+                const float4 bcf = mv[0];
+                const bool noTex = PLAIN || (__float_as_uint(mv[1].x) & 1u) != 0u;
+                const float4 one = make_float4(1.0f, 1.0f, 1.0f, 1.0f);
+                float4 bc = one, nm = one, em = one, mr = one, tr = one;
+                if (!noTex) {
+                    bc = SampleTex(s, mat.BaseColorTexture, u, v); nm = SampleTex(s, mat.NormalTexture, u, v); em = SampleTex(s, mat.EmissiveTexture, u, v);
+                    mr = SampleTex(s, mat.MetallicRoughnessTexture, u, v); tr = SampleTex(s, mat.TransmissionTexture, u, v);
+                }
+                sAlbedo = mk3(bc.x * bcf.x, bc.y * bcf.y, bc.z * bcf.z);
+                sAlpha = bc.w * bcf.w;
                 sNormal = mk3(nm.x * 2.0f - 1.0f, nm.y * 2.0f - 1.0f, gsqrt(gmax(1.0f - (nm.x * nm.x + nm.y * nm.y), 0.0f)));
-                float4 em = SampleTex(s, mat.EmissiveTexture, u, v);
                 sEmissive = mk3(em.x * mat.EmissiveFactor[0], em.y * mat.EmissiveFactor[1], em.z * mat.EmissiveFactor[2]);
                 sAbsorbance = mk3(mat.Absorbance[0], mat.Absorbance[1], mat.Absorbance[2]);
-                float4 mr = SampleTex(s, mat.MetallicRoughnessTexture, u, v);
                 sMetallic = mr.x * mat.MetallicFactor; sRoughness = mr.y * mat.RoughnessFactor;
-                float4 tr = SampleTex(s, mat.TransmissionTexture, u, v);
                 sTransmission = tr.x * mat.TransmissionFactor; sIOR = mat.IOR;
-                sAlphaCutoff = mat.AlphaCutoff; sIsVolumetric = mat.IsVolumetric != 0;
+                sAlphaCutoff = mat.AlphaCutoff; sIsVolumetric = !PLAIN && mat.IsVolumetric != 0;
             }
             {
                 sEmissive = sEmissive * 1.0f + mesh.EmissiveBias * sAlbedo;
@@ -515,9 +526,8 @@
             f3 N = normalize(worldNormal), T = normalize(worldTangent), B = normalize(cross(N, T));
             f3 tn = mk3((T.x * sNormal.x + B.x * sNormal.y) + N.x * sNormal.z, (T.y * sNormal.x + B.y * sNormal.y) + N.y * sNormal.z, (T.z * sNormal.x + B.z * sNormal.y) + N.z * sNormal.z);
             sNormal = normalize(gmix(worldNormal, tn, mesh.NormalMapStrength));
-            const float4* tv = s.triVerts + 3 * (size_t)hit.tri;
-            float4 a = tv[0], b = tv[1], c = tv[2];
-            f3 p0 = mk3(a.x, a.y, a.z), p1 = mk3(b.x, b.y, b.z), p2 = mk3(c.x, c.y, c.z);
+            if (!PLAIN) { tvA = tv[0]; tvB = tv[1]; tvC = tv[2]; }
+            f3 p0 = mk3(tvA.x, tvA.y, tvA.z), p1 = mk3(tvB.x, tvB.y, tvB.z), p2 = mk3(tvC.x, tvC.y, tvC.z);
             geometricNormal = normalize(cross(p1 - p0, p2 - p0));
             geometricNormal = normalize(xform34_transposed3(inv, geometricNormal));
         } else if (f.g.DoTraceLights) {
diff --git a/idkengine_amd/csrc/shade_tables.hpp b/idkengine_amd/csrc/shade_tables.hpp
--- /dev/null
+++ b/idkengine_amd/csrc/shade_tables.hpp
@@ -0,0 +1,41 @@
+#pragma once
+#include <stdint.h>
+
+namespace shade {
+
+inline void fill_unorm_lut(float* lut256)
+{
+    for (int b = 0; b < 256; b++) lut256[b] = (float)b / 255.0f;
+}
+
+struct MatView {
+    float baseColor[4];
+    uint32_t flags;
+    uint32_t pad[3];
+};
+enum : uint32_t {
+    MAT_NO_TEXTURE = 1u,
+    MAT_VOLUMETRIC = 2u,
+};
+
+inline bool handle_is_constant(uint64_t handle, int textureCount) { return handle == 0 || handle > (uint64_t)(textureCount > 0 ? textureCount : 0); }
+
+template <class Material>
+inline MatView mat_view(const Material& m, int textureCount, const float* unormLut)
+{
+    MatView v = {};
+    const uint32_t c = m.BaseColorFactor;
+    v.baseColor[0] = unormLut[c & 255u]; v.baseColor[1] = unormLut[(c >> 8) & 255u]; v.baseColor[2] = unormLut[(c >> 16) & 255u]; v.baseColor[3] = unormLut[(c >> 24) & 255u];
+    const bool noTex = handle_is_constant(m.BaseColorTexture, textureCount) && handle_is_constant(m.NormalTexture, textureCount) && handle_is_constant(m.EmissiveTexture, textureCount) &&
+                       handle_is_constant(m.MetallicRoughnessTexture, textureCount) && handle_is_constant(m.TransmissionTexture, textureCount);
+    v.flags = (noTex ? MAT_NO_TEXTURE : 0u) | (m.IsVolumetric != 0 ? MAT_VOLUMETRIC : 0u);
+    return v;
+}
+
+inline bool scene_plain(const MatView* views, int count)
+{
+    for (int i = 0; i < count; i++) if (views[i].flags != MAT_NO_TEXTURE) return false;
+    return count > 0;
+}
+
+}
diff --git a/idkengine_amd/pathtracer.py b/idkengine_amd/pathtracer.py
--- a/idkengine_amd/pathtracer.py
+++ b/idkengine_amd/pathtracer.py
@@ -7,7 +7,7 @@
 
 
 _OPTION_NAMES = ("force_generic", "no_tile_cull", "no_lean_primary", "leaf_min", "grab_unit_log2", "grab_fixed", "lds_pad", "trace_waves", "grid_hint", "grid_rays_x4", "grid_mid_waves", "defer_last", "split", "split_donor", "split_peek", "group_threads", "query_scheduler", "split_scatter", "fused", "fused_shade_min", "leaf_pool", "pool_min", "adv_min",
-                 "wide", "wide_cap", "wide_count", "packet", "packet_min_live", "packet_waves", "inst_tlas", "inst_tlas_overlap", "inst_braid", "inst_unify", "inst_unify_radius", "uni_refill", "inst_general", "pair_nodes", "inst_sieve", "inst_sieve_overlap", "gen_pixel_major", "gen_group_max", "bounce_pixel_major", "transport", "bvh_timing", "bvh_small", "bvh_stackopt_host", "force_no_peer", "trace_variant")
+                 "wide", "wide_cap", "wide_count", "packet", "packet_min_live", "packet_waves", "inst_tlas", "inst_tlas_overlap", "inst_braid", "inst_unify", "inst_unify_radius", "uni_refill", "inst_general", "pair_nodes", "inst_sieve", "inst_sieve_overlap", "gen_pixel_major", "gen_group_max", "bounce_pixel_major", "transport", "bvh_timing", "bvh_small", "bvh_stackopt_host", "force_no_peer", "trace_variant", "expect_shade")
 
 
 class PathTracer:
```

Result: faster. 7766, median of 6 (+1.2%).
